# NyanCAD/CedarSim.jl

Measured on AMD Instinct MI355X. Metric: newton_iters_per_sec, higher is better.
Workload: dtype f64

## Files before the change

cedarsim.jl_amd/csrc/ch_bsim4.hpp:

```cpp
#pragma once
#include <cmath>
#include <cstdint>

#include "../../include/cedarhip.h"

#if defined(__HIPCC__)
#define CH_HD __host__ __device__
#define CH_D __device__ __forceinline__
#else
#define CH_HD
#define CH_D inline
#endif

namespace chip {

#define CH_B4_PACKED(X)                                                                              \
  X(type) X(mobmod) X(capmod) X(nf) X(leff) X(weff) X(weffCV) X(weffCJ) X(vtm) X(tratio1) X(toxe)    \
  X(coxe) X(coxp) X(factor1) X(phi) X(sqrtPhi) X(Xdep0) X(vbi_phi) X(cdep0) X(litl) X(ldeb) X(k1)    \
  X(k1ox) X(k2ox) X(vbsc) X(vfb_phi) X(vth0t) X(k3) X(k3b) X(vthNarrowW) X(lpe0term) X(LpeVb)        \
  X(dvt0) X(dvt1L) X(dvt2) X(dvt0w) X(dvt1wWL) X(dvt2w) X(eta0) X(etab) X(kt1eff) X(kt2t)            \
  X(theta0vb0) X(thetaRout) X(vfbzb) X(vtfbphi1) X(vtfbphi2) X(nfactor) X(cdsc) X(cdscb) X(cdscd)    \
  X(cit) X(voffcbn) X(mstar) X(ngate) X(polyT1) X(dvtp0) X(dvtp1) X(ua) X(ub) X(uc) X(u0temp) X(eu)  \
  X(vsattemp) X(a0) X(agsa0) X(a1) X(a2) X(b0term) X(keta) X(xj) X(dwg) X(dwb) X(rds0h) X(rdswmin)   \
  X(prwg) X(prwb) X(delta) X(pclmlitl) X(pdiblb) X(fproutL) X(pdits) X(pditsd) X(pditslL) X(pscbe1l) \
// ... 105 lines not shown
  const double k1ox = k1 * toxe / toxm, k2ox = k2 * toxe / toxm;
  O(k1) = k1; O(k1ox) = k1ox; O(k2ox) = k2ox; O(vbsc) = vbsc;
  const bool vth0Given = has(CH_B4_vth0);
  double vth0 = bin(CH_B4_vth0, type > 0 ? 0.7 : -0.7), vfb;
  if (has(CH_B4_vfb)) vfb = bin(CH_B4_vfb, -1.0);
  else if (vth0Given) vfb = type * vth0 - phi - k1 * sqrtPhi;
  else vfb = -1.0;
  if (!vth0Given) vth0 = type * (vfb + phi + k1ox * sqrtPhi);
  O(vfb_phi) = vfb + phi;
  O(vth0t) = type * vth0;
  O(k3) = k3; O(k3b) = k3b;
  const double vthNW = toxe * phi / (weff + w0);
  O(vthNarrowW) = vthNW;
  const double lpe0s = std::sqrt(1.0 + lpe0 / leff);
  O(lpe0term) = k1ox * (lpe0s - 1.0) * sqrtPhi;
  O(LpeVb) = std::sqrt(1.0 + lpeb / leff);
  O(dvt0) = dvt0; O(dvt1L) = dvt1 * leff; O(dvt2) = dvt2;
  O(dvt0w) = dvt0w; O(dvt1wWL) = dvt1w * weff * leff; O(dvt2w) = dvt2w;
  O(eta0) = bin(CH_B4_eta0, 0.08); O(etab) = bin(CH_B4_etab, -0.07);
  O(kt1eff) = (kt1 + kt1l / leff) * tr1; O(kt2t) = kt2 * tr1;
  auto sce = [&](double x) {
    if (x < EXP_TH) { const double e = std::exp(x), m1 = e - 1.0; return e / (m1 * m1 + 2.0 * e * MIN_EXP); }
    return 1.0 / (MAX_EXP - 2.0);
  };
  const double lt0 = std::sqrt(EPSSI / (epsrox * EPS0) * toxe * Xdep0);
  O(theta0vb0) = sce(dsub * leff / lt0);
  O(thetaRout) = bin(CH_B4_pdiblc1, 0.39) * sce(drout * leff / lt0) + bin(CH_B4_pdiblc2, 0.0086);
  {
    const double v0 = vbi - phi, f1x = factor1 * std::sqrt(Xdep0);
    const double t8 = dvt0w * sce(dvt1w * weff * leff / f1x) * v0, t9 = dvt0 * sce(dvt1 * leff / f1x) * v0;
    const double t5 = k1ox * (lpe0s - 1.0) * sqrtPhi + (kt1 + kt1l / leff) * tr1;
    O(vfbzb) = type * vth0 - t8 - t9 + k3 * vthNW + t5 - phi - k1 * sqrtPhi;
  }
  {
    const double t3 = type * vth0 - vfb - phi;
    double a = type > 0 ? 2.0 * t3 : 2.5 * t3, b = 4.0 * t3;
    O(vtfbphi1) = a < 0 ? 0 : a; O(vtfbphi2) = b < 0 ? 0 : b;
  }
  O(nfactor) = bin(CH_B4_nfactor, 1.0); O(cdsc) = bin(CH_B4_cdsc, 2.4e-4); O(cdscb) = bin(CH_B4_cdscb, 0);
  O(cdscd) = bin(CH_B4_cdscd, 0); O(cit) = bin(CH_B4_cit, 0);
  O(voffcbn) = (bin(CH_B4_voff, -0.08) + par(CH_B4_voffl, 0) / leff) * (1.0 + bin(CH_B4_tvoff, 0) * dT);
  O(mstar) = 0.5 + std::atan(bin(CH_B4_minv, 0)) / PI;
  O(ngate) = ngate;
  O(polyT1) = 1e6 * Q * EPSSI * ngate / (coxe * coxe);
  O(dvtp0) = bin(CH_B4_dvtp0, 0); O(dvtp1) = bin(CH_B4_dvtp1, 0);
  O(ua) = bin(CH_B4_ua, mobmod == 2 ? 1e-15 : 1e-9) + bin(CH_B4_ua1, 1e-9) * tr1;
  O(ub) = bin(CH_B4_ub, 1e-19) + bin(CH_B4_ub1, -1e-18) * tr1;
  O(uc) = bin(CH_B4_uc, mobmod == 1 ? -0.0465 : -0.0465e-9) + bin(CH_B4_uc1, mobmod == 1 ? -0.056 : -0.056e-9) * tr1;
  O(u0temp) = u0 * std::pow(tr, bin(CH_B4_ute, -1.5));
  O(eu) = bin(CH_B4_eu, type > 0 ? 1.67 : 1.0);
  O(vsattemp) = bin(CH_B4_vsat, 8e4) - bin(CH_B4_at, 3.3e4) * tr1;
  const double a0 = bin(CH_B4_a0, 1.0);
  O(a0) = a0; O(agsa0) = bin(CH_B4_ags, 0) * a0; O(a1) = bin(CH_B4_a1, 0); O(a2) = bin(CH_B4_a2, 1.0);
  O(b0term) = bin(CH_B4_b0, 0) / (weff + bin(CH_B4_b1, 0));
  O(keta) = bin(CH_B4_keta, -0.047); O(xj) = xj; O(dwg) = bin(CH_B4_dwg, 0); O(dwb) = bin(CH_B4_dwb, 0);
  {
    const double prt = bin(CH_B4_prt, 0), pww = std::pow(weffCJ * 1e6, bin(CH_B4_wr, 1.0)) * nf;
    double r0 = (bin(CH_B4_rdsw, 200.0) + prt * tr1) * nf / pww, rmin = (par(CH_B4_rdswmin, 0) + prt * tr1) * nf / pww;
    O(rds0h) = 0.5 * (r0 < 0 ? 0 : r0); O(rdswmin) = rmin < 0 ? 0 : rmin;
  }
  O(prwg) = bin(CH_B4_prwg, 1.0); O(prwb) = bin(CH_B4_prwb, 0); O(delta) = bin(CH_B4_delta, 0.01);
  O(pclmlitl) = bin(CH_B4_pclm, 1.3) * litl;
  if (bin(CH_B4_pclm, 1.3) <= MIN_EXP) O(pclmlitl) = 0.0;
  O(pdiblb) = bin(CH_B4_pdiblcb, 0);
  { const double fp = bin(CH_B4_fprout, 0); O(fproutL) = fp <= 0 ? 0.0 : fp * std::sqrt(leff); }
  O(pdits) = bin(CH_B4_pdits, 0); O(pditsd) = bin(CH_B4_pditsd, 0); O(pditslL) = 1.0 + par(CH_B4_pditsl, 0) * leff;
  O(pscbe1l) = bin(CH_B4_pscbe1, 4.24e8) * litl; O(pscbe2) = bin(CH_B4_pscbe2, 1e-5); O(pvag) = bin(CH_B4_pvag, 0);
  { const double al = bin(CH_B4_alpha0, 0) + bin(CH_B4_alpha1, 0) * leff; O(alphaL) = al <= 0 ? 0.0 : al / leff; }
  O(beta0) = bin(CH_B4_beta0, 0);
  {
    const double ag = bin(CH_B4_agidl, 0), bg = bin(CH_B4_bgidl, 2.3e9), cg = bin(CH_B4_cgidl, 0.5);
    O(agidlW) = (ag > 0 && bg > 0 && cg > 0) ? ag * weffCJ * nf : 0.0;
    O(bgidl) = bg; O(cgidl) = cg; O(egidl) = bin(CH_B4_egidl, 0.8); O(toxe3) = 3.0 * toxe;
  }
  O(xpart) = par(CH_B4_xpart, 0);
  const double cgsl = bin(CH_B4_cgsl, 0), cgdl = bin(CH_B4_cgdl, 0);
  const double cf = has(CH_B4_cf) ? bin(CH_B4_cf, 0) : 2.0 * epsrox * EPS0 / PI * std::log(1.0 + 0.4e-6 / toxe);
  const bool dlcOK = has(CH_B4_dlc) && dlc0 > 0;
  const double cgdo = has(CH_B4_cgdo) ? mp[CH_B4_cgdo] : (dlcOK ? dlc0 * coxe - cgdl : 0.6 * xj * coxe);
  const double cgso = has(CH_B4_cgso) ? mp[CH_B4_cgso] : (dlcOK ? dlc0 * coxe - cgsl : 0.6 * xj * coxe);
  const double cgbo = has(CH_B4_cgbo) ? mp[CH_B4_cgbo] : 2.0 * dwc0 * coxe;
  O(cgdo) = (cgdo + cf) * weffCV * nf; O(cgso) = (cgso + cf) * weffCV * nf; O(cgbo) = cgbo * leffCV * nf;
  O(cgslW) = cgsl * weffCV * nf; O(cgdlW) = cgdl * weffCV * nf;
  O(ckappas) = bin(CH_B4_ckappas, 0.6);
  O(ckappad) = has(CH_B4_ckappad) ? bin(CH_B4_ckappad, 0.6) : out[B4I_ckappas];
  O(abulkCVfactor) = 1.0 + std::pow(bin(CH_B4_clc, 1e-7) / leffCV, bin(CH_B4_cle, 0.6));
  O(acde) = bin(CH_B4_acde, 1.0) * std::pow(ndep / 2e16, -0.25);
  O(moinVtm) = bin(CH_B4_moin, 15.0) * vtm;
  O(noff) = bin(CH_B4_noff, 1.0); O(voffcv) = bin(CH_B4_voffcv, 0);
  O(CoxWL) = coxe * weffCV * leffCV * nf; O(toxp8) = 1e8 * toxp;
  {
    double jss = par(CH_B4_jss, 1e-4), jsws = par(CH_B4_jsws, 0), jswgs = par(CH_B4_jswgs, 0);
    double jsd = par(CH_B4_jsd, jss), jswd = par(CH_B4_jswd, jsws), jswgd = par(CH_B4_jswgd, jswgs);
    const double njs = par(CH_B4_njs, 1.0), njd = par(CH_B4_njd, njs);
    const double xtis = par(CH_B4_xtis, 3.0), xtid = par(CH_B4_xtid, xtis);
    if (dT != 0.0) {
      const double e0 = Eg0 / vtm0 - Eg / vtm, lt = std::log(tr);
      const double fs = std::exp((e0 + xtis * lt) / njs), fd = std::exp((e0 + xtid * lt) / njd);
      jss *= fs; jsws *= fs; jswgs *= fs; jsd *= fd; jswd *= fd; jswgd *= fd;
    }
    auto ct = [&](double c, double tc) { const double f = 1.0 + tc * dT; return f > 0 ? c * f : 0.0; };
    auto pt = [&](double p, double tp) { const double r = p - tp * dT; return r < 0.01 ? 0.01 : r; };
    const double tcj = par(CH_B4_tcj, 0), tcjsw = par(CH_B4_tcjsw, 0), tcjswg = par(CH_B4_tcjswg, 0);
    const double tpb = par(CH_B4_tpb, 0), tpbsw = par(CH_B4_tpbsw, 0), tpbswg = par(CH_B4_tpbswg, 0);
    const double cjs = par(CH_B4_cjs, 5e-4), cjd = par(CH_B4_cjd, cjs);
    const double cjsws = par(CH_B4_cjsws, 5e-10), cjswd = par(CH_B4_cjswd, cjsws);
    const double cjswgs = par(CH_B4_cjswgs, cjsws), cjswgd = par(CH_B4_cjswgd, cjswgs);
    const double pbs = par(CH_B4_pbs, 1.0), pbd = par(CH_B4_pbd, pbs), pbsws = par(CH_B4_pbsws, 1.0);
    const double pbswd = par(CH_B4_pbswd, pbsws), pbswgs = par(CH_B4_pbswgs, pbsws), pbswgd = par(CH_B4_pbswgd, pbswgs);
    O(mjs) = par(CH_B4_mjs, 0.5); O(mjd) = par(CH_B4_mjd, out[B4I_mjs]);
    O(mjsws) = par(CH_B4_mjsws, 0.33); O(mjswd) = par(CH_B4_mjswd, out[B4I_mjsws]);
    O(mjswgs) = par(CH_B4_mjswgs, out[B4I_mjsws]); O(mjswgd) = par(CH_B4_mjswgd, out[B4I_mjswgs]);
    O(PhiBS) = pt(pbs, tpb); O(PhiBD) = pt(pbd, tpb); O(PhiBSWS) = pt(pbsws, tpbsw); O(PhiBSWD) = pt(pbswd, tpbsw);
    O(PhiBSWGS) = pt(pbswgs, tpbswg); O(PhiBSWGD) = pt(pbswgd, tpbswg);
    const double dmcg = par(CH_B4_dmcg, 0), dmci = par(CH_B4_dmci, dmcg);
    const double Piso = 2.0 * (dmcg + dmci) + weffCJ, Aiso = (dmcg + dmci) * weffCJ, Psha = 2.0 * dmcg, Asha = dmcg * weffCJ;
    double eS, iS, eD, iD;
    if (((long)nf) % 2) { eS = eD = 1.0; iS = iD = (nf - 1.0) / 2.0; } else { eD = 0.0; iD = nf / 2.0; eS = 2.0; iS = nf / 2.0 - 1.0; }
    auto g = [&](int kpar) { return !std::isnan(ip[kpar]); };
    const double As = g(CH_MOS_AS) ? ip[CH_MOS_AS] : eS * Aiso + iS * Asha, Ad = g(CH_MOS_AD) ? ip[CH_MOS_AD] : eD * Aiso + iD * Asha;
    double Ps = g(CH_MOS_PS) ? (permod == 0 ? ip[CH_MOS_PS] : ip[CH_MOS_PS] - weffCJ * nf) : eS * Piso + iS * Psha;
    double Pd = g(CH_MOS_PD) ? (permod == 0 ? ip[CH_MOS_PD] : ip[CH_MOS_PD] - weffCJ * nf) : eD * Piso + iD * Psha;
    if (Ps < 0) Ps = 0;
    if (Pd < 0) Pd = 0;
    const double Isbs = As * jss + Ps * jsws + weffCJ * nf * jswgs, Isbd = Ad * jsd + Pd * jswd + weffCJ * nf * jswgd;
    O(Isbs) = Isbs; O(Isbd) = Isbd; O(Nvtms) = vtm * njs; O(Nvtmd) = vtm * njd;
    const double ijs = par(CH_B4_ijthsfwd, 0.1), ijd = par(CH_B4_ijthdfwd, ijs);
    if (Isbs > 0) { O(vjsmFwd) = vtm * njs * std::log(ijs / Isbs + 1.0); O(IVjsmFwd) = Isbs * std::exp(out[B4I_vjsmFwd] / (vtm * njs)); }
    if (Isbd > 0) { O(vjdmFwd) = vtm * njd * std::log(ijd / Isbd + 1.0); O(IVjdmFwd) = Isbd * std::exp(out[B4I_vjdmFwd] / (vtm * njd)); }
    O(czbs) = ct(cjs, tcj) * As; O(czbssw) = ct(cjsws, tcjsw) * Ps; O(czbsswg) = ct(cjswgs, tcjswg) * weffCJ * nf;
    O(czbd) = ct(cjd, tcj) * Ad; O(czbdsw) = ct(cjswd, tcjsw) * Pd; O(czbdswg) = ct(cjswgd, tcjswg) * weffCJ * nf;
  }
#undef O
  return CH_OK;
}

#if defined(__HIPCC__)
CH_D double frcp(double x) {
  const double r = __builtin_amdgcn_rcp(x);
  const double e = fma(-x, r, 1.0);
  return fma(r, fma(e, e, e), r);
}
CH_D double fsqrt(double x) {
  double y = __builtin_amdgcn_rsq(x);
  double g = x * y, h = 0.5 * y;
  double r = fma(-h, g, 0.5);
  g = fma(g, r, g); h = fma(h, r, h);
  r = fma(-h, g, 0.5);
  g = fma(g, r, g); h = fma(h, r, h);
  g = fma(fma(-g, g, x), h, g);
  return g;
}

template <int N>
struct DN {
  double v, p[N];
};
template <int N> CH_D DN<N> mkd(double v) { DN<N> r; r.v = v; for (int i = 0; i < N; ++i) r.p[i] = 0.0; return r; }
template <int N> CH_D DN<N> operator+(DN<N> a, DN<N> b) { DN<N> r; r.v = a.v + b.v; for (int i = 0; i < N; ++i) r.p[i] = a.p[i] + b.p[i]; return r; }
template <int N> CH_D DN<N> operator-(DN<N> a, DN<N> b) { DN<N> r; r.v = a.v - b.v; for (int i = 0; i < N; ++i) r.p[i] = a.p[i] - b.p[i]; return r; }
template <int N> CH_D DN<N> operator-(DN<N> a) { DN<N> r; r.v = -a.v; for (int i = 0; i < N; ++i) r.p[i] = -a.p[i]; return r; }
template <int N> CH_D DN<N> operator+(DN<N> a, double b) { a.v += b; return a; }
template <int N> CH_D DN<N> operator+(double b, DN<N> a) { a.v += b; return a; }
template <int N> CH_D DN<N> operator-(DN<N> a, double b) { a.v -= b; return a; }
template <int N> CH_D DN<N> operator-(double b, DN<N> a) { DN<N> r; r.v = b - a.v; for (int i = 0; i < N; ++i) r.p[i] = -a.p[i]; return r; }
template <int N> CH_D DN<N> operator*(DN<N> a, double b) { DN<N> r; r.v = a.v * b; for (int i = 0; i < N; ++i) r.p[i] = a.p[i] * b; return r; }
template <int N> CH_D DN<N> operator*(double b, DN<N> a) { return a * b; }
template <int N> CH_D DN<N> operator*(DN<N> a, DN<N> b) { DN<N> r; r.v = a.v * b.v; for (int i = 0; i < N; ++i) r.p[i] = fma(a.p[i], b.v, a.v * b.p[i]); return r; }
template <int N> CH_D DN<N> recip(DN<N> a) { const double r = frcp(a.v), m = -r * r; DN<N> o; o.v = r; for (int i = 0; i < N; ++i) o.p[i] = a.p[i] * m; return o; }
template <int N> CH_D DN<N> operator/(DN<N> a, DN<N> b) {
  const double r = frcp(b.v), q = a.v * r;
  DN<N> o; o.v = q; for (int i = 0; i < N; ++i) o.p[i] = fma(-q, b.p[i], a.p[i]) * r; return o;
}
template <int N> CH_D DN<N> operator/(DN<N> a, double b) { return a * frcp(b); }
template <int N> CH_D DN<N> operator/(double a, DN<N> b) { return recip(b) * a; }
template <int N> CH_D DN<N> chain(DN<N> a, double f, double fp) { DN<N> r; r.v = f; for (int i = 0; i < N; ++i) r.p[i] = a.p[i] * fp; return r; }
template <int N> CH_D DN<N> dsqrt(DN<N> a) { const double s = fsqrt(a.v); return chain(a, s, 0.5 * frcp(s)); }
enum { KP_EXP = 0, KP_LOG = 10, KP_PRE = 22, KP_COUNT = 26 };
#define CH_KPOOL_VALUES                                                                                                        \
                                                                                \
  0x1.ade156a5dcb37p-26, 0x1.28af3fca7ab0cp-22, 0x1.71dee623fde64p-19, 0x1.a01997c89e6b0p-16, 0x1.a01a014761f6ep-13,           \
  0x1.6c16c1852b7b0p-10, 0x1.1111111122322p-7, 0x1.55555555502a1p-5, 0x1.5555555555511p-3, 0x1.000000000000bp-1,               \
                        \
  1.0 / 19.0, 1.0 / 17.0, 1.0 / 15.0, 1.0 / 13.0, 1.0 / 11.0, 1.0 / 9.0, 1.0 / 7.0, 1.0 / 5.0, 1.0 / 3.0,                      \
  6.93147180369123816490e-01, 1.90821492927058770002e-10, 0.70710678118654752440,                                             \
  0x1.71547652b82fep+0, 0x1.62e42fefa39efp-1, 0x1.abc9e3b39803fp-56, 0.0
struct KLit {
  template <int I> CH_D void pair(double& a, double& b) const { constexpr double t[KP_COUNT] = {CH_KPOOL_VALUES}; a = t[I]; b = t[I + 1]; }
};
typedef double kp_d2 __attribute__((ext_vector_type(2)));
typedef const __attribute__((address_space(3))) kp_d2* kp_lds_ptr;
struct KLds {
  kp_lds_ptr p;
  template <int I> CH_D void pair(double& a, double& b) const { static_assert(I % 2 == 0, "pairs are 16-byte aligned"); const kp_d2 v = p[I / 2]; a = v.x; b = v.y; }
};
CH_D KLds kpool_fill(double* lds_table, int tid) {
  constexpr double t[KP_COUNT] = {CH_KPOOL_VALUES};
  double v = 0.0;
#pragma unroll
  for (int i = 0; i < KP_COUNT; ++i) v = (tid == i) ? t[i] : v;
  if (tid < KP_COUNT) lds_table[tid] = v;
  return KLds{(kp_lds_ptr)(__attribute__((address_space(3))) double*)lds_table};
}

template <class K>
CH_D double fexp(double x, const K k) {
#if defined(__HIP_DEVICE_COMPILE__)
  double c11, c10, c9, c8, c7, c6, c5, c4, c3, c2;
  k.template pair<KP_EXP + 0>(c11, c10); k.template pair<KP_EXP + 2>(c9, c8); k.template pair<KP_EXP + 4>(c7, c6);
  k.template pair<KP_EXP + 6>(c5, c4); k.template pair<KP_EXP + 8>(c3, c2);
  double il2, l2h, l2l, pd;
  k.template pair<KP_PRE + 0>(il2, l2h); k.template pair<KP_PRE + 2>(l2l, pd);
  const double dn = __builtin_rint(x * il2);
  double t = fma(-dn, l2h, x);
  t = fma(-dn, l2l, t);
  double p = fma(t, c11, c10);
  p = fma(t, p, c9); p = fma(t, p, c8); p = fma(t, p, c7); p = fma(t, p, c6); p = fma(t, p, c5); p = fma(t, p, c4);
  p = fma(t, p, c3); p = fma(t, p, c2); p = fma(t, p, 1.0); p = fma(t, p, 1.0);
  double z = __builtin_ldexp(p, (int)dn);
  z = x > 1024.0 ? __builtin_inf() : z;
  z = x < -1075.0 ? 0.0 : z;
  return z;
#else
  return exp(x);
#endif
}
CH_D double fexp(double x) { return fexp(x, KLit{}); }
template <int N, class K> CH_D DN<N> dexp(DN<N> a, const K k) { const double e = fexp(a.v, k); return chain(a, e, e); }
template <int N> CH_D DN<N> dexp(DN<N> a) { return dexp(a, KLit{}); }
template <class K>
CH_D double flog(double x, const K k) {
#if defined(__HIP_DEVICE_COMPILE__)
  double l19, l17, l15, l13, l11, l9, l7, l5, l3, ln2h, ln2l, pad;
  k.template pair<KP_LOG + 0>(l19, l17); k.template pair<KP_LOG + 2>(l15, l13); k.template pair<KP_LOG + 4>(l11, l9);
  k.template pair<KP_LOG + 6>(l7, l5); k.template pair<KP_LOG + 8>(l3, ln2h); k.template pair<KP_LOG + 10>(ln2l, pad);
  double m = __builtin_amdgcn_frexp_mant(x);
  int e = __builtin_amdgcn_frexp_exp(x);
  const bool lo = m < pad;
  m = lo ? 2.0 * m : m;
  e = lo ? e - 1 : e;
  const double s = (m - 1.0) * frcp(m + 1.0);
  const double z = s * s;
  double p = l19;
  p = fma(p, z, l17); p = fma(p, z, l15); p = fma(p, z, l13); p = fma(p, z, l11);
  p = fma(p, z, l9); p = fma(p, z, l7); p = fma(p, z, l5); p = fma(p, z, l3);
  const double lm = fma(2.0 * s, p * z, 2.0 * s);
  const double de = (double)e;
  const double r = fma(de, ln2h, fma(de, ln2l, lm));
  return (x > 0.0 && x < __builtin_inf()) ? r : (x == 0.0 ? -__builtin_inf() : (x > 0.0 ? x : __builtin_nan("")));
#else
  return log(x);
#endif
}
CH_D double flog(double x) { return flog(x, KLit{}); }
template <int N, class K> CH_D DN<N> dlog(DN<N> a, const K k) { return chain(a, flog(a.v, k), frcp(a.v)); }
template <int N> CH_D DN<N> dlog(DN<N> a) { return chain(a, flog(a.v), frcp(a.v)); }

template <int N, class K> CH_D DN<N> d_sce(DN<N> x, const K kc) {
  if (x.v < k::EXP_TH) {
    const DN<N> e = dexp(x, kc), m1 = e - 1.0;
    return e / (m1 * m1 + e * (2.0 * k::MIN_EXP));
  }
  return mkd<N>(1.0 / (k::MAX_EXP - 2.0));
}

struct B4Col {
  const double* p;
  CH_D double operator[](int i) const { return p[i]; }
};
CH_D B4Col b4_col(const double* table, long col) { return B4Col{table + col * (long)B4I_COUNT}; }

template <class K>
CH_D void diode(const K kc, double vb, double Is, double Nvtm, double vjm, double IVjm, double gmin, double& i, double& g) {
  if (Is <= 0.0) { i = gmin * vb; g = gmin; return; }
  const double iN = frcp(Nvtm);
  if (vb <= vjm) {
    const double t = vb * iN;
    if (t < -k::EXP_TH) { i = Is * (k::MIN_EXP - 1.0) + gmin * vb; g = gmin; }
    else { const double e = fexp(t, kc); i = Is * (e - 1.0) + gmin * vb; g = Is * e * iN + gmin; }
  } else {
    const double s = IVjm * iN;
    i = IVjm - Is + s * (vb - vjm) + gmin * vb; g = s + gmin;
  }
}
template <class K>
CH_D void junction(const K kc, double vb, double cz, double czsw, double czswg, double pb, double pbsw, double pbswg, double mj,
                   double mjsw, double mjswg, double& q, double& c) {
  if (vb < 0.0) {
    q = 0.0; c = 0.0;
    if (cz > 0.0) { const double a = 1.0 - vb * frcp(pb), s = fexp(-mj * flog(a, kc), kc); q += pb * cz * (1.0 - a * s) * frcp(1.0 - mj); c += cz * s; }
    if (czsw > 0.0) { const double a = 1.0 - vb * frcp(pbsw), s = fexp(-mjsw * flog(a, kc), kc); q += pbsw * czsw * (1.0 - a * s) * frcp(1.0 - mjsw); c += czsw * s; }
    if (czswg > 0.0) { const double a = 1.0 - vb * frcp(pbswg), s = fexp(-mjswg * flog(a, kc), kc); q += pbswg * czswg * (1.0 - a * s) * frcp(1.0 - mjswg); c += czswg * s; }
  } else {
    const double t0 = cz + czsw + czswg, t1 = cz * mj * frcp(pb) + czsw * mjsw * frcp(pbsw) + czswg * mjswg * frcp(pbswg);
    q = vb * (t0 + 0.5 * t1 * vb); c = t0 + t1 * vb;
  }
}
CH_D void overlap(double vg, double cov, double clW, double ckappa, double& q, double& c) {
  const double t0 = vg + 0.02, t1 = fsqrt(t0 * t0 + 0.08), t2 = 0.5 * (t0 - t1), dt2 = 0.5 * (1.0 - t0 * frcp(t1));
  const double t4 = fsqrt(1.0 - 4.0 * t2 * frcp(ckappa));
  q = (cov + clW) * vg - clW * (t2 + 0.5 * ckappa * (t4 - 1.0));
  c = (cov + clW) - clW * (dt2 - dt2 * frcp(t4));
}

template <int N>
struct B4Core {
  DN<N> iD, iS, iB, qd, qg, qs, qb;
};

template <int N, class K>
CH_D void b4_core(const K kc, const B4Col P, const DN<N> Vgs, const DN<N> Vds, const DN<N> Vbs, B4Core<N>& o) {
  using namespace k;
  typedef DN<N> D;
  auto dexp = [&](const D a) { return chip::dexp(a, kc); };
  auto dlog = [&](const D a) { return chip::dlog(a, kc); };
  auto d_sce = [&](const D a) { return chip::d_sce(a, kc); };
  const double phi = P[B4I_phi], sqrtPhi = P[B4I_sqrtPhi], Vtm = P[B4I_vtm], Leff = P[B4I_leff];
  const double coxe = P[B4I_coxe], itoxe = frcp(P[B4I_toxe]), icoxe = frcp(coxe), iLeff = frcp(Leff);

  D Vbseff;
  {
    const double vbsc = P[B4I_vbsc];
    const D t0 = Vbs - (vbsc + 0.001);
    const D t1 = dsqrt(t0 * t0 - 0.004 * vbsc);
    if (t0.v >= 0.0) Vbseff = 0.5 * (t0 + t1) + vbsc;
    else Vbseff = vbsc * (1.0 + (-0.002) / (t1 - t0));
    const double t9 = 0.95 * phi;
    const D u0 = t9 - Vbseff - 0.001;
    Vbseff = t9 - 0.5 * (u0 + dsqrt(u0 * u0 + 0.004 * t9));
  }
  const D Phis = phi - Vbseff;
  const D sqrtPhis = dsqrt(Phis);
  const D Xdep = sqrtPhis * (P[B4I_Xdep0] * frcp(sqrtPhi));

  const D sqXdep = dsqrt(Xdep);
  const double f1 = P[B4I_factor1], V0 = P[B4I_vbi_phi];
  auto ltf = [&](double dv2) -> D {
    const D a = Vbseff * dv2;
    const D b = (a.v >= -0.5) ? a + 1.0 : (1.0 + 3.0 * a) / (3.0 + 8.0 * a);
    return sqXdep * b * f1;
  };
  const D Theta0 = d_sce(P[B4I_dvt1L] / ltf(P[B4I_dvt2]));
  const D Delt_vth = Theta0 * (P[B4I_dvt0] * V0);
  const double dvt0w = P[B4I_dvt0w];
  D T2w = mkd<N>(0.0);
  if (dvt0w != 0.0) T2w = d_sce(P[B4I_dvt1wWL] / ltf(P[B4I_dvt2w])) * (dvt0w * V0);
  const D T1t = P[B4I_lpe0term] + P[B4I_kt1eff] + Vbseff * P[B4I_kt2t];
  D T3d = P[B4I_eta0] + P[B4I_etab] * Vbseff;
  if (T3d.v < 1.0e-4) T3d = (2.0e-4 - T3d) / (3.0 - 2.0e4 * T3d);
  const D DIBL_Sft = T3d * Vds * P[B4I_theta0vb0];
  const double vthNW = P[B4I_vthNarrowW], LpeVb = P[B4I_LpeVb], k1ox = P[B4I_k1ox], k2ox = P[B4I_k2ox];
  D Vth = P[B4I_vth0t] + (k1ox * sqrtPhis - P[B4I_k1] * sqrtPhi) * LpeVb - k2ox * Vbseff - Delt_vth - T2w +
          (P[B4I_k3] + P[B4I_k3b] * Vbseff) * vthNW + T1t - DIBL_Sft;

  D n;
  {
    const D c1 = EPSSI / Xdep;
    const D t4 = (P[B4I_nfactor] * c1 + (P[B4I_cdsc] + P[B4I_cdscb] * Vbseff + P[B4I_cdscd] * Vds) * Theta0 + P[B4I_cit]) * icoxe;
    n = (t4.v >= -0.5) ? t4 + 1.0 : (1.0 + 3.0 * t4) / (3.0 + 8.0 * t4);
  }
  {
    const double dvtp0 = P[B4I_dvtp0];
    if (dvtp0 > 0.0) {
      const D t0 = -P[B4I_dvtp1] * Vds;
      const D t2 = (t0.v < -EXP_TH) ? mkd<N>(MIN_EXP) : dexp(t0);
      const D t3 = Leff + dvtp0 * (1.0 + t2);
      Vth = Vth - n * (Vtm * dlog(Leff / t3));
    }
  }
  D Vgs_eff = Vgs;
  {
    const double ngate = P[B4I_ngate], vfbphi = P[B4I_vfb_phi];
    if (ngate > 1.0e18 && ngate < 1.0e25 && Vgs.v > vfbphi) {
      const double iT1p = frcp(P[B4I_polyT1]);
      const D t8 = Vgs - vfbphi;
      const D t4 = dsqrt(1.0 + t8 * (2.0 * iT1p));
      const D t2 = 2.0 * t8 / (t4 + 1.0);
      const D t3 = t2 * t2 * (0.5 * iT1p);
      const D t7 = 1.07 - t3;
      const D t6 = dsqrt(t7 * t7 + 0.224);
      Vgs_eff = Vgs - (1.12 - 0.5 * (t7 + t6));
    }
  }
  const D Vgst = Vgs_eff - Vth;

  D Vgsteff;
  const D inVt = recip(n * Vtm);
  {
    const double mstar = P[B4I_mstar], cc = coxe * frcp(P[B4I_cdep0]);
    const D t1 = mstar * Vgst;
    const D t2 = t1 * inVt;
    D t10;
    if (t2.v > EXP_TH) t10 = t1;
    else if (t2.v < -EXP_TH) t10 = n * (Vtm * log(1.0 + MIN_EXP));
    else t10 = (n * Vtm) * dlog(1.0 + dexp(t2));
    const D h2 = (P[B4I_voffcbn] - (1.0 - mstar) * Vgst) * inVt;
    D t9;
    if (h2.v < -EXP_TH) t9 = mstar + n * (cc * MIN_EXP);
    else if (h2.v > EXP_TH) t9 = mstar + n * (cc * MAX_EXP);
    else t9 = mstar + n * (cc * dexp(h2));
    Vgsteff = t10 / t9;
  }

  const D dsp = sqrtPhis - sqrtPhi;
  D Weff = P[B4I_weff] - 2.0 * (P[B4I_dwg] * Vgsteff + P[B4I_dwb] * dsp);
  if (Weff.v < 2.0e-8) Weff = 2.0e-8 * (4.0e-8 - Weff) / (6.0e-8 - 2.0 * Weff);
  D Rds;
  {
    const D t2 = recip(1.0 + P[B4I_prwg] * Vgsteff) + P[B4I_prwb] * dsp;
    Rds = P[B4I_rdswmin] + (t2 + dsqrt(t2 * t2 + 0.01)) * P[B4I_rds0h];
  }
  D Abulk0, Abulk;
  {
    const D t1 = (0.5 * k1ox * LpeVb) / sqrtPhis + (k2ox - P[B4I_k3b] * vthNW);
    const D t5 = Leff / (Leff + 2.0 * dsqrt(P[B4I_xj] * Xdep));
    const D t2 = P[B4I_a0] * t5 + P[B4I_b0term];
    Abulk0 = 1.0 + t1 * t2;
    const D dAdVg = -t1 * (P[B4I_agsa0] * (t5 * t5 * t5));
    Abulk = Abulk0 + dAdVg * Vgsteff;
    if (Abulk0.v < 0.1) Abulk0 = (0.2 - Abulk0) / (3.0 - 20.0 * Abulk0);
    if (Abulk.v < 0.1) Abulk = (0.2 - Abulk) / (3.0 - 20.0 * Abulk);
    const D t2k = P[B4I_keta] * Vbseff;
    const D t0k = (t2k.v >= -0.9) ? recip(1.0 + t2k) : (17.0 + 20.0 * t2k) / (0.8 + t2k);
    Abulk = Abulk * t0k;
    Abulk0 = Abulk0 * t0k;
  }
  D iueff;
  {
    const int mobmod = (int)P[B4I_mobmod];
    D t5;
    if (mobmod == 0) {
      const D t3 = (Vgsteff + Vth + Vth) * itoxe;
      t5 = t3 * (P[B4I_ua] + P[B4I_uc] * Vbseff + P[B4I_ub] * t3);
    } else if (mobmod == 1) {
      const D t3 = (Vgsteff + Vth + Vth) * itoxe;
      t5 = t3 * (P[B4I_ua] + P[B4I_ub] * t3) * (1.0 + P[B4I_uc] * Vbseff);
    } else {
      const D t0 = (Vgsteff + P[B4I_vtfbphi1]) * itoxe;
      t5 = dexp(P[B4I_eu] * dlog(t0)) * (P[B4I_ua] + P[B4I_uc] * Vbseff);
    }
    const D den = (t5.v >= -0.8) ? t5 + 1.0 : (0.6 + t5) / (7.0 + 10.0 * t5);
    iueff = den * frcp(P[B4I_u0temp]);
  }
  const D ueff = recip(iueff);
  const double vsat = P[B4I_vsattemp];
  const D WVCoxRds = Weff * Rds * (vsat * coxe);
  const D Esat = (2.0 * vsat) * iueff;
  const D EsatL = Esat * Leff;
  const D iEsatL = recip(EsatL);
  D Lambda;
  {
    const double a1 = P[B4I_a1], a2 = P[B4I_a2];
    if (a1 == 0.0) Lambda = mkd<N>(a2);
    else if (a1 > 0.0) {
      const double t0 = 1.0 - a2;
      const D t1 = t0 - a1 * Vgsteff - 0.0001;
      Lambda = a2 + t0 - 0.5 * (t1 + dsqrt(t1 * t1 + 0.0004 * t0));
    } else {
      const D t1 = a2 + a1 * Vgsteff - 0.0001;
      Lambda = 0.5 * (t1 + dsqrt(t1 * t1 + 0.0004 * a2));
    }
  }
  const D iLam = recip(Lambda);
  const D Vgst2Vtm = Vgsteff + 2.0 * Vtm;
  const D iVgst2Vtm = recip(Vgst2Vtm);
  D Vdsat;
  if (Rds.v == 0.0 && Lambda.v == 1.0) Vdsat = EsatL * Vgst2Vtm / (Abulk * EsatL + Vgst2Vtm);
  else {
    const D t9 = Abulk * WVCoxRds;
    const D t0 = 2.0 * Abulk * (t9 - 1.0 + iLam);
    const D t1 = Vgst2Vtm * (2.0 * iLam - 1.0) + Abulk * EsatL + 3.0 * (Vgst2Vtm * t9);
    const D t2 = Vgst2Vtm * (EsatL + 2.0 * (Vgst2Vtm * WVCoxRds));
    Vdsat = (t1 - dsqrt(t1 * t1 - 2.0 * t0 * t2)) / t0;
  }
  D Vdseff;
  {
    const double delta = P[B4I_delta];
    const D t1 = Vdsat - Vds - delta;
    const D t2 = dsqrt(t1 * t1 + 4.0 * delta * Vdsat);
    if (t1.v >= 0.0) Vdseff = Vdsat - 0.5 * (t1 + t2);
    else Vdseff = Vdsat * (1.0 - (2.0 * delta) / (t2 - t1));
    if (Vds.v == 0.0) Vdseff = Vds;
    if (Vdseff.v > Vds.v) Vdseff = Vds;
  }
  const D diffVds = Vds - Vdseff;
  const D Vasat = (EsatL + Vdsat + 2.0 * (WVCoxRds * Vgsteff) * (1.0 - 0.5 * Abulk * Vdsat * iVgst2Vtm)) / ((2.0 * iLam - 1.0) + WVCoxRds * Abulk);
  D Idl;
  {
    const D t0 = (Vgsteff + P[B4I_vtfbphi2]) * (0.5 * frcp(P[B4I_toxp8]));
    const D Tcen = 1.9e-9 / (1.0 + dexp(0.7 * dlog(t0)));
    const double coxp = P[B4I_coxp];
    const D Coxeff = (EPSSI * coxp) / (EPSSI + coxp * Tcen);
    const D beta = ueff * Coxeff * Weff * iLeff;
    const D fg1 = Vgsteff * (1.0 - 0.5 * Vdseff * Abulk * iVgst2Vtm);
    const D gche = beta * fg1 / (1.0 + Vdseff * iEsatL);
    Idl = gche / (1.0 + gche * Rds);
  }
  const double fpL = P[B4I_fproutL];
  const D FP = (fpL <= 0.0) ? mkd<N>(1.0) : recip(1.0 + fpL * iVgst2Vtm);
  D Pvag;
  {
    const D t9 = (P[B4I_pvag] * iEsatL) * Vgsteff;
    Pvag = (t9.v > -0.9) ? t9 + 1.0 : (0.8 + t9) / (17.0 + 20.0 * t9);
  }
  D iCclm, VACLM;
  {
    const double pl = P[B4I_pclmlitl];
    if (pl > 0.0 && diffVds.v > 1.0e-10) {
      const D Cclm = FP * Pvag * (1.0 + Rds * Idl) * (Leff + Vdsat * ueff * (0.5 * frcp(vsat))) * frcp(pl);
      iCclm = recip(Cclm);
      VACLM = Cclm * diffVds;
    } else { iCclm = mkd<N>(1.0 / MAX_EXP); VACLM = mkd<N>(MAX_EXP); }
  }
  D iVADIBL;
  {
    const double th = P[B4I_thetaRout];
    if (th > MIN_EXP) {
      const D t8 = Abulk * Vdsat;
      D va = (Vgst2Vtm - Vgst2Vtm * t8 / (Vgst2Vtm + t8)) * frcp(th);
      const D t7 = P[B4I_pdiblb] * Vbseff;
      va = va * ((t7.v >= -0.9) ? recip(1.0 + t7) : (17.0 + 20.0 * t7) / (0.8 + t7));
      iVADIBL = recip(va * Pvag);
    } else iVADIBL = mkd<N>(1.0 / MAX_EXP);
  }
  D iVADITS;
  {
    const double pdits = P[B4I_pdits];
    if (pdits > MIN_EXP) {
      const D t0 = P[B4I_pditsd] * Vds;
      const D t1 = (t0.v > EXP_TH) ? mkd<N>(MAX_EXP) : dexp(t0);
      iVADITS = recip((1.0 + P[B4I_pditslL] * t1) * frcp(pdits) * FP);
    } else iVADITS = mkd<N>(1.0 / MAX_EXP);
  }
  D iVASCBE;
  {
    const double ps2 = P[B4I_pscbe2], ps1l = P[B4I_pscbe1l];
    if (ps2 > 0.0) {
      if (diffVds.v > ps1l / EXP_TH) iVASCBE = (ps2 * iLeff) * dexp(-ps1l / diffVds);
      else iVASCBE = mkd<N>(ps2 * iLeff / MAX_EXP);
    } else iVASCBE = mkd<N>(1.0 / MAX_EXP);
  }
  D Idsa = Idl * (1.0 + diffVds * iVADIBL);
  Idsa = Idsa * (1.0 + diffVds * iVADITS);
  Idsa = Idsa * (1.0 + dlog((Vasat + VACLM) / Vasat) * iCclm);
  D Isub = mkd<N>(0.0);
  {
    const double aL = P[B4I_alphaL], beta0 = P[B4I_beta0];
    if (aL > 0.0 && beta0 > 0.0) {
      D t1;
      if (diffVds.v > beta0 / EXP_TH) t1 = aL * diffVds * dexp(-beta0 / diffVds);
      else t1 = (aL * MIN_EXP) * diffVds;
      Isub = t1 * (Idsa * Vdseff);
    }
  }
  const double nf = P[B4I_nf];
  const D Ids = Idsa * (1.0 + diffVds * iVASCBE) * Vdseff * nf;
  Isub = Isub * nf;
  D Igidl = mkd<N>(0.0), Igisl = mkd<N>(0.0);
  {
    const double agW = P[B4I_agidlW];
    if (agW > 0.0) {
      const double bg = P[B4I_bgidl], cg = P[B4I_cgidl], eg = P[B4I_egidl], it3x = frcp(P[B4I_toxe3]);
      const D Vbd = Vbs - Vds;
      const D t1 = (Vds - Vgs_eff - eg) * it3x;
      if (t1.v > 0.0 && Vbd.v <= 0.0) {
        const D t2 = bg / t1;
        const D ig = (t2.v < 100.0) ? agW * t1 * dexp(-t2) : (agW * 3.720075976e-44) * t1;
        const D t5 = -Vbd * Vbd * Vbd;
        Igidl = ig * (t5 / (cg + t5));
      }
      const D s1 = (-Vgs_eff - eg) * it3x;
      if (s1.v > 0.0 && Vbs.v <= 0.0) {
        const D t2 = bg / s1;
        const D ig = (t2.v < 100.0) ? agW * s1 * dexp(-t2) : (agW * 3.720075976e-44) * s1;
        const D t5 = -Vbs * Vbs * Vbs;
        Igisl = ig * (t5 / (cg + t5));
      }
    }
  }
  D qg = mkd<N>(0.0), qb = mkd<N>(0.0), qsm = mkd<N>(0.0), qdm = mkd<N>(0.0);
  const double xpart = P[B4I_xpart];
  if (xpart >= 0.0 && (int)P[B4I_capmod] != 0) {
    const D VbseffCV = (Vbseff.v < 0.0) ? Vbseff : phi - Phis;
    const double CoxWL = P[B4I_CoxWL], vfbzb = P[B4I_vfbzb], Cox = P[B4I_coxp], Tox = P[B4I_toxp8], ldeb = P[B4I_ldeb];
    const double iTox = frcp(Tox), cwl = CoxWL * icoxe;
    const D T0q = n * (Vtm * P[B4I_noff]);
    const D T1q = (Vgst - P[B4I_voffcv]) / T0q;
    D Vgc;
    if (T1q.v > EXP_TH) Vgc = Vgst - P[B4I_voffcv];
    else if (T1q.v < -EXP_TH) Vgc = T0q * log(1.0 + MIN_EXP);
    else Vgc = T0q * dlog(1.0 + dexp(T1q));
    const D V3 = vfbzb - Vgs_eff + VbseffCV - 0.02;
    const D Vfbeff = vfbzb - 0.5 * (V3 + dsqrt(V3 * V3 + ((vfbzb <= 0.0) ? -0.08 * vfbzb : 0.08 * vfbzb)));
    const D tm = (Vgs_eff - VbseffCV - vfbzb) * (P[B4I_acde] * iTox);
    D Tcen;
    if (tm.v > -EXP_TH && tm.v < EXP_TH) Tcen = ldeb * dexp(tm);
    else Tcen = mkd<N>(tm.v <= -EXP_TH ? ldeb * MIN_EXP : ldeb * MAX_EXP);
    const double LINK = 1.0e-11 * Tox;
    const D V3c = ldeb - Tcen - LINK;
    Tcen = ldeb - 0.5 * (V3c + dsqrt(V3c * V3c + 4.0 * LINK * ldeb));
    D CoxWLcen = (Cox * EPSSI * cwl) / (Cox * Tcen + EPSSI);
    const D Qac0 = CoxWLcen * (Vfbeff - vfbzb);
    const double h0 = 0.5 * k1ox;
    const D T3s = Vgs_eff - Vfbeff - VbseffCV - Vgc;
    D T1s;
    if (k1ox == 0.0) T1s = mkd<N>(0.0);
    else if (T3s.v < 0.0) T1s = h0 + T3s * frcp(k1ox);
    else T1s = dsqrt(h0 * h0 + T3s);
    const D Qsub0 = CoxWLcen * (k1ox * (T1s - h0));
    double Den, T0d;
    if (k1ox <= 0.0) { Den = 0.25 * P[B4I_moinVtm]; T0d = 0.5 * sqrtPhi; }
    else { Den = P[B4I_moinVtm] * k1ox * k1ox; T0d = k1ox * sqrtPhi; }
    const D DeltaPhi = Vtm * dlog(1.0 + (2.0 * T0d + Vgc) * Vgc * frcp(Den));
    const D T3t = 4.0 * (Vth - vfbzb - phi);
    const D T0t = ((T3t.v >= 0.0) ? Vgc + T3t : Vgc + 1.0e-20) * (0.5 * iTox);
    Tcen = 1.9e-9 / (1.0 + dexp(0.7 * dlog(T0t)));
    CoxWLcen = (Cox * EPSSI * cwl) / (Cox * Tcen + EPSSI);
    const D AbulkCV = Abulk0 * P[B4I_abulkCVfactor];
    const D T1 = Vgc - DeltaPhi;
    const D VdsatCV = T1 / AbulkCV;
    const D T0v = VdsatCV - Vds - 0.02;
    const D T1v = dsqrt(T0v * T0v + 0.08 * VdsatCV);
    D VdseffCV;
    if (T0v.v >= 0.0) VdseffCV = VdsatCV - 0.5 * (T0v + T1v);
    else VdseffCV = VdsatCV * (1.0 - 0.04 / (T1v - T0v));
    if (Vds.v == 0.0) VdseffCV = Vds;
    const D T0 = AbulkCV * VdseffCV;
    const D T2 = 12.0 * (T1 - 0.5 * T0 + 1.0e-20);
    const D iT2 = recip(T2);
    const D T3 = T0 * iT2;
    qg = CoxWLcen * (T1 - T0 * (0.5 - T3));
    qb = CoxWLcen * (1.0 - AbulkCV) * (0.5 * VdseffCV - T3 * VdseffCV);
    if (xpart > 0.5) qsm = -CoxWLcen * (0.5 * T1 + 0.25 * T0 - 0.5 * T0 * T3);
    else if (xpart < 0.5) {
      const D T4b = T1 * ((2.0 / 3.0) * T0 * T0 + T1 * (T1 - (4.0 / 3.0) * T0)) - (2.0 / 15.0) * T0 * T0 * T0;
      qsm = -(72.0 * CoxWLcen * (iT2 * iT2)) * T4b;
    } else qsm = -0.5 * qg;
    qg = qg + Qac0 + Qsub0 - qb;
    qb = qb - (Qac0 + Qsub0);
    qdm = -(qg + qb + qsm);
  }
  o.iD = Ids + Isub + Igidl; o.iS = Igisl - Ids; o.iB = -(Isub + Igidl + Igisl);
  o.qd = qdm; o.qg = qg; o.qs = qsm; o.qb = qb;
}

struct B4Two {
  double ibs, gbs, ibd, gbd, qbs, cbs, qbd, cbd, qgd, cgd, qgs, cgs, qgb, cgb;
};
template <class K>
CH_D void b4_two_terminal(const K kc, const B4Col P, double vgs, double vds, double vbs, double gmin, B4Two& t) {
  const double vbd = vbs - vds;
  diode(kc, vbs, P[B4I_Isbs], P[B4I_Nvtms], P[B4I_vjsmFwd], P[B4I_IVjsmFwd], gmin, t.ibs, t.gbs);
  diode(kc, vbd, P[B4I_Isbd], P[B4I_Nvtmd], P[B4I_vjdmFwd], P[B4I_IVjdmFwd], gmin, t.ibd, t.gbd);
  junction(kc, vbs, P[B4I_czbs], P[B4I_czbssw], P[B4I_czbsswg], P[B4I_PhiBS], P[B4I_PhiBSWS], P[B4I_PhiBSWGS], P[B4I_mjs], P[B4I_mjsws], P[B4I_mjswgs], t.qbs, t.cbs);
  junction(kc, vbd, P[B4I_czbd], P[B4I_czbdsw], P[B4I_czbdswg], P[B4I_PhiBD], P[B4I_PhiBSWD], P[B4I_PhiBSWGD], P[B4I_mjd], P[B4I_mjswd], P[B4I_mjswgd], t.qbd, t.cbd);
  if ((int)P[B4I_capmod] != 0) {
    overlap(vgs - vds, P[B4I_cgdo], P[B4I_cgdlW], P[B4I_ckappad], t.qgd, t.cgd);
    overlap(vgs, P[B4I_cgso], P[B4I_cgslW], P[B4I_ckappas], t.qgs, t.cgs);
    t.cgb = P[B4I_cgbo]; t.qgb = t.cgb * (vgs - vbs);
  } else { t.qgd = t.cgd = t.qgs = t.cgs = t.qgb = t.cgb = 0.0; }
}

template <class K = KLit>
CH_D void b4_device(const B4Col P, double vd, double vg, double vs, double vb, double gmin, double* out, const K kc = K{}) {
  const double tp = P[B4I_type];
  const double vds = tp * (vd - vs), vgs = tp * (vg - vs), vbs = tp * (vb - vs);
  const bool fwd = vds >= 0.0;
  typedef DN<3> D3;
  D3 Vgs = mkd<3>(fwd ? vgs : vgs - vds), Vds = mkd<3>(fwd ? vds : -vds), Vbs = mkd<3>(fwd ? vbs : vbs - vds);
  Vgs.p[0] = 1.0; Vds.p[1] = 1.0; Vbs.p[2] = 1.0;
  B4Core<3> c;
  b4_core<3>(kc, P, Vgs, Vds, Vbs, c);
  double* I = out; double* Qo = out + 4; double* G = out + 8; double* C = out + 24;
  auto put = [&](int row, const D3& x, double* val, double* M) {
    val[row] = x.v; M[row * 4 + 0] = x.p[1]; M[row * 4 + 1] = x.p[0]; M[row * 4 + 3] = x.p[2]; M[row * 4 + 2] = -(x.p[0] + x.p[1] + x.p[2]);
  };
  put(0, c.iD, I, G); put(1, mkd<3>(0.0), I, G); put(2, c.iS, I, G); put(3, c.iB, I, G);
  put(0, c.qd, Qo, C); put(1, c.qg, Qo, C); put(2, c.qs, Qo, C); put(3, c.qb, Qo, C);
  if (!fwd) {
    auto sw = [](double& x, double& y) { const double t = x; x = y; y = t; };
    sw(I[0], I[2]); sw(Qo[0], Qo[2]);
#pragma unroll
    for (int cc = 0; cc < 4; ++cc) { sw(G[0 * 4 + cc], G[2 * 4 + cc]); sw(C[0 * 4 + cc], C[2 * 4 + cc]); }
#pragma unroll
    for (int r = 0; r < 4; ++r) { sw(G[r * 4 + 0], G[r * 4 + 2]); sw(C[r * 4 + 0], C[r * 4 + 2]); }
  }
  B4Two t;
  b4_two_terminal(kc, P, vgs, vds, vbs, gmin, t);
  auto two = [&](double* val, double* M, int a, int b, double x, double dx) {
    val[a] += x; val[b] -= x;
    M[a * 4 + a] += dx; M[a * 4 + b] -= dx; M[b * 4 + a] -= dx; M[b * 4 + b] += dx;
  };
  two(I, G, 3, 2, t.ibs, t.gbs); two(I, G, 3, 0, t.ibd, t.gbd);
  two(Qo, C, 3, 2, t.qbs, t.cbs); two(Qo, C, 3, 0, t.qbd, t.cbd);
  two(Qo, C, 1, 0, t.qgd, t.cgd); two(Qo, C, 1, 2, t.qgs, t.cgs); two(Qo, C, 1, 3, t.qgb, t.cgb);
#pragma unroll
  for (int r = 0; r < 4; ++r) { I[r] *= tp; Qo[r] *= tp; }
}

CH_D void b4_device_quad(const B4Col P, double vd, double vg, double vs, double vb, double gmin, int sub, double m, double* st) {
  const double tp = P[B4I_type];
  const double vds = tp * (vd - vs), vgs = tp * (vg - vs), vbs = tp * (vb - vs);
  const bool fwd = vds >= 0.0;
  typedef DN<1> D1;
  D1 Vgs = mkd<1>(fwd ? vgs : vgs - vds), Vds = mkd<1>(fwd ? vds : -vds), Vbs = mkd<1>(fwd ? vbs : vbs - vds);
  Vgs.p[0] = sub == 0 ? 1.0 : 0.0; Vds.p[0] = sub == 1 ? 1.0 : 0.0; Vbs.p[0] = sub == 2 ? 1.0 : 0.0;
  B4Core<1> c;
  b4_core<1>(KLit{}, P, Vgs, Vds, Vbs, c);
  auto quad_sum = [](double x) { x += __shfl_xor(x, 1); x += __shfl_xor(x, 2); return x; };
  auto colval = [&](const D1& x) { const double sum = quad_sum(x.p[0]); return sub == 3 ? -sum : x.p[0]; };
  double gI[4] = {colval(c.iD), 0.0, colval(c.iS), colval(c.iB)};
  double gQ[4] = {colval(c.qd), colval(c.qg), colval(c.qs), colval(c.qb)};
  double I4[4] = {c.iD.v, 0.0, c.iS.v, c.iB.v}, Q4[4] = {c.qd.v, c.qg.v, c.qs.v, c.qb.v};
  int col = sub == 0 ? 1 : (sub == 1 ? 0 : (sub == 2 ? 3 : 2));
  if (!fwd) {
    auto sw = [](double& x, double& y) { const double t = x; x = y; y = t; };
    sw(gI[0], gI[2]); sw(gQ[0], gQ[2]); sw(I4[0], I4[2]); sw(Q4[0], Q4[2]);
    col = col == 0 ? 2 : (col == 2 ? 0 : col);
  }
  B4Two t;
  b4_two_terminal(KLit{}, P, vgs, vds, vbs, gmin, t);
  auto two = [&](double* val, double* gcol, int a, int b, double x, double dx) {
    val[a] += x; val[b] -= x;
    const double s = col == a ? dx : (col == b ? -dx : 0.0);
    gcol[a] += s; gcol[b] -= s;
  };
  two(I4, gI, 3, 2, t.ibs, t.gbs); two(I4, gI, 3, 0, t.ibd, t.gbd);
  two(Q4, gQ, 3, 2, t.qbs, t.cbs); two(Q4, gQ, 3, 0, t.qbd, t.cbd);
  two(Q4, gQ, 1, 0, t.qgd, t.cgd); two(Q4, gQ, 1, 2, t.qgs, t.cgs); two(Q4, gQ, 1, 3, t.qgb, t.cgb);
#pragma unroll
  for (int r = 0; r < 4; ++r) { st[8 + r * 4 + col] = m * gI[r]; st[24 + r * 4 + col] = m * gQ[r]; }
  if (sub == 3) {
    const double mt = m * tp;
#pragma unroll
    for (int r = 0; r < 4; ++r) { st[r] = mt * I4[r]; st[4 + r] = mt * Q4[r]; }
  }
}
#endif

}
```

cedarsim.jl_amd/csrc/ch_engine_persist.hpp:

```cpp
#pragma once

constexpr size_t P_MAX_ENTRIES = 64, P_MAX_PWL = 2048;
inline bool ch_circuit::persist_eligible(std::string& why, bool own_steps) {
  auto no = [&](const char* m) { why = m; return false; };
  if (nwt.path != 1) return no("the circuit takes the sparse path");
  if (desc.A.n_comp < 1) return no("the circuit has no unknowns");
  if (!(stru.lu_variant == 8 || stru.lu_variant == 12 || stru.lu_variant == 16)) return no("a Jacobian block has more than 16 unknowns");
  if (desc.A.wide) {
    if (desc.A.classes.size() != 1) return no("compiled Verilog-A devices in blocks of several classes");
    if (desc.A.nb > 0) return no("compiled Verilog-A devices in a bordered form");
    if (stru.wide_split ? (stru.wide_l + stru.wide_other > 32) : (stru.h_cms[0].nslots > 64)) return no("a block's compiled devices need more evaluation lanes than a wave pair offers");
    if (own_steps && tab.S == 1 && desc.A.n_comp > 1) return no("per-block steps of one circuit with compiled Verilog-A devices");
  } else if (stru.block_threads != 64) return no("a block needs more than one wavefront of device slots");
  if (tab.max_mc > 8) return no("more than 8 MOSFET classes in a block");
  if (tab.Ssrc != 1) return no("per-sample source parameters");
  const bool wg_consts = own_steps && tab.S == 1 && desc.A.n_comp > 1;
  if (!wg_consts && (stru.needed_src.size() > (size_t)P_MAXSRC || desc.A.known.size() + (size_t)stru.n_dev_src() > P_MAX_ENTRIES)) return no("more than 64 sources / known-node and source values per attempt");
  if (!(tab.S == 1 || desc.A.n_comp == 1)) return no("several blocks per sample in a multi-sample batch");
  if (desc.A.nb > 0 && (tab.S != 1 || desc.A.border_dev.size() > 8)) return no("bordered form: one sample and at most 8 devices on the border alone");
  for (const ClassMeta& m : stru.h_cms) if ((!desc.A.wide && m.nslots > 64) || m.nc > stru.lu_variant || m.n_work <= 0 || m.spare1 <= 0) return no("a block class does not fit the one-wave register path");
  if (ps.n_cu == 0) { hipDeviceProp_t prop; if (hipGetDeviceProperties(&prop, ctx->device) != hipSuccess) return no("hipGetDeviceProperties failed"); ps.n_cu = prop.multiProcessorCount; }
  const long nblk = (long)desc.A.n_comp * tab.S;
  const int bpw = persist_bpw(nblk);
  if (nblk > (long)bpw * ps.n_cu && !own_steps) return no("more blocks than resident wavefronts (4 per CU)");
  if (!own_steps && (nblk + bpw - 1) / bpw > 256) return no("more than 256 workgroups in a grid-wide reduction");
  size_t npwl = 0; for (int i : stru.needed_src) npwl += desc.src[i].ts.size();
  if (!wg_consts && npwl > P_MAX_PWL) return no("piecewise-linear tables above 2048 points");
  return true;
}
inline int ch_circuit::persist_bpw(long nblk) const {
  if (ps.n_cu > 0 && desc.A.wide && stru.wide_split && nblk <= 2L * ps.n_cu) return 2;
  return PW;
}
inline bool ch_circuit::persist_own_steps(const ch_tran_opts& o) const {
  return ((desc.A.n_comp == 1 && tab.S > 1) || (tab.S == 1 && desc.A.n_comp > 1 && desc.A.nb == 0 && !desc.A.wide)) && o.n_saveat > 0 && o.step_control != CH_STEPS_SHARED && !env_on(Env::LOCKSTEP);
}
inline size_t ch_circuit::persist_wave_doubles(bool wg_consts) const {
  const size_t n_ent = wg_consts ? (size_t)P_MAXSRC : desc.A.known.size() + stru.n_dev_src();
  return stru.lds_doubles_fixed + 16 * (size_t)desc.A.max_nc + 10 + 48 + P_MAXSRC + n_ent + (size_t)tab.max_mc * B4L_STRIDE + (stru.lds_extra_bytes + stru.lds_plan_bytes + 7) / 8 + 2;
}
inline bool ch_circuit::persist_blob(const std::vector<int>& kn, const std::vector<int>& ds, std::vector<int>& bi, std::vector<double>& bd, std::vector<int>& need) const {
  const int nsrc = (int)desc.src.size();
  std::vector<char> nd(std::max(1, nsrc), 0);
  for (int k : kn) for (auto& tm : desc.A.known[k].terms) nd[tm.first] = 1;
  for (int j : ds) if (j < (int)stru.dev_src.size()) nd[stru.dev_src[j]] = 1;
  need.clear();
  for (int i = 0; i < nsrc; ++i) if (nd[i]) need.push_back(i);
  std::vector<int> pos(std::max(1, nsrc), -1);
  for (size_t i = 0; i < need.size(); ++i) pos[need[i]] = (int)i;
  std::vector<double> pt, py;
  bi = {(int)need.size(), (int)(kn.size() + ds.size()), 0, (int)kn.size()};
  for (int i : need) { bi.push_back(desc.src[i].kind); bi.push_back((int)pt.size()); bi.push_back((int)desc.src[i].ts.size()); pt.insert(pt.end(), desc.src[i].ts.begin(), desc.src[i].ts.end()); py.insert(py.end(), desc.src[i].ys.begin(), desc.src[i].ys.end()); }
  bi[2] = (int)pt.size();
  std::vector<int> eptr(1, 0), eidx; std::vector<double> ecoef;
  for (int k : kn) { for (auto& tm : desc.A.known[k].terms) { eidx.push_back(pos[tm.first]); ecoef.push_back(tm.second); } eptr.push_back((int)eidx.size()); }
  for (int j : ds) { if (j < (int)stru.dev_src.size()) { eidx.push_back(pos[stru.dev_src[j]]); ecoef.push_back(1.0); } eptr.push_back((int)eidx.size()); }
  bi.insert(bi.end(), eptr.begin(), eptr.end()); bi.insert(bi.end(), eidx.begin(), eidx.end());
  bd.clear();
  for (int i : need) for (int k = 0; k < CH_SRC_NPAR; ++k) bd.push_back(tab.h_src_par[(size_t)i * CH_SRC_NPAR + k]);
  bd.insert(bd.end(), ecoef.begin(), ecoef.end()); bd.insert(bd.end(), pt.begin(), pt.end()); bd.insert(bd.end(), py.begin(), py.end());
  for (size_t q = 4; q < bi.size(); ++q) if (bi[q] < 0) return false;
  return need.size() <= (size_t)P_MAXSRC && kn.size() + ds.size() <= P_MAX_ENTRIES && pt.size() <= P_MAX_PWL;
}

inline const void* persist_kernel(bool wide, int mode, int nc, bool pair) {
  struct Row { bool wide; int mode, nc; bool pair; const void* fn; };
  static const Row rows[] = {
    {true, PM_OWN, 16, true, (const void*)tran_persistent_kernel<16, true, PM_OWN, true>}, {true, PM_OWN, 16, false, (const void*)tran_persistent_kernel<16, false, PM_OWN, true>},
    {true, PM_LOCKSTEP, 16, true, (const void*)tran_persistent_kernel<16, true, PM_LOCKSTEP, true>}, {true, PM_LOCKSTEP, 16, false, (const void*)tran_persistent_kernel<16, false, PM_LOCKSTEP, true>},
    {false, PM_BORDER, 16, true, (const void*)tran_persistent_kernel<16, true, PM_BORDER>}, {false, PM_BORDER, 16, false, (const void*)tran_persistent_kernel<16, false, PM_BORDER>},
    {false, PM_OWN, 12, true, (const void*)tran_persistent_kernel<12, true, PM_OWN>}, {false, PM_OWN, 12, false, (const void*)tran_persistent_kernel<12, false, PM_OWN>},
    {false, PM_OWN, 16, true, (const void*)tran_persistent_kernel<16, true, PM_OWN>}, {false, PM_OWN, 16, false, (const void*)tran_persistent_kernel<16, false, PM_OWN>},
    {false, PM_LOCKSTEP, 12, true, (const void*)tran_persistent_kernel<12, true>}, {false, PM_LOCKSTEP, 12, false, (const void*)tran_persistent_kernel<12, false>},
    {false, PM_LOCKSTEP, 16, true, (const void*)tran_persistent_kernel<16, true>}, {false, PM_LOCKSTEP, 16, false, (const void*)tran_persistent_kernel<16, false>},
  };
  for (const Row& r : rows) if (r.wide == wide && r.mode == mode && r.nc == nc && r.pair == pair) return r.fn;
  return nullptr;
}

struct PersistConsts {
  std::vector<int> ci; std::vector<double> cd; size_t max_ci = 0, max_cd = 0;
  std::vector<int> wgc, wgk;
  std::vector<double> bps_all;
};
inline bool ch_circuit::persist_consts(bool wg_consts, int n_wg, int bpw, double t0, double t1, PersistConsts& pc) {
  const int nblk = desc.A.n_comp * tab.S, nk = (int)desc.A.known.size(), nds = stru.n_dev_src();
  if (!wg_consts) {
    std::vector<int> kn(nk), ds(nds), need;
    std::iota(kn.begin(), kn.end(), 0); std::iota(ds.begin(), ds.end(), 0);
    if (!persist_blob(kn, ds, pc.ci, pc.cd, need)) { set_err("device-resident stepper: the source tables exceed the kernel's limits"); return false; }
    pc.max_ci = pc.ci.size(); pc.max_cd = pc.cd.size();
  } else {
    pc.wgk.assign((size_t)n_wg * P_MAXSRC, -1);
    for (int w = 0; w < n_wg; ++w) {
      std::vector<char> uk(nk, 0), ud(nds, 0);
      for (int b = w * bpw; b < std::min(nblk, (w + 1) * bpw); ++b)
        for (int i = 0; i < desc.A.comp_ndev[b]; ++i) {
          const EDev& e = desc.A.edev[desc.A.comp_dofs[b] + i];
          for (int k = 0; k < NTERM; ++k) if (e.term[k] < 0) uk[-e.term[k] - 1] = 1;
          if (e.src >= 0) ud[torn.dsrc_host[desc.A.comp_dofs[b] + i]] = 1;
        }
      std::vector<int> kn, ds, need, bi; std::vector<double> bd;
      for (int k = 0; k < nk; ++k) if (uk[k]) kn.push_back(k);
      for (int j = 0; j < nds; ++j) if (ud[j]) ds.push_back(j);
      if (ds.empty()) ds.push_back(0);
      if (!persist_blob(kn, ds, bi, bd, need)) { set_err("device-resident stepper: a workgroup's blocks reference more than 64 sources / known nodes"); return false; }
      for (size_t q = 0; q < kn.size(); ++q) pc.wgk[(size_t)w * P_MAXSRC + q] = kn[q];
      for (size_t q = 0; q < ds.size(); ++q) pc.wgk[(size_t)w * P_MAXSRC + kn.size() + q] = ds[q];
      std::vector<double> wb, wc;
      { std::vector<std::pair<double, double>> pts;
        for (int i : need) source_breakpoint_codes(desc.src[i], &tab.h_src_par[(size_t)i * CH_SRC_NPAR], t0, t1, pts);
        merge_breakpoints(pts, t1, wb, wc); }
      pc.wgc.insert(pc.wgc.end(), {(int)pc.ci.size(), (int)pc.cd.size(), (int)bi.size(), (int)bd.size(), (int)pc.bps_all.size(), (int)wb.size()});
      pc.ci.insert(pc.ci.end(), bi.begin(), bi.end()); pc.cd.insert(pc.cd.end(), bd.begin(), bd.end());
      pc.bps_all.insert(pc.bps_all.end(), wb.begin(), wb.end());
      pc.bps_all.insert(pc.bps_all.end(), wc.begin(), wc.end());
      pc.max_ci = std::max(pc.max_ci, bi.size()); pc.max_cd = std::max(pc.max_cd, bd.size());
    }
  }
  return true;
}

inline size_t ch_circuit::persist_va_arena(int bpw, size_t& lds) const {
  size_t va_arena = 0;
  if (desc.A.wide && !env_on(Env::VA_NO_LDS)) {
    size_t worst = 0;
    for (int cpt = 0; cpt < desc.A.n_comp; ++cpt) {
      size_t need = 0;
      for (int i = 0; i < desc.A.comp_ndev[cpt]; ++i) {
        const EDev& e = desc.A.edev[desc.A.comp_dofs[cpt] + i];
        if (e.kind != K_VA) continue;
        const int mod = desc.dev[e.hdev].ipar[0];
        need += (size_t)((va_gen::param_doubles(mod) + 1) & ~1) + (size_t)((va_gen::cache_doubles(mod) + 1) & ~1);
      }
      worst = std::max(worst, need);
    }
    const size_t room = lds < 148 * 1024 ? (148 * 1024 - lds) / sizeof(double) : 0;
    va_arena = std::min(worst * (size_t)bpw, room);
    lds += va_arena * sizeof(double);
    if (env_on(Env::DEBUG_STEPPER)) std::fprintf(stderr, "[stepper] compiled devices: %zu doubles per block, LDS arena %zu doubles, workgroup LDS %zu bytes\n", worst, va_arena, lds);
  }
  return va_arena;
}

inline int ch_circuit::persist_collect(ch_result& R, const TranCtl& cs, bool own_steps, bool single_batch, const std::vector<double>& htimes,
                                       const std::vector<double>& hpts, const std::vector<double>& hrows, int status, hclock::time_point tstart) {
  hipStream_t st = ctx->stream;
  const int n_obs = R.n_obs;
  stats.persist_attempts = cs.n_attempts;
  stats.persist_barrier_s = (double)cs.t_cycles_barrier * 1e-8;
#ifdef CH_STAMPS
  { static const char* nm[12] = {"set-up", "coefficients", "sources", "predictor", "eval", "gather", "rows+norm", "LU+solves", "update", "candidate", "grid-reduce", "controller"};
    std::fprintf(stderr, "[pstamps] attempts %lld; cycles per attempt (wave 0 of workgroup 0):", cs.n_attempts);
    for (int q = 0; q < 12; ++q) std::fprintf(stderr, " %s %.0f", nm[q], (double)cs.stamps[q] / (double)std::max<long long>(1, cs.n_attempts));
    std::fprintf(stderr, "\n"); }
#endif
  R.stats.naccept += cs.naccept; R.stats.nreject += cs.nreject; R.stats.nnonlinconvfail += cs.nconvfail;
  const long long arr_iters = (own_steps && tab.S == 1) ? cs.max_iters : cs.sum_iters;
  R.stats.n_block_iters += cs.sum_block_iters; R.stats.nnonliniter += arr_iters; R.stats.nf += arr_iters; R.stats.njacs += arr_iters;
  R.stats.nfactors += arr_iters; R.stats.nsolve += arr_iters;
  const size_t nt = htimes.size();
  R.times = htimes;
  R.pts.assign(nt, 0);
  if (own_steps == false) for (size_t r = 0; r < nt; ++r) R.pts[r] = (int32_t)hpts[r];
  R.values.assign((size_t)n_obs * nt * tab.S, 0.0);
  if (single_batch) {
    const size_t n = (size_t)n_obs * nt * tab.S;
    if (n > 0) {
      HIPCHK(ps.d_ptrans.alloc(n));
      hipLaunchKernelGGL(transpose_rows_kernel, dim3((unsigned)std::min<size_t>(65535, (n + 255) / 256)), dim3(256), 0, st, (const double*)ps.d_prows.p, ps.d_ptrans.p, (long)nt, (long)n_obs, tab.S);
      HIPCHK(hipGetLastError());
      HIPCHK(hipMemcpyAsync(R.values.data(), ps.d_ptrans.p, n * sizeof(double), hipMemcpyDeviceToHost, st));
      HIPCHK(hipStreamSynchronize(st));
      bool plain = true;
      for (int ob = 0; ob < n_obs && plain; ++ob) {
        if (stru.obs_primary[ob] != ob) plain = false;
        else if (desc.obs_kind[ob] == 0 && desc.A.node_unknown[desc.obs_index[ob]] < 0) plain = false;
        else if (desc.obs_kind[ob] == 1) { const int br = desc.dev[desc.obs_index[ob]].branch; if (br < 0 || desc.A.branch_unknown[br] < 0) plain = false; }
      }
      if (plain) { R.dev_values = ps.d_ptrans.p; R.dev_n = (int64_t)n; }
    }
  } else
  rows_to_obs_major(hrows.data(), nt, 0, nt, n_obs, tab.S, R.values.data());
  return finish_tran(R, 0, cs.t, status, tstart);
}

inline int ch_circuit::tran_persistent(double t0, double t1, const ch_tran_opts& o, ch_result& R, const std::vector<double>& bps, int kmax, double dtmin, double dtmax,
                                       int max_steps, int nmaxit, hclock::time_point tstart, bool& used, const ch_dc_opts* dcm, long long* dc_iters,
                                       const std::vector<double>* bpc) {
  used = false;
  hipStream_t st = ctx->stream;
  g_arena = &arena;
// ... 196 lines not shown
```

cedarsim.jl_amd/csrc/ch_kernels.hpp:

```cpp
#pragma once
#include <hip/hip_runtime.h>

#include "ch_analysis.hpp"
#include "ch_bsim4.hpp"
#include "_generated/va_models.hpp"

namespace chip {

struct ClassMeta {
  int nc, ndev, nonlinear, nslots;
  int wl_ofs, n_work, spare0, spare1;
  int n_mat_src, n_vec_src, blob_ofs, blob_ints;
};

struct BlockMeta {
  int uofs, dofs, mc_n, mc_ofs;
  ClassMeta cm;
  int mc[8];
};

struct BlockOut {
  int status;
  int iters;
  int ndiff;
// ... 87 lines not shown
};
__device__ __forceinline__ void widen_stamp(const double* t, double* st) {
#pragma unroll
  for (int k = 0; k < 4; ++k) {
    st[k] = t[k]; st[8 + k] = t[4 + k];
#pragma unroll
    for (int j = 0; j < 4; ++j) { st[16 + k * 8 + j] = t[8 + k * 4 + j]; st[80 + k * 8 + j] = t[24 + k * 4 + j]; }
  }
}

__device__ __forceinline__ void eval_linear(const EvalCtx& a, int kind, int d, long pi, double m, const double (&v)[4], const double* svl, double* st) {
  switch (kind) {
    case K_R: {
      const double g = m / a.dpar[pi], i = g * (v[0] - v[1]);
      st[0] = i; st[1] = -i; st[4] = 0.0; st[5] = 0.0;
      st[8] = g; st[9] = -g; st[12] = -g; st[13] = g;
      st[24] = 0.0; st[25] = 0.0; st[28] = 0.0; st[29] = 0.0;
    } break;
    case K_C: {
      const double c = m * a.dpar[pi], q = c * (v[0] - v[1]);
      st[0] = 0.0; st[1] = 0.0; st[4] = q; st[5] = -q;
      st[8] = 0.0; st[9] = 0.0; st[12] = 0.0; st[13] = 0.0;
      st[24] = c; st[25] = -c; st[28] = -c; st[29] = c;
    } break;
    case K_I: {
      const double i = m * svl[a.dsrc[d]];
      st[0] = i; st[1] = -i; st[4] = 0.0; st[5] = 0.0;
    } break;
    case K_V: case K_L: case K_VCVS_A: {
      const double ib = v[2];
      const double src = kind == K_V ? svl[a.dsrc[d]] : 0.0;
      const double l = kind == K_L ? a.dpar[pi] : 0.0;
      st[0] = m * ib; st[1] = -m * ib; st[2] = v[0] - v[1] - src;
      st[4] = 0.0; st[5] = 0.0; st[6] = -l * ib;
      st[8 + 2] = m; st[8 + 6] = -m; st[8 + 8] = 1.0; st[8 + 9] = -1.0; st[8 + 10] = 0.0;
      st[24 + 2] = 0.0; st[24 + 6] = 0.0; st[24 + 8] = 0.0; st[24 + 9] = 0.0; st[24 + 10] = -l;
    } break;
    case K_VCVS_B: {
      const double g = a.dpar[pi];
      st[0] = -g * (v[1] - v[2]); st[4] = 0.0;
      st[8 + 1] = -g; st[8 + 2] = g; st[24 + 1] = 0.0; st[24 + 2] = 0.0;
    } break;
    case K_VCCS: {
      const double g = m * a.dpar[pi], i = g * (v[2] - v[3]);
      st[0] = i; st[1] = -i; st[4] = 0.0; st[5] = 0.0;
      st[8 + 2] = g; st[8 + 3] = -g; st[8 + 6] = -g; st[8 + 7] = g;
      st[24 + 2] = 0.0; st[24 + 3] = 0.0; st[24 + 6] = 0.0; st[24 + 7] = 0.0;
    } break;
  }
}

__device__ __noinline__ void b4_device_call(const B4Col P, double vd, double vg, double vs, double vb, double gmin, double* out) {
  VA_KEEP_RETURN_ADDRESS;
  b4_device(P, vd, vg, vs, vb, gmin, out);
}
template <bool WIDE>
__device__ __forceinline__ void eval_slot(const EvalCtx a, int s, int dofs, int slot, const double* xl, int uofs,
                                          const double* kvl, const double* svl, const double* pl, double* stage) {
  const int dl = (slot >> 4) & 0x01ffffff;
  const int d = dofs + dl;
  double* st_final = stage + (size_t)dl * StampLayout<WIDE>::STRIDE;
  const int kind = a.dkind[d];
  const int* tm = a.dterm + NTERM * d;
  if (WIDE && kind == K_VA) {
    double vv[NTERM];
#pragma unroll
    for (int k = 0; k < NTERM; ++k) { const int t = tm[k]; vv[k] = t >= 0 ? xl[t - uofs] : kvl[-t - 1]; }
    const long pi = (long)a.dhdev[d] * a.Spar + (a.Spar > 1 ? s : 0);
    const va::Env env{a.temp_k, a.gmin};
    va_gen::stamp_dir_c(a.dcls_local[d], a.vapar + a.dsrc[d], a.vacache + a.dvac[d], vv, env, a.dmult[pi], slot & 7, (slot & 8) != 0,
                        (slot & (1 << 29)) ? ((slot >> 30) & 1) : -1, st_final);
    return;
  }
  double tmp40[WIDE ? 40 : 1];
  double* st = WIDE ? tmp40 : st_final;
  if (WIDE) {
#pragma unroll
    for (int j = 0; j < 40; ++j) tmp40[j] = 0.0;
  }
  double v[4];
#pragma unroll
  for (int k = 0; k < 4; ++k) { const int t = tm[k]; v[k] = t >= 0 ? xl[t - uofs] : kvl[-t - 1]; }
  const int hd = a.dhdev[d];
  const long pi = (long)hd * a.Spar + (a.Spar > 1 ? s : 0);
  const double m = a.dmult[pi];
  if (kind == K_MOS) {
    const B4Col P{pl + (size_t)a.dcls_local[d] * B4L_STRIDE};
    double o[40];
    if (WIDE) b4_device_call(P, v[0], v[1], v[2], v[3], a.gmin, o);
    else b4_device(P, v[0], v[1], v[2], v[3], a.gmin, o);
#pragma unroll
    for (int j = 0; j < 40; ++j) st[j] = m * o[j];
    if (WIDE) widen_stamp(st, st_final);
    return;
  }
  eval_linear(a, kind, d, pi, m, v, svl, st);
  if (WIDE) widen_stamp(st, st_final);
}

struct WideMeta {
  int mod, dl;
  const double* P; const double* C;
  double m;
  int t[NTERM];
};
__device__ __forceinline__ WideMeta load_wide_meta(const EvalCtx& a, int s, int dofs, int slot) {
  WideMeta q;
  q.mod = -1; q.dl = 0; q.P = nullptr; q.C = nullptr; q.m = 0.0;
#pragma unroll
  for (int k = 0; k < NTERM; ++k) q.t[k] = -1;
  if (slot < 0) return q;
  const int dl = (slot >> 4) & 0x01ffffff, d = dofs + dl;
  if (a.dkind[d] != K_VA) return q;
  q.dl = dl; q.mod = a.dcls_local[d];
  q.P = a.vapar + a.dsrc[d]; q.C = a.vacache + a.dvac[d];
  q.m = a.dmult[(long)a.dhdev[d] * a.Spar + (a.Spar > 1 ? s : 0)];
#pragma unroll
  for (int k = 0; k < NTERM; ++k) q.t[k] = a.dterm[NTERM * d + k];
  return q;
}
template <bool LDS>
__device__ __forceinline__ void eval_wide_cached(const WideMeta& q, const EvalCtx& a, int slot, const double* xl, int uofs, const double* kvl, double* stage) {
  double vv[NTERM];
#pragma unroll
  for (int k = 0; k < NTERM; ++k) { const int t = q.t[k]; vv[k] = t >= 0 ? xl[t - uofs] : kvl[-t - 1]; }
  const va::Env env{a.temp_k, a.gmin};
  const int part = (slot & (1 << 29)) ? ((slot >> 30) & 1) : -1;
  double* st = stage + (size_t)q.dl * StampLayout<true>::STRIDE;
  if (LDS) va_gen::stamp_dir_lds(q.mod, (va::lds_cptr)q.P, (va::lds_cptr)q.C, vv, env, q.m, slot & 7, (slot & 8) != 0, part, st);
  else va_gen::stamp_dir_c(q.mod, q.P, q.C, vv, env, q.m, slot & 7, (slot & 8) != 0, part, st);
}

struct SlotMeta {
  int kind;
  int dl;
  int t[4];
  int cls, src;
  double m, par;
};
__device__ __forceinline__ SlotMeta load_slot_meta(const EvalCtx& a, int s, int dofs, int uofs, int slot) {
  SlotMeta q;
  q.kind = 0; q.dl = 0; q.cls = 0; q.src = 0; q.m = 0.0; q.par = 0.0;
#pragma unroll
  for (int k = 0; k < 4; ++k) q.t[k] = -1;
  if (slot < 0) return q;
  const int dl = slot >> 4, d = dofs + dl;
  q.dl = dl; q.kind = a.dkind[d];
#pragma unroll
  for (int k = 0; k < 4; ++k) { const int t = a.dterm[NTERM * d + k]; q.t[k] = t >= 0 ? t - uofs : t; }
  const long pi = (long)a.dhdev[d] * a.Spar + (a.Spar > 1 ? s : 0);
  q.m = a.dmult[pi]; q.par = a.dpar[pi]; q.cls = a.dcls_local[d]; q.src = a.dsrc[d];
  return q;
}
template <int PART, class K = KLit>
__device__ __forceinline__ void eval_cached(const SlotMeta& q, double gmin, const double* xl, const double* kvl, const double* svl, const double* pl, double* stage, const K kc = K{}) {
  if (q.kind == 0 || (PART == 0 && q.kind != K_MOS)) return;
  double* st = stage + (size_t)q.dl * StampLayout<false>::STRIDE;
  double v[4];
#pragma unroll
  for (int k = 0; k < 4; ++k) v[k] = q.t[k] >= 0 ? xl[q.t[k]] : kvl[-q.t[k] - 1];
  if (q.kind == K_MOS) {
    const B4Col P{pl + (size_t)q.cls * B4L_STRIDE};
    double o[40];
    b4_device(P, v[0], v[1], v[2], v[3], gmin, o, kc);
    if (PART != 1) {
#pragma unroll
      for (int j = 0; j < 4; ++j) st[j] = q.m * o[j];
#pragma unroll
      for (int j = 8; j < 24; ++j) st[j] = q.m * o[j];
    }
    if (PART != 0) {
#pragma unroll
      for (int j = 4; j < 8; ++j) st[j] = q.m * o[j];
#pragma unroll
      for (int j = 24; j < 40; ++j) st[j] = q.m * o[j];
    }
    return;
  }
  const double m = q.m;
  switch (q.kind) {
    case K_R: {
      const double g = m / q.par, i = g * (v[0] - v[1]);
      st[0] = i; st[1] = -i; st[4] = 0.0; st[5] = 0.0;
      st[8] = g; st[9] = -g; st[12] = -g; st[13] = g;
      st[24] = 0.0; st[25] = 0.0; st[28] = 0.0; st[29] = 0.0;
    } break;
    case K_C: {
      const double c = m * q.par, qq = c * (v[0] - v[1]);
      st[0] = 0.0; st[1] = 0.0; st[4] = qq; st[5] = -qq;
      st[8] = 0.0; st[9] = 0.0; st[12] = 0.0; st[13] = 0.0;
      st[24] = c; st[25] = -c; st[28] = -c; st[29] = c;
    } break;
    case K_I: {
      const double i = m * svl[q.src];
      st[0] = i; st[1] = -i; st[4] = 0.0; st[5] = 0.0;
    } break;
    case K_V: case K_L: case K_VCVS_A: {
      const double ib = v[2];
      const double src = q.kind == K_V ? svl[q.src] : 0.0;
      const double l = q.kind == K_L ? q.par : 0.0;
      st[0] = m * ib; st[1] = -m * ib; st[2] = v[0] - v[1] - src;
      st[4] = 0.0; st[5] = 0.0; st[6] = -l * ib;
      st[8 + 2] = m; st[8 + 6] = -m; st[8 + 8] = 1.0; st[8 + 9] = -1.0; st[8 + 10] = 0.0;
      st[24 + 2] = 0.0; st[24 + 6] = 0.0; st[24 + 8] = 0.0; st[24 + 9] = 0.0; st[24 + 10] = -l;
    } break;
    case K_VCVS_B: {
      const double g = q.par;
      st[0] = -g * (v[1] - v[2]); st[4] = 0.0;
      st[8 + 1] = -g; st[8 + 2] = g; st[24 + 1] = 0.0; st[24 + 2] = 0.0;
    } break;
    case K_VCCS: {
      const double g = m * q.par, i = g * (v[2] - v[3]);
      st[0] = i; st[1] = -i; st[4] = 0.0; st[5] = 0.0;
      st[8 + 2] = g; st[8 + 3] = -g; st[8 + 6] = -g; st[8 + 7] = g;
      st[24 + 2] = 0.0; st[24 + 3] = 0.0; st[24 + 6] = 0.0; st[24 + 7] = 0.0;
    } break;
  }
}

template <int CTRL> __device__ __forceinline__ int dpp_i(int v) { return __builtin_amdgcn_update_dpp(v, v, CTRL, 0xF, 0xF, false); }
template <int CTRL> __device__ __forceinline__ double dpp_d(double v) {
  const int lo = dpp_i<CTRL>(__double2loint(v)), hi = dpp_i<CTRL>(__double2hiint(v));
  return __hiloint2double(hi, lo);
}
constexpr int DPP_QP_1032 = 0xB1, DPP_QP_2301 = 0x4E, DPP_HALF_MIRROR = 0x141, DPP_MIRROR = 0x140;
template <int NCV> __device__ __forceinline__ double row_max(double v) {
  v = fmax(v, dpp_d<DPP_QP_1032>(v)); v = fmax(v, dpp_d<DPP_QP_2301>(v));
  v = fmax(v, dpp_d<DPP_HALF_MIRROR>(v)); v = fmax(v, dpp_d<DPP_MIRROR>(v));
  if (NCV > 16) v = fmax(v, __shfl_xor(v, 16));
  return v;
}
template <int NCV> __device__ __forceinline__ double row_sum(double v) {
  v += dpp_d<DPP_QP_1032>(v); v += dpp_d<DPP_QP_2301>(v); v += dpp_d<DPP_HALF_MIRROR>(v); v += dpp_d<DPP_MIRROR>(v);
  if (NCV > 16) v += __shfl_xor(v, 16);
  return v;
}
template <int NCV> __device__ __forceinline__ int row_min_i(int v) {
  v = min(v, dpp_i<DPP_QP_1032>(v)); v = min(v, dpp_i<DPP_QP_2301>(v)); v = min(v, dpp_i<DPP_HALF_MIRROR>(v)); v = min(v, dpp_i<DPP_MIRROR>(v));
  if (NCV > 16) v = min(v, __shfl_xor(v, 16));
  return v;
}

template <int NCV> __device__ __forceinline__ int row_max_i(int v) {
  v = max(v, dpp_i<DPP_QP_1032>(v)); v = max(v, dpp_i<DPP_QP_2301>(v)); v = max(v, dpp_i<DPP_HALF_MIRROR>(v)); v = max(v, dpp_i<DPP_MIRROR>(v));
  if (NCV > 16) v = max(v, __shfl_xor(v, 16));
  return v;
}

template <int NC>
__device__ __forceinline__ bool lu_solve_regs(double (&r)[NC + 1], int nc, int lane, double& sol, int* myrow_out = nullptr) {
  bool done = lane >= nc;
  int mystep = -1;
  double ipiv = 0.0;
  int piv[NC];
#pragma unroll
  for (int k = 0; k < NC; ++k) {
    piv[k] = 0;
    if (k < nc) {
      const int hi = __double2hiint(r[k]) & 0x7fffffff;
      const int key = done ? -1 : ((hi & ~63) | (63 - lane));
      const int best = __builtin_amdgcn_readfirstlane(row_max_i<NC>(key));
      if (best < 64 || best >= 0x7e300000) return false;
      const int bi = 63 - (best & 63);
      piv[k] = bi;
      const double ipk = frcp(bcast(r[k], bi));
      const double l = (!done && lane != bi) ? r[k] * ipk : 0.0;
#pragma unroll
      for (int j = k + 1; j <= NC; ++j) r[j] = fma(-l, bcast(r[j], bi), r[j]);
      if (lane == bi) { done = true; mystep = k; ipiv = ipk; }
    }
  }
  double rhs = 0.0;
#pragma unroll
  for (int j = 0; j <= NC; ++j) if (j == nc) rhs = r[j];
  double out = 0.0;
#pragma unroll
  for (int k = NC - 1; k >= 0; --k) {
    if (k < nc) {
      const double xk = bcast(rhs * ipiv, piv[k]);
      if (lane == k) out = xk;
      if (mystep >= 0 && mystep < k) rhs = fma(-r[k], xk, rhs);
    }
  }
  sol = out;
  if (myrow_out) {
    int mr = lane;
#pragma unroll
    for (int k = 0; k < NC; ++k) if (k < nc && lane == k) mr = piv[k];
    *myrow_out = mr;
  }
  return true;
}

template <int K> __device__ __forceinline__ double row_bcast(double v) {
  static_assert(K >= 0 && K < 16, "row_newbcast lane");
  const double b = __builtin_amdgcn_update_dpp(v, v, 0x150 + K, 0xF, 0xF, true);
  return b;
}
template <int NC, int J> struct RowDot {
  static __device__ __forceinline__ double run(const double (&c)[NC], double x, int nc, double q) {
    if constexpr (J < NC) {
      if (J < nc) { const double xj = row_bcast<J>(x); q = fma(c[J], xj, q); }
      return RowDot<NC, J + 1>::run(c, x, nc, q);
    } else return q;
  }
};

template <int NC, int K>
struct LuStaticStep {
  static __device__ __forceinline__ void fwd(double (&r)[NC + 1], int nc, int lane, int& lkey, double& ipiv) {
    if constexpr (K < NC) {
      if (K < nc) {
        const double ipk = frcp(row_bcast<K>(r[K]));
        double pj[NC + 1];
#pragma unroll
        for (int j = K + 1; j <= NC; ++j) pj[j] = row_bcast<K>(r[j]);
        if (lane == K) ipiv = ipk;
// ... 885 lines not shown
```

cedarsim.jl_amd/csrc/ch_persist.hpp:

```cpp
#pragma once
#include <hip/hip_runtime.h>

#include "ch_gather_plan.hpp"
#include "ch_kernels.hpp"

#ifdef CH_STAMPS
#define P_STAMP(slot) do { const unsigned long long now_ = __builtin_readcyclecounter(); pacc_[slot] += now_ - plast_; plast_ = now_; } while (0)
#else
#define P_STAMP(slot) do { } while (0)
#endif

namespace chip {

constexpr int PW = 4;
constexpr int P_MAXSRC = 64;
constexpr int P_NREC = 8;
constexpr int P_SCR = 64;
enum { PX_RUNNING = 0, PX_DONE = 1, PX_ROWS_FULL = 2, PX_ABORT = 3 };

struct TranCtl {
  double t, h;
  double tslot[8];
  int k, nhist, steps_at_order, reset_rate;
  int ibp, isave, status, exit_reason;
// ... 176 lines not shown
    double v = part[f];
#pragma unroll
    for (int w = 1; w < PW; ++w) { const double u = part[w * P_NREC + f]; v = fmaxop ? fmax(v, u) : v + u; }
    if (p.n_wg > 1) {
      if (lane < 16) st_gran(wrec + (size_t)wg * 16 + g16, p_split(v, lane, gen));
      const long long t0 = wall_clock64();
      if (wg < n_grp) {
        const int members = (p.n_wg - grp + 7) >> 3;
        p_u64 x[8];
        for (;;) {
          bool all = true;
          const unsigned ab = ld_agent_u(abort_flag);
#pragma unroll
          for (int q = 0; q < 8; ++q) {
            const int mm = q * 4 + m4;
            x[q] = mm < members ? ld_gran(wrec + (size_t)(grp + 8 * mm) * 16 + g16) : ((p_u64)gen << 32);
            all = all && (unsigned)(x[q] >> 32) == gen;
          }
          if (__all(all)) break;
          if (ab != 0u) { ok = false; break; }
          if (wall_clock64() - t0 > p.spin_ticks) { __hip_atomic_store(abort_flag, 1u | (gen << 8), __ATOMIC_RELAXED, __HIP_MEMORY_SCOPE_AGENT); ok = false; break; }
          __builtin_amdgcn_s_sleep(1);
        }
        double acc = (m4 < members) ? p_join(x[0], lane) : 0.0;
#pragma unroll
        for (int q = 1; q < 8; ++q) {
          const double u = (q * 4 + m4 < members) ? p_join(x[q], lane) : 0.0;
          acc = fmaxop ? fmax(acc, u) : acc + u;
        }
        acc = p_rows4(acc, fmaxop, scr, lane);
        if (lane < 16) st_gran(grec + (size_t)grp * 16 + g16, p_split(acc, lane, gen));
      }
      p_u64 y[2];
      for (;;) {
        bool all = true;
        const unsigned ab = ok ? ld_agent_u(abort_flag) : 1u;
#pragma unroll
        for (int q = 0; q < 2; ++q) {
          const int gg = q * 4 + m4;
          y[q] = (ok && gg < n_grp) ? ld_gran(grec + (size_t)gg * 16 + g16) : ((p_u64)gen << 32);
          all = all && (unsigned)(y[q] >> 32) == gen;
        }
        if (__all(all) || !ok) break;
        if (ab != 0u) { ok = false; break; }
        if (wall_clock64() - t0 > p.spin_ticks) { __hip_atomic_store(abort_flag, 2u | (gen << 8), __ATOMIC_RELAXED, __HIP_MEMORY_SCOPE_AGENT); ok = false; break; }
        __builtin_amdgcn_s_sleep(1);
      }
      double acc = (m4 < n_grp) ? p_join(y[0], lane) : 0.0;
      { const double u = (4 + m4 < n_grp) ? p_join(y[1], lane) : 0.0; acc = fmaxop ? fmax(acc, u) : acc + u; }
      v = p_rows4(acc, fmaxop, scr, lane);
    }
    if (lane < 16 && !(lane & 1)) summ[f] = v;
    if (lane == 0) *s_abort = ok ? 0 : 1;
  }
  __syncthreads();
  return *s_abort == 0;
}

__device__ __forceinline__ double p_coef(double tau0, const double* tsl, int head, int kk, int np, int nkm1, int nkp1, bool lte, double hh, int lane, double& a0) {
  double tau[8];
  tau[0] = tau0;
#pragma unroll
  for (int i = 1; i < 8; ++i) tau[i] = tsl[(head - (i - 1)) & 7];
  const int set = lane >> 3, j = lane & 7;
  const int npk = kk | (np << 4) | (nkm1 << 8) | (nkp1 << 12);
  const int n = set <= 3 ? (npk >> (4 * set)) & 15 : 0;
  const bool act = set <= 3 && j >= 1 && j <= n;
  const unsigned mn = act ? ((2u << n) - 2u) & ~(1u << j) : 0u;
  const unsigned md = mn | ((act && set == 0) ? 1u : 0u);
  const bool rcp = lane >= 33 && lane <= 37, cks = lane >= 38 && lane <= 40;
  const int pick = lane == 38 ? kk + 1 : lane == 39 ? kk : kk + 2;
  const int m = cks ? ((pick >= 1 && pick <= 8) ? pick : 1) : j;
  const double tj = tsl[(head - (m - 1)) & 7];
  double num = 1.0, den = 1.0;
#pragma unroll
  for (int i = 0; i < 8; ++i) {
    num *= ((mn >> i) & 1u) ? tau[0] - tau[i] : 1.0;
    den *= ((md >> i) & 1u) ? tj - tau[i] : 1.0;
  }
  if (!act) { num = 0.0; den = 1.0; }
  const bool on = rcp ? j <= kk : lane == 38 ? lte : lane == 39 ? nkm1 > 0 : nkp1 > 0;
  if (rcp || cks) { num = on ? (rcp ? 1.0 : hh) : 0.0; den = tau[0] - tj; }
  if (num == 0.0) den = 1.0;
  const double q = num / den;
  a0 = bcast(row_sum<16>(rcp ? q : 0.0), 32);
  return q;
}
__device__ __attribute__((noinline, cold)) double p_coef_dense(double tsv, const double* tsl, int head, int msv, int lane) {
  double a0;
  return p_coef(tsv, tsl, head, 0, msv, 0, 0, false, 0.0, lane, a0);
}

enum { PM_LOCKSTEP = 0, PM_OWN = 1, PM_BORDER = 2 };
template <int NC, bool PAIR, int MODE = PM_LOCKSTEP, bool WIDE = false>
__global__ __launch_bounds__(PW * 64, 1) void tran_persistent_kernel(const PersistArgs p) {
  typedef StampLayout<WIDE> SL;
  extern __shared__ double lds[];
  __shared__ int s_abort;
  __shared__ double s_bdec[4];
  __shared__ __attribute__((aligned(16))) double s_kpool[KP_COUNT];
  const NewtonArgs& a = p.a;
  const int tid = threadIdx.x, lane = tid & 63, wave = tid >> 6, wg = blockIdx.x;
  const long long cyc0 = wall_clock64();
  long long cyc_bar = 0;
#ifdef CH_STAMPS
  unsigned long long pacc_[12] = {0, 0, 0, 0, 0, 0, 0, 0, 0, 0, 0, 0}, plast_ = __builtin_readcyclecounter();
#endif
  double* cdl = lds;
  int* cil = (int*)(cdl + p.n_cd);
  double* part = cdl + p.n_cd + ((p.n_ci + 1) >> 1);
  double* summ = part + PW * P_NREC;
  int* pfl = (int*)(summ + P_NREC);
  double* W = summ + P_NREC + 4 + P_SCR + (size_t)wave * p.wave_doubles;
  constexpr bool own = MODE == PM_OWN;
  const int* const wgc = own ? p.wgc : nullptr;
  const double* bps_own = nullptr; int nbp_own = 0;
  if (own && wgc) {
    const int* e = wgc + 6 * wg;
    const int* gci = p.ci + e[0]; const double* gcd = p.cd + e[1]; const int n_ci = e[2], n_cd = e[3];
    bps_own = p.bps + e[4]; nbp_own = e[5];
    for (int i = tid; i < n_cd; i += PW * 64) cdl[i] = gcd[i];
    for (int i = tid; i < n_ci; i += PW * 64) cil[i] = gci[i];
  } else {
    for (int i = tid; i < p.n_cd; i += PW * 64) cdl[i] = p.cd[i];
    for (int i = tid; i < p.n_ci; i += PW * 64) cil[i] = p.ci[i];
  }
#define P_BPS ((own && wgc) ? bps_own : p.bps)
#define P_NBP ((own && wgc) ? nbp_own : p.nbp)
  if (tid == 0) s_abort = 0;
  if (tid < 8) pfl[tid] = 0;
  const KLds kpool = kpool_fill(s_kpool, tid);
  __syncthreads();
  const PConst C{cil, cdl};

  const int blk = wg * p.bpw + wave;
  const bool live = wave < p.bpw && blk < p.nblk;
  const int bq = live ? blk : 0;
  const int c = bq / a.S, s = bq - c * a.S;
  const BlockMeta bm = a.bmeta[c];
  const ClassMeta cm = bm.cm;
  const int nc = cm.nc, ndev = cm.ndev, uofs = bm.uofs, dofs = bm.dofs, lda = nc + 1;
  double* st = W;
  double* A = st + (size_t)ndev * SL::STRIDE;
  double* Cm = A + (size_t)nc * lda;
  double* xl = Cm + (size_t)nc * nc;
  double* xp = xl + nc; double* Fv = xp + nc; double* Qv = Fv + nc; double* hq = Qv + nc;
  double* wv = hq + nc; double* qn = wv + nc; double* pm = qn + nc; double* pp = pm + nc; double* x0l = pp + nc;
  int* dml = (int*)(x0l + nc);
  double* Xh = x0l + 2 * nc; double* Qh = Xh + 8 * nc;
  double* tsl = Qh + 8 * nc; double* coef = tsl + 8;
  long long* stl = (long long*)(coef + 40);
  double* kvl = coef + 48; double* svl = kvl + (wgc ? C.ci[3] : a.nk);
  double* pl = wgc ? kvl + P_MAXSRC : svl + a.nsrc;
  int* mptr = (int*)(pl + (size_t)a.max_mc * B4L_STRIDE);
  int* slots = mptr + (nc * nc + 1) + (nc + 1);
  const int* gplan = mptr + cm.blob_ints;
  const int g_recs = (cm.spare0 - GP_HEAD_INTS) / 3;
  const uint2* gsrc = (const uint2*)(gplan + GP_HEAD_INTS);
  const unsigned* gctl = (const unsigned*)(gplan + GP_HEAD_INTS + 2 * g_recs);
  const int g_trips = __builtin_amdgcn_readfirstlane(cm.spare1);
  const long sofs = (long)s * a.n_unk + uofs;
  const bool mine = live && lane < nc;
  const int nc_s = __builtin_amdgcn_readfirstlane(nc);
  const int role = wave & 1, pairq = wave >> 1, half = lane >> 5;
  int* pf = pfl + pairq * 4;
  const int blk_h = wg * p.bpw + (wave & ~1) + half;
  const bool live_h = PAIR && (wave & ~1) + half < p.bpw && blk_h < p.nblk;
  const int bqh = live_h ? blk_h : 0, c_h = bqh / a.S, s_h = bqh - c_h * a.S;
  const int uofs_h = PAIR ? a.bmeta[c_h].uofs : uofs, dofs_h = PAIR ? a.bmeta[c_h].dofs : dofs;
  double* Wh = summ + P_NREC + 4 + P_SCR + (size_t)((wave & ~1) + half) * p.wave_doubles;
  double* st_h = Wh; double* xl_h = Wh + (xl - W); double* pl_h = Wh + (pl - W);
  const int* slots_h = (const int*)((const char*)slots + ((const char*)Wh - (const char*)W));
  int pseq = 0; bool pair_broken = false;
  auto pair_sync = [&]() {
    ++pseq;
    lds_fence();
    if (lane == 0) __hip_atomic_store(pf + role, pseq, __ATOMIC_RELAXED, __HIP_MEMORY_SCOPE_WORKGROUP);
    long long t0w = 0;
    for (unsigned trip = 1; __hip_atomic_load(pf + (1 - role), __ATOMIC_RELAXED, __HIP_MEMORY_SCOPE_WORKGROUP) < pseq; ++trip) {
      if (trip % P_SPIN_CLOCK == 0u) {
        const long long now = wall_clock64();
        if (trip == P_SPIN_CLOCK) t0w = now;
        else if (now - t0w > p.spin_ticks) { pair_broken = true; __hip_atomic_store(p.counters + 9 * 32, 3u | ((unsigned)pseq << 8), __ATOMIC_RELAXED, __HIP_MEMORY_SCOPE_AGENT); break; }
      }
      __builtin_amdgcn_s_sleep(0);
    }
    lds_fence();
  };

  if (live) {
    const int* bsrc = a.blob + cm.blob_ofs;
    for (int i = lane; i < cm.blob_ints + cm.spare0; i += 64) mptr[i] = bsrc[i];
    const long scol = a.Smos > 1 ? s : 0;
    const int total = bm.mc_n * B4I_COUNT;
    for (int e = lane; e < total; e += 64) {
      const int j = e / B4I_COUNT, i = e - j * B4I_COUNT;
      int cl = bm.mc[0];
#pragma unroll
      for (int q = 1; q < 8; ++q) cl = (j == q) ? bm.mc[q] : cl;
      pl[j * B4L_STRIDE + i] = a.mosp[((long)cl * a.Smos + scol) * (long)B4I_COUNT + i];
    }
    for (int i = lane; i < nc * lda + nc * nc; i += 64) A[i] = 0.0;
    if (mine) {
      dml[lane] = a.dmask[uofs + lane] | ((a.unk_obs[uofs + lane] + 1) << 8);
#pragma unroll
      for (int j = 0; j < 7; ++j) {
        const bool have = j < p.ctl->nhist;
        Xh[((8 - j) & 7) * nc + lane] = have ? a.X[(long)j * a.slot_stride + sofs + lane] : 0.0;
        Qh[((8 - j) & 7) * nc + lane] = have ? a.Qh[(long)j * a.slot_stride + sofs + lane] : 0.0;
      }
      Xh[1 * nc + lane] = 0.0; Qh[1 * nc + lane] = 0.0;
    }
  }
  if (lane < 8) tsl[(8 - lane) & 7] = p.ctl->tslot[lane];
  {
    const double nd = row_sum<16>((mine && (dml[lane] & 1)) ? 1.0 : 0.0);
    if (lane == 0) coef[35] = nd;
  }
  double t, h; int k, nhist, steps_at_order, ibp, isave, status = CH_OK, exit_reason = PX_RUNNING;
  bool reset_rate;
  int nsaved, step;
  enum { ST_ACC = 0, ST_REJ, ST_FAIL, ST_ITERS, ST_BITERS, ST_ATT };
  int head = 0;
  {
    const TranCtl* cs = p.ctl;
    t = cs->t; h = cs->h; k = cs->k; nhist = cs->nhist; steps_at_order = cs->steps_at_order; reset_rate = cs->reset_rate != 0;
    ibp = cs->ibp; isave = cs->isave; nsaved = (int)cs->nsaved; step = (int)cs->step;
    if (lane == 0) { stl[ST_ACC] = cs->naccept; stl[ST_REJ] = cs->nreject; stl[ST_FAIL] = cs->nconvfail; stl[ST_ITERS] = cs->sum_iters; stl[ST_BITERS] = cs->sum_block_iters; stl[ST_ATT] = cs->n_attempts; }
  }
  double rate_prev = 1.0;
  int myrow = lane;
  const unsigned g_head = live ? (unsigned)gplan[lane] : 0u;
  if (MODE != PM_BORDER && a.perm && mine && p.resume) myrow = lane ^ (int)a.perm[(long)blk * 16 + lane];
  lds_fence();
  __syncthreads();

  const int s_e = PAIR ? s_h : s;
  const EvalCtx ectx{a.dkind, a.dterm, a.dsrc, a.dcls_local, a.dhdev, a.dpar, a.dmult, a.Spar, a.gmin_s[a.Sgmin > 1 ? s_e : 0],
                     WIDE ? a.vapar + (long)s_e * a.va_stride : a.vapar, WIDE ? a.temp_s[a.Stemp > 1 ? s_e : 0] + 273.15 : 300.15,
                     WIDE ? a.vacache + (long)s_e * a.vac_stride : nullptr, WIDE ? a.dvac : nullptr};
  const double gmin_h = a.gmin_s[a.Sgmin > 1 ? (PAIR ? s_h : s) : 0];
  SlotMeta smeta;
  int wslot = -1;
  if (WIDE) {
    smeta = load_slot_meta(ectx, 0, 0, 0, -1);
    if (PAIR) {
      const int sq = lane & 31;
      if (live_h) {
        if (sq < p.wide_l) wslot = slots_h[role == 0 ? sq : 64 + sq];
        else if (role == 0 && sq - p.wide_l < p.wide_other) wslot = slots_h[64 + p.wide_l + (sq - p.wide_l)];
      }
    } else if (live && lane < cm.nslots) wslot = slots[lane];
  }
  WideMeta wmeta = load_wide_meta(ectx, PAIR ? s_h : s, PAIR ? dofs_h : dofs, WIDE ? wslot : -1);
  bool va_lds = false;
  if (WIDE && p.va_arena > 0) {
    __shared__ unsigned long long s_va_ptr[32];
    __shared__ int s_va_ofs[32];
    __shared__ int s_va_n, s_va_top, s_va_fail;
    double* arena = summ + P_NREC + 4 + P_SCR + (size_t)PW * p.wave_doubles;
    if (tid == 0) { s_va_n = 0; s_va_top = 0; s_va_fail = 0; }
    __syncthreads();
    const double* staged[2] = {nullptr, nullptr};
    for (int w = 0; w < PW; ++w) {
      if (wave == w) {
#pragma unroll
        for (int which = 0; which < 2; ++which) {
          const double* g = which ? wmeta.C : wmeta.P;
          const int n = wmeta.mod < 0 ? 0 : (which ? va_gen::cache_doubles(wmeta.mod) : va_gen::param_doubles(wmeta.mod));
          bool pend = n > 0;
          for (;;) {
            const unsigned long long bal = __ballot(pend);
            if (!bal) break;
            const int srcl = __ffsll((long long)bal) - 1;
            const unsigned long long gp = ((unsigned long long)(unsigned)__shfl((int)((unsigned long long)g >> 32), srcl) << 32) | (unsigned)__shfl((int)(unsigned long long)g, srcl);
            const int nn = __shfl(n, srcl);
            const int ndir = s_va_n, top = s_va_top;
            int ofs = -1;
            for (int e = 0; e < ndir; ++e) if (s_va_ptr[e] == gp) ofs = s_va_ofs[e];
            if (ofs < 0 && ndir < 32 && top + nn <= p.va_arena) {
              ofs = top;
              const double* gsrc = (const double*)gp;
              for (int i = lane; i < nn; i += 64) arena[top + i] = gsrc[i];
              lds_fence();
              if (lane == 0) { s_va_ptr[ndir] = gp; s_va_ofs[ndir] = top; s_va_n = ndir + 1; s_va_top = top + ((nn + 1) & ~1); }
              lds_fence();
            }
            if (ofs < 0 && lane == 0) s_va_fail = 1;
            if (pend && (unsigned long long)g == gp) { staged[which] = ofs >= 0 ? arena + ofs : nullptr; pend = false; }
          }
        }
      }
      __syncthreads();
    }
    va_lds = s_va_fail == 0;
    if (va_lds && wmeta.mod >= 0) { wmeta.P = staged[0] ? staged[0] : arena; wmeta.C = staged[1] ? staged[1] : arena; }
  }
  if (!WIDE)
  {
    int slot = -1;
    if (PAIR) { const int sq = lane & 31; if (live_h && sq < cm.nslots) slot = slots_h[sq]; }
    else if (live && lane < cm.nslots) slot = slots[lane];
    smeta = load_slot_meta(ectx, PAIR ? s_h : s, PAIR ? dofs_h : dofs, PAIR ? uofs_h : uofs, slot);
    if (wgc && smeta.kind != 0) {
      const int* wk = p.wgk + (size_t)wg * P_MAXSRC;
      const int nkl = C.ci[3], nel = C.n_ent();
#pragma unroll
      for (int k = 0; k < 4; ++k) if (smeta.t[k] < 0) {
        const int g = -smeta.t[k] - 1; int j = 0;
        while (j < nkl - 1 && wk[j] != g) ++j;
        smeta.t[k] = -(j + 1);
      }
      if (smeta.kind == K_I || smeta.kind == K_V) { int j = nkl; while (j < nel - 1 && wk[j] != smeta.src) ++j; smeta.src = j - nkl; }
    }
  }
  const int n_ent = C.n_ent();
  const int e_p0 = lane < n_ent ? C.ent_ptr()[lane] : 0, e_nt = lane < n_ent ? C.ent_ptr()[lane + 1] - e_p0 : 0;
  const int e_i0 = e_nt > 0 ? C.ent_idx()[e_p0] : 0, e_i1 = e_nt > 1 ? C.ent_idx()[e_p0 + 1] : 0;
  const double e_c0 = e_nt > 0 ? C.ent_coef()[e_p0] : 0.0, e_c1 = e_nt > 1 ? C.ent_coef()[e_p0 + 1] : 0.0;
  double s0_lo = __builtin_inf(), s0_hi = -__builtin_inf(), s0_y = 0.0, s0_m = 0.0, s1_lo = __builtin_inf(), s1_hi = -__builtin_inf(), s1_y = 0.0, s1_m = 0.0;
  double bp_next = 0.0; int bp_at = -1;
  double bp_code = -1.0;
  double sv_next = 0.0; int sv_at = -1;
  const long long row_stride = (long long)p.n_obs * a.S;
  const int my_ob = mine ? (dml[lane] >> 8) - 1 : -1;
  unsigned gen = 0;

  if (!p.resume) {
    if (p.n_saveat == 0) {
      if (my_ob >= 0) p.out_rows[(long long)nsaved * row_stride + (long long)my_ob * a.S + s] = Xh[lane];
      if (blk == 0 && lane == 0) p.out_times[nsaved] = t;
      ++nsaved;
    } else {
      while (isave < p.n_saveat && p.saveat[isave] <= t) {
        if (my_ob >= 0) p.out_rows[(long long)nsaved * row_stride + (long long)my_ob * a.S + s] = Xh[lane];
        if (blk == 0 && lane == 0) p.out_times[nsaved] = p.saveat[isave];
        ++nsaved; ++isave;
      }
    }
  }

  P_STAMP(0);
  while (step < p.max_steps && t < p.t1) {
    if (p.n_saveat == 0 && nsaved >= p.max_rows) { exit_reason = PX_ROWS_FULL; break; }
    int ln = lane;
    asm volatile("" : "+v"(ln));
    for (;;) {
      if (bp_at != ibp) { bp_next = ibp < P_NBP ? P_BPS[ibp] : p.t1; bp_code = ibp < P_NBP ? P_BPS[P_NBP + ibp] : -1.0; bp_at = ibp; }
      if (ibp < P_NBP && bp_next <= t * (1 + 1e-15) + 1e-300) ++ibp; else break;
    }
    const double tb = bp_next;
    bool hit_bp = false;
    double tn = t + h;
    if (tn >= tb - 1e-3 * h) { tn = tb; hit_bp = true; }
    const double hh = tn - t;
    const bool dcm = MODE == PM_BORDER && p.dc_mode != 0;
    if (!dcm && hh < p.dtmin) { status = CH_ERR_DTMIN; break; }
    const int nh = nhist, kk = k < nh ? k : nh, np = (kk + 1) < nh ? (kk + 1) : nh;
    const bool lte = np >= kk + 1;
    const bool try_up = lte && kk < p.kmax && nh >= kk + 2 && steps_at_order + 1 >= kk + 1;
    const int nkm1 = (lte && kk > 1) ? kk : 0, nkp1 = try_up ? kk + 2 : 0;
    double alpha0;
    const double cq = p_coef(tn, tsl, head, kk, np, nkm1, nkp1, lte, hh, ln, alpha0);
    if (dcm) alpha0 = 0.0;
    if (ln < 32 || (ln >= 38 && ln <= 40)) coef[ln < 32 ? ln : ln - 6] = cq;
    lds_fence();
    P_STAMP(1);
    {
      const double ts = (hit_bp && tn > 0.0) ? __longlong_as_double(__double_as_longlong(tn) - 1) : (hit_bp ? nextafter(tn, -__builtin_inf()) : tn);
      if (dcm) { if (lane < n_ent) kvl[lane] = p.dc_entries[lane]; }
      else if (lane < n_ent) {
        double v = 0.0;
        if (e_nt <= 2) {
          if (e_nt > 0) {
            double u;
            if (s0_lo <= ts && ts < s0_hi) u = (s0_m == 0.0) ? s0_y : s0_y + (ts - s0_lo) * s0_m;
            else { const PPiece q = p_source_miss(C.ci, C.cd, e_i0, ts); s0_lo = q.lo; s0_hi = q.hi; s0_y = q.y; s0_m = q.m; u = q.u; }
            v += e_c0 * u;
          }
          if (e_nt > 1) {
            double u;
            if (s1_lo <= ts && ts < s1_hi) u = (s1_m == 0.0) ? s1_y : s1_y + (ts - s1_lo) * s1_m;
            else { const PPiece q = p_source_miss(C.ci, C.cd, e_i1, ts); s1_lo = q.lo; s1_hi = q.hi; s1_y = q.y; s1_m = q.m; u = q.u; }
            v += e_c1 * u;
          }
        } else for (int q = e_p0; q < e_p0 + e_nt; ++q) v += C.ent_coef()[q] * p_source_cold(C.ci, C.cd, C.ent_idx()[q], ts);
        kvl[lane] = v;
      }
    }
    P_STAMP(2);
    const int cand = (head + 1) & 7;
    double x0 = 0.0;
    {
      double pr = 0.0, hs = 0.0, m1 = 0.0, p1 = 0.0;
      const double* xr = Xh + (mine ? lane : 0);
      const double* qr = Qh + (mine ? lane : 0);
#pragma unroll
      for (int j = 0; j < 7; ++j) {
        const int so = ((head - j) & 7) * nc_s;
        const double xj = xr[so], qj = j < 5 ? qr[so] : 0.0;
        const double xv = (mine && j < nh) ? xj : 0.0;
        if (j == 0) x0 = xv;
        pr = fma(coef[8 + j + 1], xv, pr);
        m1 = fma(coef[16 + j + 1], xv, m1);
        p1 = fma(coef[24 + j + 1], xv, p1);
        if (j < 5) hs = fma(coef[j + 1], (mine && j < kk) ? qj : 0.0, hs);
      }
      if (mine) {
        xp[lane] = pr; xl[lane] = pr; hq[lane] = hs; qn[lane] = 0.0; pm[lane] = m1; pp[lane] = p1;
        wv[lane] = 1.0 / (a.reltol * fabs(x0) + a.abstol);
      }
    }
    if (dcm && mine) { xp[lane] = x0; xl[lane] = x0; hq[lane] = 0.0; pm[lane] = x0; pp[lane] = x0; }
    lds_fence();
    P_STAMP(3);

    int nstat = 1, iters = 0;
    double rate_new = -1.0, dn_prev = 0.0;
    const double rp = reset_rate ? 1.0 : rate_prev;
    bool done_own = !live;
    constexpr bool bbd = MODE == PM_BORDER;
    const int no = nc - p.nb;
    bool stop_all = false, abort_all = false;
    bool dc_bad = false;
    double bA = 0.0, bB = 0.0, bC = 0.0, bN = 0.0;
    if (live || PAIR || bbd) {
      for (int it = 0; PAIR || bbd || it <= a.maxit; ++it) {
        if (bbd && stop_all) break;
        if (PAIR) {
          if (lane == 0) pf[2 + role] = done_own ? 1 : 0;
          pair_sync();
          const int d0 = pf[2], d1 = pf[3];
          if (!bbd && ((d0 && d1) || pair_broken)) break;
          if (!(half ? d1 : d0)) {
            if (WIDE) {
              if (wmeta.mod >= 0) { if (va_lds) eval_wide_cached<true>(wmeta, ectx, wslot, xl_h, uofs_h, kvl, st_h); else eval_wide_cached<false>(wmeta, ectx, wslot, xl_h, uofs_h, kvl, st_h); }
              else if (wslot >= 0) eval_slot<true>(ectx, s_h, dofs_h, wslot, xl_h, uofs_h, kvl, svl, pl_h, st_h);
            }
            else {
            if (role == 0) eval_cached<0>(smeta, gmin_h, xl_h, kvl, svl, pl_h, st_h, kpool);
            if (role == 1 ? (p.pair_dbg & 1) == 0 : (p.pair_dbg & 1) == 1) eval_cached<1>(smeta, gmin_h, xl_h, kvl, svl, pl_h, st_h, kpool);
            }
          }
          pair_sync();
          P_STAMP(4);
          if (!bbd) {
            if (pair_broken) break;
            if (done_own) continue;
          }
        } else {
        if (WIDE) {
          if (wmeta.mod >= 0) { if (va_lds) eval_wide_cached<true>(wmeta, ectx, wslot, xl, uofs, kvl, st); else eval_wide_cached<false>(wmeta, ectx, wslot, xl, uofs, kvl, st); }
          else if (wslot >= 0) eval_slot<true>(ectx, s, dofs, wslot, xl, uofs, kvl, svl, pl, st);
        }
        else if (!bbd || live) eval_cached<-1>(smeta, gmin_h, xl, kvl, svl, pl, st, kpool);
        lds_fence();
        P_STAMP(4);
        }
        {
          const int T = (bbd && !live) ? 0 : g_trips;
          double s1 = 0.0, s2 = 0.0;
          const int gb = (int)(g_head & 0xffffu), gn = (int)(g_head >> 16);
          int rec = gn > 0 ? gb : 0;
          uint2 ow = gsrc[rec]; unsigned cw = gctl[rec];
          for (int tr = 0; tr < T; ++tr) {
            const uint2 o = ow; const unsigned c = cw;
            rec = tr + 1 < gn ? gb + tr + 1 : 0;
            ow = gsrc[rec]; cw = gctl[rec];
            const int n = (int)(c & GP_N_MASK);
            const bool vec = c & GP_VEC;
            const int off2 = vec ? SL::QO : SL::CO;
            const int o0 = (int)(o.x & 0xffffu), o1 = (int)(o.x >> 16), o2 = (int)(o.y & 0xffffu), o3 = (int)(o.y >> 16);
            const int oa = (int)((c >> GP_A_SHIFT) & GP_OFS_MASK), oc = (int)(c >> GP_C_SHIFT);
            const double a0 = st[o0], b0 = st[o0 + off2], a1 = st[o1], b1 = st[o1 + off2], a2 = st[o2], b2 = st[o2 + off2], a3 = st[o3], b3 = st[o3 + off2];
            const double hqe = Cm[oc + nc_s];
            { const double u1 = s1 + a0, u2 = s2 + b0; s1 = n > 0 ? u1 : s1; s2 = n > 0 ? u2 : s2; }
            { const double u1 = s1 + a1, u2 = s2 + b1; s1 = n > 1 ? u1 : s1; s2 = n > 1 ? u2 : s2; }
            { const double u1 = s1 + a2, u2 = s2 + b2; s1 = n > 2 ? u1 : s1; s2 = n > 2 ? u2 : s2; }
            { const double u1 = s1 + a3, u2 = s2 + b3; s1 = n > 3 ? u1 : s1; s2 = n > 3 ? u2 : s2; }
            if (c & GP_END) {
              const double G = s1 + alpha0 * s2;
              if (vec) {
                const double F = G + hqe;
                Cm[oc - nc_s] = F;
                A[oa] = -F;
              } else A[oa] = G;
              Cm[oc] = s2;
              s1 = 0.0; s2 = 0.0;
            }
          }
        }
        lds_fence();
        P_STAMP(5);
        constexpr int NCR = NC;
        double r[NCR + 1], cr[NCR];
        if constexpr (MODE == PM_BORDER) {
#pragma unroll
          for (int j = 0; j <= NCR; ++j) r[j] = (mine && j <= nc) ? A[lane * lda + j] : 0.0;
        }
        int lr = lane;
        asm volatile("" : "+v"(lr));
        const int rlim = ((bbd ? live : true) && lr < nc) ? nc : 0;
        const int rrow = rlim > 0 ? lr : 0;
        {
          const double* crow = Cm + rrow * nc_s;
#pragma unroll
          for (int j = 0; j < NCR; ++j) { const double v = crow[j]; cr[j] = j < rlim ? v : 0.0; }
        }
        const double Fr = Fv[rrow], Qr = Qv[rrow], xr_ = xl[rrow], wr = wv[rrow];
        const double Fi = rlim > 0 ? Fr : 0.0, Qi = rlim > 0 ? Qr : 0.0, xi = rlim > 0 ? xr_ : 0.0, wi = rlim > 0 ? wr : 0.0;
        const double fnorm = bcast(row_max<NCR>(fabs(Fi)), 0);
        if (bbd) {
          bool lfail = live && (!(fnorm == fnorm) || fnorm > 1e300 || dc_bad);
          const double fown = bcast(row_max<NCR>((mine && lane < no) ? fabs(Fi) : 0.0), 0);
          int piv[NCR]; int mystep; double ipiv;
          if (!lu_bbd_factor<NCR>(r, no, nc, lane, piv, mystep, ipiv)) lfail = live;
          double srec[P_NREC];
          {
            double c0 = 0.0, c1 = 0.0, cr_ = 0.0;
#pragma unroll
            for (int j = 0; j <= NCR; ++j) { if (j == no) c0 = r[j]; if (j == no + 1 && j < nc) c1 = r[j]; if (j == nc) cr_ = r[j]; }
            const bool use = live && !lfail;
            srec[0] = use ? bcast(c0, no) : 0.0; srec[1] = use ? bcast(c1, no) : 0.0; srec[2] = use ? bcast(cr_, no) : 0.0;
            const int l1 = p.nb > 1 ? no + 1 : no;
            srec[3] = (use && p.nb > 1) ? bcast(c0, l1) : 0.0; srec[4] = (use && p.nb > 1) ? bcast(c1, l1) : 0.0; srec[5] = (use && p.nb > 1) ? bcast(cr_, l1) : 0.0;
            srec[6] = (lfail ? 1.0 : 0.0) + (pair_broken ? 1048576.0 : 0.0);
            srec[7] = (dcm && live && !(fown < p.dc_abstol)) ? 1.0 : 0.0;
          }
          ++gen;
          const long long cbA = wall_clock64();
          bool okr = p_grid_reduce<true>(p, gen, srec, part, summ, &s_abort, wave, lane, wg);
          double S00 = summ[0], S01 = summ[1], g0 = summ[2], S10 = summ[3], S11 = summ[4], g1 = summ[5];
          const bool gfail = summ[6] != 0.0;
          const double n_viol = summ[7];
          if (!okr || summ[6] >= 1048576.0) abort_all = true;
          __syncthreads();
          cyc_bar += wall_clock64() - cbA;
          if (abort_all) break;
          if (gfail) { nstat = 2; break; }
          {
            const double xb0 = xl[no], xb1 = p.nb > 1 ? xl[no + 1] : 0.0;
            double hb0 = 0.0, hb1 = 0.0;
#pragma unroll
            for (int j = 0; j < 5; ++j) {
              const int sl = (head - j) & 7;
              const double w = (j < kk) ? coef[j + 1] : 0.0;
              hb0 = fma(w, (j < kk) ? Xh[sl * nc + no] : 0.0, hb0);
              if (p.nb > 1) hb1 = fma(w, (j < kk) ? Xh[sl * nc + no + 1] : 0.0, hb1);
            }
            if (dcm) { hb0 = 0.0; hb1 = 0.0; }
            for (int q = 0; q < p.n_bdev; ++q) {
              const int ta = p.bd_ta[q], tb = p.bd_tb[q];
              const double va = ta >= 0 ? (ta == 0 ? xb0 : xb1) : kvl[-ta - 1], vb = tb >= 0 ? (tb == 0 ? xb0 : xb1) : kvl[-tb - 1];
              double gj, f;
              if (p.bd_kind[q] == K_R) { gj = p.bd_val[q]; f = gj * (va - vb); }
              else {
                const double ha = ta >= 0 ? (ta == 0 ? hb0 : hb1) : 0.0, hb = tb >= 0 ? (tb == 0 ? hb0 : hb1) : 0.0;
                gj = alpha0 * p.bd_val[q]; f = gj * (va - vb) + p.bd_val[q] * (ha - hb);
              }
              if (ta == 0) { S00 += gj; g0 -= f; if (tb == 1) S01 -= gj; }
              if (ta == 1) { S11 += gj; g1 -= f; if (tb == 0) S10 -= gj; }
              if (tb == 0) { S00 += gj; g0 += f; if (ta == 1) S01 -= gj; }
              if (tb == 1) { S11 += gj; g1 += f; if (ta == 0) S10 -= gj; }
            }
          }
          double dxb0, dxb1 = 0.0;
          if (p.nb > 1) {
            const double det = S00 * S11 - S01 * S10;
            dxb0 = (g0 * S11 - S01 * g1) / det; dxb1 = (S00 * g1 - S10 * g0) / det;
          } else dxb0 = g0 / S00;
          if (wave == 0 && lane == 0) { s_bdec[0] = dxb0; s_bdec[1] = dxb1; s_bdec[2] = g0; s_bdec[3] = g1; }
          __syncthreads();
          dxb0 = s_bdec[0]; dxb1 = s_bdec[1]; g0 = s_bdec[2]; g1 = s_bdec[3];
          if (!(fabs(dxb0) < 1e300) || !(fabs(dxb1) < 1e300)) { nstat = 2; break; }
          if (dcm) {
            if (n_viol == 0.0 && fmax(fabs(g0), fabs(g1)) < p.dc_abstol) { nstat = 0; stop_all = true; continue; }
            double dx = 0.0, mo = 0.0;
            if (live) {
              dx = lu_bbd_back<NCR>(r, no, nc, lane, piv, mystep, ipiv, dxb0, dxb1);
              mo = bcast(row_max<NCR>((mine && lane < no && !(dml[lane] & 2)) ? fabs(dx) : 0.0), 0);
              if (__ballot(mine && !(dx == dx))) dc_bad = true;
            }
            double brec[P_NREC] = {0.0, 0.0, 0.0, 0.0, mo, 0.0, 0.0, 0.0};
            ++gen;
            const long long cbD = wall_clock64();
            const bool okd = p_grid_reduce(p, gen, brec, part, summ, &s_abort, wave, lane, wg);
            const double gmax = fmax(summ[4], fmax(fabs(dxb0), fabs(dxb1)));
            __syncthreads();
            cyc_bar += wall_clock64() - cbD;
            if (!okd) { abort_all = true; break; }
            const double sc = (p.dv_max > 0.0 && gmax > p.dv_max) ? p.dv_max / gmax : 1.0;
            if (live) {
              const double xn = xi + sc * dx;
              if (mine) xl[lane] = xn;
              if (__ballot(mine && (!(xn == xn) || fabs(xn) > 1e300))) dc_bad = true;
            }
            ++iters;
            if (it + 1 >= p.dc_maxit) stop_all = true;
            lds_fence();
            continue;
          }
          double e2own = 0.0, l2k = 0.0, l2m = 0.0, l2p = 0.0, lnd = 0.0, lbad = 0.0;
          if (live) {
            const double dx = lu_bbd_back<NCR>(r, no, nc, lane, piv, mystep, ipiv, dxb0, dxb1);
            const double xn = xi + dx;
            if (mine) xl[lane] = xn;
            const bool bad = mine && (!(xn == xn) || fabs(xn) > 1e300);
            double q = Qi;
// ... 254 lines not shown
```

Before: 58710.

## Track derivative sparsity in dual numbers and precompute per-class reciprocals in LDS

The dual-number type now carries a compile-time sparsity state for each partial, so operations skip partials known to be zero. Seeds have a single nonzero partial, and constants carry none. Separately, per-model-class reciprocals (1/toxe, 1/PhiBS, 1/(1-mj), and others) are computed once when parameters are loaded into LDS and read from a table. This replaces frcp calls inside every BSIM4 evaluation. The cost is extra LDS per wave and added template complexity, and signed-zero semantics must be preserved.

New measurement: 60020 (median of 6 runs). 1.02x the previous value.

```diff
diff --git a/cedarsim.jl_amd/csrc/ch_bsim4.hpp b/cedarsim.jl_amd/csrc/ch_bsim4.hpp
--- a/cedarsim.jl_amd/csrc/ch_bsim4.hpp
+++ b/cedarsim.jl_amd/csrc/ch_bsim4.hpp
@@ -281,30 +281,124 @@
   return g;
 }
 
-template <int N>
+namespace dn {
+enum : unsigned { ZP = 0, ZN = 1, ZR = 2, PR = 3, PX = 4 };
+constexpr unsigned st(unsigned s, int i) { return (s >> (3 * i)) & 7u; }
+constexpr bool has(unsigned s, int i) { return st(s, i) >= PR; }
+constexpr int slot(unsigned s, int i) { int c = 0; for (int j = 0; j < i; ++j) c += has(s, j) ? 1 : 0; return c; }
+constexpr unsigned all(int n, unsigned k) { unsigned s = 0; for (int i = 0; i < n; ++i) s |= k << (3 * i); return s; }
+constexpr unsigned mask(unsigned s, int n) { unsigned m = 0; for (int i = 0; i < n; ++i) m |= has(s, i) ? 1u << i : 0u; return m; }
+constexpr unsigned from_mask(unsigned m, int n) { unsigned s = 0; for (int i = 0; i < n; ++i) s |= (((m >> i) & 1u) ? PR : ZR) << (3 * i); return s; }
+constexpr unsigned neg1(unsigned a) { return a == ZP ? ZN : (a == ZN ? ZP : a); }
+constexpr unsigned add1(unsigned a, unsigned b) {
+  if (a >= PR && b >= PR) return PR;
+  if (a >= PR) return b == ZN ? a : PR;
+  if (b >= PR) return a == ZN ? b : PR;
+  return (a == ZR || b == ZR) ? ZR : ((a == ZN && b == ZN) ? ZN : ZP);
+}
+constexpr unsigned sub1(unsigned a, unsigned b) {
+  if (a >= PR && b >= PR) return PR;
+  if (a >= PR) return b == ZP ? a : PR;
+  if (b >= PR) return a == ZN ? b : PR;
+  return (a == ZR || b == ZR) ? ZR : ((a == ZN && b == ZP) ? ZN : ZP);
+}
+constexpr unsigned scl1(unsigned a, unsigned) { return a >= PR ? PX : ZR; }
+constexpr unsigned mul1(unsigned a, unsigned b) { return (a >= PR || b >= PR) ? PR : ZR; }
+constexpr unsigned div1(unsigned a, unsigned b) { return (a >= PR || b >= PR) ? PX : ZR; }
+constexpr unsigned lift(unsigned (*f)(unsigned, unsigned), unsigned a, unsigned b, int n) {
+  unsigned s = 0; for (int i = 0; i < n; ++i) s |= f(st(a, i), st(b, i)) << (3 * i); return s;
+}
+constexpr unsigned neg(unsigned a, int n) { unsigned s = 0; for (int i = 0; i < n; ++i) s |= neg1(st(a, i)) << (3 * i); return s; }
+CH_D double mulr(double x, double y) {
+#pragma clang fp contract(off)
+  return x * y;
+}
+}
+template <int N, unsigned S = dn::all(N, dn::PR)>
 struct DN {
-  double v, p[N];
+  static constexpr int n = N, cnt = dn::slot(S, N);
+  static constexpr unsigned state = S, mask = dn::mask(S, N);
+  double v, p[cnt ? cnt : 1];
+  DN() = default;
+  template <unsigned S2>
+  CH_D DN(const DN<N, S2>& a) {
+    v = a.v;
+    static_assert(ok_from(S2), "a conversion only widens");
+    for (int i = 0; i < N; ++i) if (dn::has(S, i)) p[dn::slot(S, i)] = a.get(i);
+  }
+  static constexpr bool ok_from(unsigned s2) {
+    for (int i = 0; i < N; ++i) {
+      const unsigned t = dn::st(S, i), f = dn::st(s2, i);
+      if (!(t == dn::PR || (t == dn::ZR && f < dn::PR) || t == f)) return false;
+    }
+    return true;
+  }
+  CH_D double get(int i) const { return dn::has(S, i) ? p[dn::slot(S, i)] : (dn::st(S, i) == dn::ZN ? -0.0 : 0.0); }
 };
 template <int N> CH_D DN<N> mkd(double v) { DN<N> r; r.v = v; for (int i = 0; i < N; ++i) r.p[i] = 0.0; return r; }
-template <int N> CH_D DN<N> operator+(DN<N> a, DN<N> b) { DN<N> r; r.v = a.v + b.v; for (int i = 0; i < N; ++i) r.p[i] = a.p[i] + b.p[i]; return r; }
-template <int N> CH_D DN<N> operator-(DN<N> a, DN<N> b) { DN<N> r; r.v = a.v - b.v; for (int i = 0; i < N; ++i) r.p[i] = a.p[i] - b.p[i]; return r; }
-template <int N> CH_D DN<N> operator-(DN<N> a) { DN<N> r; r.v = -a.v; for (int i = 0; i < N; ++i) r.p[i] = -a.p[i]; return r; }
-template <int N> CH_D DN<N> operator+(DN<N> a, double b) { a.v += b; return a; }
-template <int N> CH_D DN<N> operator+(double b, DN<N> a) { a.v += b; return a; }
-template <int N> CH_D DN<N> operator-(DN<N> a, double b) { a.v -= b; return a; }
-template <int N> CH_D DN<N> operator-(double b, DN<N> a) { DN<N> r; r.v = b - a.v; for (int i = 0; i < N; ++i) r.p[i] = -a.p[i]; return r; }
-template <int N> CH_D DN<N> operator*(DN<N> a, double b) { DN<N> r; r.v = a.v * b; for (int i = 0; i < N; ++i) r.p[i] = a.p[i] * b; return r; }
-template <int N> CH_D DN<N> operator*(double b, DN<N> a) { return a * b; }
-template <int N> CH_D DN<N> operator*(DN<N> a, DN<N> b) { DN<N> r; r.v = a.v * b.v; for (int i = 0; i < N; ++i) r.p[i] = fma(a.p[i], b.v, a.v * b.p[i]); return r; }
-template <int N> CH_D DN<N> recip(DN<N> a) { const double r = frcp(a.v), m = -r * r; DN<N> o; o.v = r; for (int i = 0; i < N; ++i) o.p[i] = a.p[i] * m; return o; }
-template <int N> CH_D DN<N> operator/(DN<N> a, DN<N> b) {
+template <int N> CH_D DN<N, dn::all(N, dn::ZP)> cstd(double v) { DN<N, dn::all(N, dn::ZP)> r; r.v = v; return r; }
+template <int N, int I> CH_D DN<N, dn::PR << (3 * I)> seed(double v) { DN<N, dn::PR << (3 * I)> r; r.v = v; r.p[0] = 1.0; return r; }
+#define CH_DN_EACH(SR) for (int i = 0; i < N; ++i) if (dn::has(SR, i))
+template <int N, unsigned SA, unsigned SB> CH_D DN<N, dn::lift(dn::add1, SA, SB, N)> operator+(DN<N, SA> a, DN<N, SB> b) {
+  constexpr unsigned SR = dn::lift(dn::add1, SA, SB, N);
+  DN<N, SR> r; r.v = a.v + b.v;
+  CH_DN_EACH(SR) {
+    double& o = r.p[dn::slot(SR, i)];
+    const unsigned sa = dn::st(SA, i), sb = dn::st(SB, i);
+    if (sa >= dn::PR && sb >= dn::PR) o = a.get(i) + b.get(i);
+    else if (sa >= dn::PR) o = (sa == dn::PX && sb != dn::ZN) ? a.get(i) + 0.0 : a.get(i);
+    else o = (sb == dn::PX && sa != dn::ZN) ? b.get(i) + 0.0 : b.get(i);
+  }
+  return r;
+}
+template <int N, unsigned SA, unsigned SB> CH_D DN<N, dn::lift(dn::sub1, SA, SB, N)> operator-(DN<N, SA> a, DN<N, SB> b) {
+  constexpr unsigned SR = dn::lift(dn::sub1, SA, SB, N);
+  DN<N, SR> r; r.v = a.v - b.v;
+  CH_DN_EACH(SR) {
+    double& o = r.p[dn::slot(SR, i)];
+    const unsigned sa = dn::st(SA, i), sb = dn::st(SB, i);
+    if (sa >= dn::PR && sb >= dn::PR) o = a.get(i) - b.get(i);
+    else if (sa >= dn::PR) o = (sa == dn::PX && sb != dn::ZP) ? a.get(i) + 0.0 : a.get(i);
+    else o = (sb == dn::PX && sa != dn::ZN) ? 0.0 - b.get(i) : -b.get(i);
+  }
+  return r;
+}
+template <int N, unsigned S> CH_D DN<N, dn::neg(S, N)> operator-(DN<N, S> a) { DN<N, dn::neg(S, N)> r; r.v = -a.v; for (int i = 0; i < a.cnt; ++i) r.p[i] = -a.p[i]; return r; }
+template <int N, unsigned S> CH_D DN<N, S> operator+(DN<N, S> a, double b) { a.v += b; return a; }
+template <int N, unsigned S> CH_D DN<N, S> operator+(double b, DN<N, S> a) { a.v += b; return a; }
+template <int N, unsigned S> CH_D DN<N, S> operator-(DN<N, S> a, double b) { a.v -= b; return a; }
+template <int N, unsigned S> CH_D DN<N, dn::neg(S, N)> operator-(double b, DN<N, S> a) { DN<N, dn::neg(S, N)> r; r.v = b - a.v; for (int i = 0; i < a.cnt; ++i) r.p[i] = -a.p[i]; return r; }
+template <int N, unsigned S> CH_D DN<N, dn::lift(dn::scl1, S, S, N)> operator*(DN<N, S> a, double b) { DN<N, dn::lift(dn::scl1, S, S, N)> r; r.v = a.v * b; for (int i = 0; i < a.cnt; ++i) r.p[i] = a.p[i] * b; return r; }
+template <int N, unsigned S> CH_D DN<N, dn::lift(dn::scl1, S, S, N)> operator*(double b, DN<N, S> a) { return a * b; }
+template <int N, unsigned SA, unsigned SB> CH_D DN<N, dn::lift(dn::mul1, SA, SB, N)> operator*(DN<N, SA> a, DN<N, SB> b) {
+  constexpr unsigned SR = dn::lift(dn::mul1, SA, SB, N);
+  DN<N, SR> r; r.v = a.v * b.v;
+  CH_DN_EACH(SR) {
+    double& o = r.p[dn::slot(SR, i)];
+    if (dn::has(SA, i) && dn::has(SB, i)) o = fma(a.get(i), b.v, a.v * b.get(i));
+    else if (dn::has(SA, i)) o = dn::mulr(a.get(i), b.v);
+    else o = dn::mulr(a.v, b.get(i));
+  }
+  return r;
+}
+template <int N, unsigned S> CH_D DN<N, dn::lift(dn::scl1, S, S, N)> recip(DN<N, S> a) { const double r = frcp(a.v), m = -r * r; DN<N, dn::lift(dn::scl1, S, S, N)> o; o.v = r; for (int i = 0; i < a.cnt; ++i) o.p[i] = a.p[i] * m; return o; }
+template <int N, unsigned SA, unsigned SB> CH_D DN<N, dn::lift(dn::div1, SA, SB, N)> operator/(DN<N, SA> a, DN<N, SB> b) {
+  constexpr unsigned SR = dn::lift(dn::div1, SA, SB, N);
   const double r = frcp(b.v), q = a.v * r;
-  DN<N> o; o.v = q; for (int i = 0; i < N; ++i) o.p[i] = fma(-q, b.p[i], a.p[i]) * r; return o;
-}
-template <int N> CH_D DN<N> operator/(DN<N> a, double b) { return a * frcp(b); }
-template <int N> CH_D DN<N> operator/(double a, DN<N> b) { return recip(b) * a; }
-template <int N> CH_D DN<N> chain(DN<N> a, double f, double fp) { DN<N> r; r.v = f; for (int i = 0; i < N; ++i) r.p[i] = a.p[i] * fp; return r; }
-template <int N> CH_D DN<N> dsqrt(DN<N> a) { const double s = fsqrt(a.v); return chain(a, s, 0.5 * frcp(s)); }
+  DN<N, SR> o; o.v = q;
+  CH_DN_EACH(SR) {
+    double& x = o.p[dn::slot(SR, i)];
+    if (dn::has(SA, i) && dn::has(SB, i)) x = fma(-q, b.get(i), a.get(i)) * r;
+    else if (dn::has(SA, i)) x = a.get(i) * r;
+    else x = dn::mulr(-q, b.get(i)) * r;
+  }
+  return o;
+}
+#undef CH_DN_EACH
+template <int N, unsigned S> CH_D DN<N, dn::lift(dn::scl1, S, S, N)> operator/(DN<N, S> a, double b) { return a * frcp(b); }
+template <int N, unsigned S> CH_D DN<N, dn::lift(dn::scl1, S, S, N)> operator/(double a, DN<N, S> b) { return recip(b) * a; }
+template <int N, unsigned S> CH_D DN<N, dn::lift(dn::scl1, S, S, N)> chain(DN<N, S> a, double f, double fp) { DN<N, dn::lift(dn::scl1, S, S, N)> r; r.v = f; for (int i = 0; i < a.cnt; ++i) r.p[i] = a.p[i] * fp; return r; }
+template <int N, unsigned S> CH_D DN<N, dn::lift(dn::scl1, S, S, N)> dsqrt(DN<N, S> a) { const double s = fsqrt(a.v); return chain(a, s, 0.5 * frcp(s)); }
 enum { KP_EXP = 0, KP_LOG = 10, KP_PRE = 22, KP_COUNT = 26 };
 #define CH_KPOOL_VALUES                                                                                                        \
                                                                                 \
@@ -355,8 +449,8 @@
 #endif
 }
 CH_D double fexp(double x) { return fexp(x, KLit{}); }
-template <int N, class K> CH_D DN<N> dexp(DN<N> a, const K k) { const double e = fexp(a.v, k); return chain(a, e, e); }
-template <int N> CH_D DN<N> dexp(DN<N> a) { return dexp(a, KLit{}); }
+template <int N, unsigned S, class K> CH_D auto dexp(DN<N, S> a, const K k) { const double e = fexp(a.v, k); return chain(a, e, e); }
+template <int N, unsigned S> CH_D auto dexp(DN<N, S> a) { return dexp(a, KLit{}); }
 template <class K>
 CH_D double flog(double x, const K k) {
 #if defined(__HIP_DEVICE_COMPILE__)
@@ -382,15 +476,15 @@
 #endif
 }
 CH_D double flog(double x) { return flog(x, KLit{}); }
-template <int N, class K> CH_D DN<N> dlog(DN<N> a, const K k) { return chain(a, flog(a.v, k), frcp(a.v)); }
-template <int N> CH_D DN<N> dlog(DN<N> a) { return chain(a, flog(a.v), frcp(a.v)); }
-
-template <int N, class K> CH_D DN<N> d_sce(DN<N> x, const K kc) {
+template <int N, unsigned S, class K> CH_D auto dlog(DN<N, S> a, const K k) { return chain(a, flog(a.v, k), frcp(a.v)); }
+template <int N, unsigned S> CH_D auto dlog(DN<N, S> a) { return chain(a, flog(a.v), frcp(a.v)); }
+
+template <int N, unsigned S, class K> CH_D DN<N, dn::from_mask(dn::mask(S, N), N)> d_sce(DN<N, S> x, const K kc) {
   if (x.v < k::EXP_TH) {
-    const DN<N> e = dexp(x, kc), m1 = e - 1.0;
+    const auto e = dexp(x, kc), m1 = e - 1.0;
     return e / (m1 * m1 + e * (2.0 * k::MIN_EXP));
   }
-  return mkd<N>(1.0 / (k::MAX_EXP - 2.0));
+  return cstd<N>(1.0 / (k::MAX_EXP - 2.0));
 }
 
 struct B4Col {
@@ -399,10 +493,64 @@
 };
 CH_D B4Col b4_col(const double* table, long col) { return B4Col{table + col * (long)B4I_COUNT}; }
 
-template <class K>
-CH_D void diode(const K kc, double vb, double Is, double Nvtm, double vjm, double IVjm, double gmin, double& i, double& g) {
+enum B4DIdx {
+  B4D_itoxe, B4D_icoxe, B4D_iLeff, B4D_isqrtPhi, B4D_ipolyT1, B4D_icdep0, B4D_iu0temp, B4D_ivsat, B4D_itoxp8, B4D_ipclmlitl,
+  B4D_ithetaRout, B4D_ipdits, B4D_itoxe3, B4D_ik1ox, B4D_iDen,
+  B4D_iNvtms, B4D_iNvtmd,
+  B4D_iPhiBS, B4D_iPhiBSWS, B4D_iPhiBSWGS, B4D_i1mjs, B4D_i1mjsws, B4D_i1mjswgs,
+  B4D_iPhiBD, B4D_iPhiBSWD, B4D_iPhiBSWGD, B4D_i1mjd, B4D_i1mjswd, B4D_i1mjswgd,
+  B4D_ickappad, B4D_ickappas, B4D_COUNT
+};
+constexpr int B4D_STRIDE = 32;
+static_assert(B4D_COUNT <= B4D_STRIDE, "one table row per class");
+CH_D double b4_derive(const B4Col P, int i) {
+  switch (i) {
+    case B4D_itoxe: return frcp(P[B4I_toxe]);
+    case B4D_icoxe: return frcp(P[B4I_coxe]);
+    case B4D_iLeff: return frcp(P[B4I_leff]);
+    case B4D_isqrtPhi: return frcp(P[B4I_sqrtPhi]);
+    case B4D_ipolyT1: return frcp(P[B4I_polyT1]);
+    case B4D_icdep0: return frcp(P[B4I_cdep0]);
+    case B4D_iu0temp: return frcp(P[B4I_u0temp]);
+    case B4D_ivsat: return frcp(P[B4I_vsattemp]);
+    case B4D_itoxp8: return frcp(P[B4I_toxp8]);
+    case B4D_ipclmlitl: return frcp(P[B4I_pclmlitl]);
+    case B4D_ithetaRout: return frcp(P[B4I_thetaRout]);
+    case B4D_ipdits: return frcp(P[B4I_pdits]);
+    case B4D_itoxe3: return frcp(P[B4I_toxe3]);
+    case B4D_ik1ox: return frcp(P[B4I_k1ox]);
+    case B4D_iDen: { const double k1ox = P[B4I_k1ox]; return frcp(k1ox <= 0.0 ? 0.25 * P[B4I_moinVtm] : P[B4I_moinVtm] * k1ox * k1ox); }
+    case B4D_iNvtms: return frcp(P[B4I_Nvtms]);
+    case B4D_iNvtmd: return frcp(P[B4I_Nvtmd]);
+    case B4D_iPhiBS: return frcp(P[B4I_PhiBS]);
+    case B4D_iPhiBSWS: return frcp(P[B4I_PhiBSWS]);
+    case B4D_iPhiBSWGS: return frcp(P[B4I_PhiBSWGS]);
+    case B4D_i1mjs: return frcp(1.0 - P[B4I_mjs]);
+    case B4D_i1mjsws: return frcp(1.0 - P[B4I_mjsws]);
+    case B4D_i1mjswgs: return frcp(1.0 - P[B4I_mjswgs]);
+    case B4D_iPhiBD: return frcp(P[B4I_PhiBD]);
+    case B4D_iPhiBSWD: return frcp(P[B4I_PhiBSWD]);
+    case B4D_iPhiBSWGD: return frcp(P[B4I_PhiBSWGD]);
+    case B4D_i1mjd: return frcp(1.0 - P[B4I_mjd]);
+    case B4D_i1mjswd: return frcp(1.0 - P[B4I_mjswd]);
+    case B4D_i1mjswgd: return frcp(1.0 - P[B4I_mjswgd]);
+    case B4D_ickappad: return frcp(P[B4I_ckappad]);
+    case B4D_ickappas: return frcp(P[B4I_ckappas]);
+  }
+  return 0.0;
+}
+struct B4DHere {
+  CH_D double get(const B4Col P, int i) const { return b4_derive(P, i); }
+};
+struct B4DTab {
+  const double* d;
+  CH_D double get(const B4Col, int i) const { return d[i]; }
+};
+
+template <class K, class DS>
+CH_D void diode(const K kc, const DS ds, const B4Col P, int iNvtm, double vb, double Is, double vjm, double IVjm, double gmin, double& i, double& g) {
   if (Is <= 0.0) { i = gmin * vb; g = gmin; return; }
-  const double iN = frcp(Nvtm);
+  const double iN = ds.get(P, iNvtm);
   if (vb <= vjm) {
     const double t = vb * iN;
     if (t < -k::EXP_TH) { i = Is * (k::MIN_EXP - 1.0) + gmin * vb; g = gmin; }
@@ -412,22 +560,22 @@
     i = IVjm - Is + s * (vb - vjm) + gmin * vb; g = s + gmin;
   }
 }
-template <class K>
-CH_D void junction(const K kc, double vb, double cz, double czsw, double czswg, double pb, double pbsw, double pbswg, double mj,
+template <class K, class DS>
+CH_D void junction(const K kc, const DS ds, const B4Col P, int d0, double vb, double cz, double czsw, double czswg, double pb, double pbsw, double pbswg, double mj,
                    double mjsw, double mjswg, double& q, double& c) {
   if (vb < 0.0) {
     q = 0.0; c = 0.0;
-    if (cz > 0.0) { const double a = 1.0 - vb * frcp(pb), s = fexp(-mj * flog(a, kc), kc); q += pb * cz * (1.0 - a * s) * frcp(1.0 - mj); c += cz * s; }
-    if (czsw > 0.0) { const double a = 1.0 - vb * frcp(pbsw), s = fexp(-mjsw * flog(a, kc), kc); q += pbsw * czsw * (1.0 - a * s) * frcp(1.0 - mjsw); c += czsw * s; }
-    if (czswg > 0.0) { const double a = 1.0 - vb * frcp(pbswg), s = fexp(-mjswg * flog(a, kc), kc); q += pbswg * czswg * (1.0 - a * s) * frcp(1.0 - mjswg); c += czswg * s; }
+    if (cz > 0.0) { const double a = 1.0 - vb * ds.get(P, d0 + 0), s = fexp(-mj * flog(a, kc), kc); q += pb * cz * (1.0 - a * s) * ds.get(P, d0 + 3); c += cz * s; }
+    if (czsw > 0.0) { const double a = 1.0 - vb * ds.get(P, d0 + 1), s = fexp(-mjsw * flog(a, kc), kc); q += pbsw * czsw * (1.0 - a * s) * ds.get(P, d0 + 4); c += czsw * s; }
+    if (czswg > 0.0) { const double a = 1.0 - vb * ds.get(P, d0 + 2), s = fexp(-mjswg * flog(a, kc), kc); q += pbswg * czswg * (1.0 - a * s) * ds.get(P, d0 + 5); c += czswg * s; }
   } else {
-    const double t0 = cz + czsw + czswg, t1 = cz * mj * frcp(pb) + czsw * mjsw * frcp(pbsw) + czswg * mjswg * frcp(pbswg);
+    const double t0 = cz + czsw + czswg, t1 = cz * mj * ds.get(P, d0 + 0) + czsw * mjsw * ds.get(P, d0 + 1) + czswg * mjswg * ds.get(P, d0 + 2);
     q = vb * (t0 + 0.5 * t1 * vb); c = t0 + t1 * vb;
   }
 }
-CH_D void overlap(double vg, double cov, double clW, double ckappa, double& q, double& c) {
+CH_D void overlap(double vg, double cov, double clW, double ckappa, double ickappa, double& q, double& c) {
   const double t0 = vg + 0.02, t1 = fsqrt(t0 * t0 + 0.08), t2 = 0.5 * (t0 - t1), dt2 = 0.5 * (1.0 - t0 * frcp(t1));
-  const double t4 = fsqrt(1.0 - 4.0 * t2 * frcp(ckappa));
+  const double t4 = fsqrt(1.0 - 4.0 * t2 * ickappa);
   q = (cov + clW) * vg - clW * (t2 + 0.5 * ckappa * (t4 - 1.0));
   c = (cov + clW) - clW * (dt2 - dt2 * frcp(t4));
 }
@@ -437,120 +585,128 @@
   DN<N> iD, iS, iB, qd, qg, qs, qb;
 };
 
-template <int N, class K>
-CH_D void b4_core(const K kc, const B4Col P, const DN<N> Vgs, const DN<N> Vds, const DN<N> Vbs, B4Core<N>& o) {
+template <int N, class K, class DS, class VG, class VD, class VB>
+CH_D void b4_core(const K kc, const DS ds, const B4Col P, const VG Vgs, const VD Vds, const VB Vbs, B4Core<N>& o) {
   using namespace k;
-  typedef DN<N> D;
-  auto dexp = [&](const D a) { return chip::dexp(a, kc); };
-  auto dlog = [&](const D a) { return chip::dlog(a, kc); };
-  auto d_sce = [&](const D a) { return chip::d_sce(a, kc); };
+  constexpr unsigned MG = VG::mask, MD = VD::mask, MB = VB::mask;
+  constexpr bool DENSE = (MG & MD & MB) == (MG | MD | MB);
+  typedef DN<N, dn::from_mask(MG, N)> DG;
+  typedef DN<N, dn::from_mask(MD, N)> DD;
+  typedef DN<N, dn::from_mask(MB, N)> DB;
+  typedef DN<N, dn::from_mask(MG | MD, N)> DGD;
+  typedef DN<N, dn::from_mask(MG | MB, N)> DGB;
+  typedef DN<N, dn::from_mask(MB | MD, N)> DBD;
+  typedef DN<N, dn::from_mask(MG | MD | MB, N)> D;
+  auto cst = [](double x) { if constexpr (DENSE) return mkd<N>(x); else return cstd<N>(x); };
+  auto dexp = [&](const auto a) { return chip::dexp(a, kc); };
+  auto dlog = [&](const auto a) { return chip::dlog(a, kc); };
+  auto d_sce = [&](const auto a) { return chip::d_sce(a, kc); };
   const double phi = P[B4I_phi], sqrtPhi = P[B4I_sqrtPhi], Vtm = P[B4I_vtm], Leff = P[B4I_leff];
-  const double coxe = P[B4I_coxe], itoxe = frcp(P[B4I_toxe]), icoxe = frcp(coxe), iLeff = frcp(Leff);
-
-  D Vbseff;
+  const double coxe = P[B4I_coxe], itoxe = ds.get(P, B4D_itoxe), icoxe = ds.get(P, B4D_icoxe), iLeff = ds.get(P, B4D_iLeff);
+
+  DB Vbseff0;
   {
     const double vbsc = P[B4I_vbsc];
-    const D t0 = Vbs - (vbsc + 0.001);
-    const D t1 = dsqrt(t0 * t0 - 0.004 * vbsc);
-    if (t0.v >= 0.0) Vbseff = 0.5 * (t0 + t1) + vbsc;
-    else Vbseff = vbsc * (1.0 + (-0.002) / (t1 - t0));
-    const double t9 = 0.95 * phi;
-    const D u0 = t9 - Vbseff - 0.001;
-    Vbseff = t9 - 0.5 * (u0 + dsqrt(u0 * u0 + 0.004 * t9));
-  }
-  const D Phis = phi - Vbseff;
-  const D sqrtPhis = dsqrt(Phis);
-  const D Xdep = sqrtPhis * (P[B4I_Xdep0] * frcp(sqrtPhi));
-
-  const D sqXdep = dsqrt(Xdep);
+    const auto t0 = Vbs - (vbsc + 0.001);
+    const auto t1 = dsqrt(t0 * t0 - 0.004 * vbsc);
+    if (t0.v >= 0.0) Vbseff0 = 0.5 * (t0 + t1) + vbsc;
+    else Vbseff0 = vbsc * (1.0 + (-0.002) / (t1 - t0));
+  }
+  const double t9b = 0.95 * phi;
+  const auto u0b = t9b - Vbseff0 - 0.001;
+  const auto Vbseff = t9b - 0.5 * (u0b + dsqrt(u0b * u0b + 0.004 * t9b));
+  const auto Phis = phi - Vbseff;
+  const auto sqrtPhis = dsqrt(Phis);
+  const auto Xdep = sqrtPhis * (P[B4I_Xdep0] * ds.get(P, B4D_isqrtPhi));
+
+  const auto sqXdep = dsqrt(Xdep);
   const double f1 = P[B4I_factor1], V0 = P[B4I_vbi_phi];
-  auto ltf = [&](double dv2) -> D {
-    const D a = Vbseff * dv2;
-    const D b = (a.v >= -0.5) ? a + 1.0 : (1.0 + 3.0 * a) / (3.0 + 8.0 * a);
+  auto ltf = [&](double dv2) {
+    const auto a = Vbseff * dv2;
+    const DB b = (a.v >= -0.5) ? DB(a + 1.0) : DB((1.0 + 3.0 * a) / (3.0 + 8.0 * a));
     return sqXdep * b * f1;
   };
-  const D Theta0 = d_sce(P[B4I_dvt1L] / ltf(P[B4I_dvt2]));
-  const D Delt_vth = Theta0 * (P[B4I_dvt0] * V0);
+  const auto Theta0 = d_sce(P[B4I_dvt1L] / ltf(P[B4I_dvt2]));
+  const auto Delt_vth = Theta0 * (P[B4I_dvt0] * V0);
   const double dvt0w = P[B4I_dvt0w];
-  D T2w = mkd<N>(0.0);
+  DB T2w = cst(0.0);
   if (dvt0w != 0.0) T2w = d_sce(P[B4I_dvt1wWL] / ltf(P[B4I_dvt2w])) * (dvt0w * V0);
-  const D T1t = P[B4I_lpe0term] + P[B4I_kt1eff] + Vbseff * P[B4I_kt2t];
-  D T3d = P[B4I_eta0] + P[B4I_etab] * Vbseff;
+  const auto T1t = P[B4I_lpe0term] + P[B4I_kt1eff] + Vbseff * P[B4I_kt2t];
+  DB T3d = P[B4I_eta0] + P[B4I_etab] * Vbseff;
   if (T3d.v < 1.0e-4) T3d = (2.0e-4 - T3d) / (3.0 - 2.0e4 * T3d);
-  const D DIBL_Sft = T3d * Vds * P[B4I_theta0vb0];
+  const auto DIBL_Sft = T3d * Vds * P[B4I_theta0vb0];
   const double vthNW = P[B4I_vthNarrowW], LpeVb = P[B4I_LpeVb], k1ox = P[B4I_k1ox], k2ox = P[B4I_k2ox];
-  D Vth = P[B4I_vth0t] + (k1ox * sqrtPhis - P[B4I_k1] * sqrtPhi) * LpeVb - k2ox * Vbseff - Delt_vth - T2w +
+  DBD Vth = P[B4I_vth0t] + (k1ox * sqrtPhis - P[B4I_k1] * sqrtPhi) * LpeVb - k2ox * Vbseff - Delt_vth - T2w +
           (P[B4I_k3] + P[B4I_k3b] * Vbseff) * vthNW + T1t - DIBL_Sft;
 
-  D n;
-  {
-    const D c1 = EPSSI / Xdep;
-    const D t4 = (P[B4I_nfactor] * c1 + (P[B4I_cdsc] + P[B4I_cdscb] * Vbseff + P[B4I_cdscd] * Vds) * Theta0 + P[B4I_cit]) * icoxe;
-    n = (t4.v >= -0.5) ? t4 + 1.0 : (1.0 + 3.0 * t4) / (3.0 + 8.0 * t4);
+  DBD n;
+  {
+    const auto c1 = EPSSI / Xdep;
+    const auto t4 = (P[B4I_nfactor] * c1 + (P[B4I_cdsc] + P[B4I_cdscb] * Vbseff + P[B4I_cdscd] * Vds) * Theta0 + P[B4I_cit]) * icoxe;
+    n = (t4.v >= -0.5) ? DBD(t4 + 1.0) : DBD((1.0 + 3.0 * t4) / (3.0 + 8.0 * t4));
   }
   {
     const double dvtp0 = P[B4I_dvtp0];
     if (dvtp0 > 0.0) {
-      const D t0 = -P[B4I_dvtp1] * Vds;
-      const D t2 = (t0.v < -EXP_TH) ? mkd<N>(MIN_EXP) : dexp(t0);
-      const D t3 = Leff + dvtp0 * (1.0 + t2);
+      const auto t0 = -P[B4I_dvtp1] * Vds;
+      const DD t2 = (t0.v < -EXP_TH) ? DD(cst(MIN_EXP)) : DD(dexp(t0));
+      const auto t3 = Leff + dvtp0 * (1.0 + t2);
       Vth = Vth - n * (Vtm * dlog(Leff / t3));
     }
   }
-  D Vgs_eff = Vgs;
+  DG Vgs_eff = Vgs;
   {
     const double ngate = P[B4I_ngate], vfbphi = P[B4I_vfb_phi];
     if (ngate > 1.0e18 && ngate < 1.0e25 && Vgs.v > vfbphi) {
-      const double iT1p = frcp(P[B4I_polyT1]);
-      const D t8 = Vgs - vfbphi;
-      const D t4 = dsqrt(1.0 + t8 * (2.0 * iT1p));
-      const D t2 = 2.0 * t8 / (t4 + 1.0);
-      const D t3 = t2 * t2 * (0.5 * iT1p);
-      const D t7 = 1.07 - t3;
-      const D t6 = dsqrt(t7 * t7 + 0.224);
+      const double iT1p = ds.get(P, B4D_ipolyT1);
+      const auto t8 = Vgs - vfbphi;
+      const auto t4 = dsqrt(1.0 + t8 * (2.0 * iT1p));
+      const auto t2 = 2.0 * t8 / (t4 + 1.0);
+      const auto t3 = t2 * t2 * (0.5 * iT1p);
+      const auto t7 = 1.07 - t3;
+      const auto t6 = dsqrt(t7 * t7 + 0.224);
       Vgs_eff = Vgs - (1.12 - 0.5 * (t7 + t6));
     }
   }
-  const D Vgst = Vgs_eff - Vth;
-
-  D Vgsteff;
-  const D inVt = recip(n * Vtm);
-  {
-    const double mstar = P[B4I_mstar], cc = coxe * frcp(P[B4I_cdep0]);
-    const D t1 = mstar * Vgst;
-    const D t2 = t1 * inVt;
-    D t10;
+  const auto Vgst = Vgs_eff - Vth;
+
+  const auto inVt = recip(n * Vtm);
+  D t10, t9;
+  {
+    const double mstar = P[B4I_mstar], cc = coxe * ds.get(P, B4D_icdep0);
+    const auto t1 = mstar * Vgst;
+    const auto t2 = t1 * inVt;
     if (t2.v > EXP_TH) t10 = t1;
     else if (t2.v < -EXP_TH) t10 = n * (Vtm * log(1.0 + MIN_EXP));
     else t10 = (n * Vtm) * dlog(1.0 + dexp(t2));
-    const D h2 = (P[B4I_voffcbn] - (1.0 - mstar) * Vgst) * inVt;
-    D t9;
+    const auto h2 = (P[B4I_voffcbn] - (1.0 - mstar) * Vgst) * inVt;
     if (h2.v < -EXP_TH) t9 = mstar + n * (cc * MIN_EXP);
     else if (h2.v > EXP_TH) t9 = mstar + n * (cc * MAX_EXP);
     else t9 = mstar + n * (cc * dexp(h2));
-    Vgsteff = t10 / t9;
-  }
-
-  const D dsp = sqrtPhis - sqrtPhi;
+  }
+  const auto Vgsteff = t10 / t9;
+
+  const auto dsp = sqrtPhis - sqrtPhi;
   D Weff = P[B4I_weff] - 2.0 * (P[B4I_dwg] * Vgsteff + P[B4I_dwb] * dsp);
   if (Weff.v < 2.0e-8) Weff = 2.0e-8 * (4.0e-8 - Weff) / (6.0e-8 - 2.0 * Weff);
   D Rds;
   {
-    const D t2 = recip(1.0 + P[B4I_prwg] * Vgsteff) + P[B4I_prwb] * dsp;
+    const auto t2 = recip(1.0 + P[B4I_prwg] * Vgsteff) + P[B4I_prwb] * dsp;
     Rds = P[B4I_rdswmin] + (t2 + dsqrt(t2 * t2 + 0.01)) * P[B4I_rds0h];
   }
-  D Abulk0, Abulk;
-  {
-    const D t1 = (0.5 * k1ox * LpeVb) / sqrtPhis + (k2ox - P[B4I_k3b] * vthNW);
-    const D t5 = Leff / (Leff + 2.0 * dsqrt(P[B4I_xj] * Xdep));
-    const D t2 = P[B4I_a0] * t5 + P[B4I_b0term];
+  DB Abulk0;
+  D Abulk;
+  {
+    const auto t1 = (0.5 * k1ox * LpeVb) / sqrtPhis + (k2ox - P[B4I_k3b] * vthNW);
+    const auto t5 = Leff / (Leff + 2.0 * dsqrt(P[B4I_xj] * Xdep));
+    const auto t2 = P[B4I_a0] * t5 + P[B4I_b0term];
     Abulk0 = 1.0 + t1 * t2;
-    const D dAdVg = -t1 * (P[B4I_agsa0] * (t5 * t5 * t5));
+    const auto dAdVg = -t1 * (P[B4I_agsa0] * (t5 * t5 * t5));
     Abulk = Abulk0 + dAdVg * Vgsteff;
     if (Abulk0.v < 0.1) Abulk0 = (0.2 - Abulk0) / (3.0 - 20.0 * Abulk0);
     if (Abulk.v < 0.1) Abulk = (0.2 - Abulk) / (3.0 - 20.0 * Abulk);
-    const D t2k = P[B4I_keta] * Vbseff;
-    const D t0k = (t2k.v >= -0.9) ? recip(1.0 + t2k) : (17.0 + 20.0 * t2k) / (0.8 + t2k);
+    const auto t2k = P[B4I_keta] * Vbseff;
+    const DB t0k = (t2k.v >= -0.9) ? DB(recip(1.0 + t2k)) : DB((17.0 + 20.0 * t2k) / (0.8 + t2k));
     Abulk = Abulk * t0k;
     Abulk0 = Abulk0 * t0k;
   }
@@ -559,120 +715,121 @@
     const int mobmod = (int)P[B4I_mobmod];
     D t5;
     if (mobmod == 0) {
-      const D t3 = (Vgsteff + Vth + Vth) * itoxe;
+      const auto t3 = (Vgsteff + Vth + Vth) * itoxe;
       t5 = t3 * (P[B4I_ua] + P[B4I_uc] * Vbseff + P[B4I_ub] * t3);
     } else if (mobmod == 1) {
-      const D t3 = (Vgsteff + Vth + Vth) * itoxe;
+      const auto t3 = (Vgsteff + Vth + Vth) * itoxe;
       t5 = t3 * (P[B4I_ua] + P[B4I_ub] * t3) * (1.0 + P[B4I_uc] * Vbseff);
     } else {
-      const D t0 = (Vgsteff + P[B4I_vtfbphi1]) * itoxe;
+      const auto t0 = (Vgsteff + P[B4I_vtfbphi1]) * itoxe;
       t5 = dexp(P[B4I_eu] * dlog(t0)) * (P[B4I_ua] + P[B4I_uc] * Vbseff);
     }
-    const D den = (t5.v >= -0.8) ? t5 + 1.0 : (0.6 + t5) / (7.0 + 10.0 * t5);
-    iueff = den * frcp(P[B4I_u0temp]);
-  }
-  const D ueff = recip(iueff);
+    const D den = (t5.v >= -0.8) ? D(t5 + 1.0) : D((0.6 + t5) / (7.0 + 10.0 * t5));
+    iueff = den * ds.get(P, B4D_iu0temp);
+  }
+  const auto ueff = recip(iueff);
   const double vsat = P[B4I_vsattemp];
-  const D WVCoxRds = Weff * Rds * (vsat * coxe);
-  const D Esat = (2.0 * vsat) * iueff;
-  const D EsatL = Esat * Leff;
-  const D iEsatL = recip(EsatL);
+  const auto WVCoxRds = Weff * Rds * (vsat * coxe);
+  const auto Esat = (2.0 * vsat) * iueff;
+  const auto EsatL = Esat * Leff;
+  const auto iEsatL = recip(EsatL);
   D Lambda;
   {
     const double a1 = P[B4I_a1], a2 = P[B4I_a2];
-    if (a1 == 0.0) Lambda = mkd<N>(a2);
+    if (a1 == 0.0) Lambda = cst(a2);
     else if (a1 > 0.0) {
       const double t0 = 1.0 - a2;
-      const D t1 = t0 - a1 * Vgsteff - 0.0001;
+      const auto t1 = t0 - a1 * Vgsteff - 0.0001;
       Lambda = a2 + t0 - 0.5 * (t1 + dsqrt(t1 * t1 + 0.0004 * t0));
     } else {
-      const D t1 = a2 + a1 * Vgsteff - 0.0001;
+      const auto t1 = a2 + a1 * Vgsteff - 0.0001;
       Lambda = 0.5 * (t1 + dsqrt(t1 * t1 + 0.0004 * a2));
     }
   }
-  const D iLam = recip(Lambda);
-  const D Vgst2Vtm = Vgsteff + 2.0 * Vtm;
-  const D iVgst2Vtm = recip(Vgst2Vtm);
+  const auto iLam = recip(Lambda);
+  const auto Vgst2Vtm = Vgsteff + 2.0 * Vtm;
+  const auto iVgst2Vtm = recip(Vgst2Vtm);
   D Vdsat;
   if (Rds.v == 0.0 && Lambda.v == 1.0) Vdsat = EsatL * Vgst2Vtm / (Abulk * EsatL + Vgst2Vtm);
   else {
-    const D t9 = Abulk * WVCoxRds;
-    const D t0 = 2.0 * Abulk * (t9 - 1.0 + iLam);
-    const D t1 = Vgst2Vtm * (2.0 * iLam - 1.0) + Abulk * EsatL + 3.0 * (Vgst2Vtm * t9);
-    const D t2 = Vgst2Vtm * (EsatL + 2.0 * (Vgst2Vtm * WVCoxRds));
+    const auto t9 = Abulk * WVCoxRds;
+    const auto t0 = 2.0 * Abulk * (t9 - 1.0 + iLam);
+    const auto t1 = Vgst2Vtm * (2.0 * iLam - 1.0) + Abulk * EsatL + 3.0 * (Vgst2Vtm * t9);
+    const auto t2 = Vgst2Vtm * (EsatL + 2.0 * (Vgst2Vtm * WVCoxRds));
     Vdsat = (t1 - dsqrt(t1 * t1 - 2.0 * t0 * t2)) / t0;
   }
   D Vdseff;
   {
     const double delta = P[B4I_delta];
-    const D t1 = Vdsat - Vds - delta;
-    const D t2 = dsqrt(t1 * t1 + 4.0 * delta * Vdsat);
+    const auto t1 = Vdsat - Vds - delta;
+    const auto t2 = dsqrt(t1 * t1 + 4.0 * delta * Vdsat);
     if (t1.v >= 0.0) Vdseff = Vdsat - 0.5 * (t1 + t2);
     else Vdseff = Vdsat * (1.0 - (2.0 * delta) / (t2 - t1));
     if (Vds.v == 0.0) Vdseff = Vds;
     if (Vdseff.v > Vds.v) Vdseff = Vds;
   }
-  const D diffVds = Vds - Vdseff;
-  const D Vasat = (EsatL + Vdsat + 2.0 * (WVCoxRds * Vgsteff) * (1.0 - 0.5 * Abulk * Vdsat * iVgst2Vtm)) / ((2.0 * iLam - 1.0) + WVCoxRds * Abulk);
+  const auto diffVds = Vds - Vdseff;
+  const auto Vasat = (EsatL + Vdsat + 2.0 * (WVCoxRds * Vgsteff) * (1.0 - 0.5 * Abulk * Vdsat * iVgst2Vtm)) / ((2.0 * iLam - 1.0) + WVCoxRds * Abulk);
   D Idl;
   {
-    const D t0 = (Vgsteff + P[B4I_vtfbphi2]) * (0.5 * frcp(P[B4I_toxp8]));
-    const D Tcen = 1.9e-9 / (1.0 + dexp(0.7 * dlog(t0)));
+    const auto t0 = (Vgsteff + P[B4I_vtfbphi2]) * (0.5 * ds.get(P, B4D_itoxp8));
+    const auto Tcen = 1.9e-9 / (1.0 + dexp(0.7 * dlog(t0)));
     const double coxp = P[B4I_coxp];
-    const D Coxeff = (EPSSI * coxp) / (EPSSI + coxp * Tcen);
-    const D beta = ueff * Coxeff * Weff * iLeff;
-    const D fg1 = Vgsteff * (1.0 - 0.5 * Vdseff * Abulk * iVgst2Vtm);
-    const D gche = beta * fg1 / (1.0 + Vdseff * iEsatL);
+    const auto Coxeff = (EPSSI * coxp) / (EPSSI + coxp * Tcen);
+    const auto beta = ueff * Coxeff * Weff * iLeff;
+    const auto fg1 = Vgsteff * (1.0 - 0.5 * Vdseff * Abulk * iVgst2Vtm);
+    const auto gche = beta * fg1 / (1.0 + Vdseff * iEsatL);
     Idl = gche / (1.0 + gche * Rds);
   }
   const double fpL = P[B4I_fproutL];
-  const D FP = (fpL <= 0.0) ? mkd<N>(1.0) : recip(1.0 + fpL * iVgst2Vtm);
+  const D FP = (fpL <= 0.0) ? D(cst(1.0)) : D(recip(1.0 + fpL * iVgst2Vtm));
   D Pvag;
   {
-    const D t9 = (P[B4I_pvag] * iEsatL) * Vgsteff;
-    Pvag = (t9.v > -0.9) ? t9 + 1.0 : (0.8 + t9) / (17.0 + 20.0 * t9);
+    const auto t9 = (P[B4I_pvag] * iEsatL) * Vgsteff;
+    Pvag = (t9.v > -0.9) ? D(t9 + 1.0) : D((0.8 + t9) / (17.0 + 20.0 * t9));
   }
   D iCclm, VACLM;
   {
     const double pl = P[B4I_pclmlitl];
     if (pl > 0.0 && diffVds.v > 1.0e-10) {
-      const D Cclm = FP * Pvag * (1.0 + Rds * Idl) * (Leff + Vdsat * ueff * (0.5 * frcp(vsat))) * frcp(pl);
+      const auto Cclm = FP * Pvag * (1.0 + Rds * Idl) * (Leff + Vdsat * ueff * (0.5 * ds.get(P, B4D_ivsat))) * ds.get(P, B4D_ipclmlitl);
       iCclm = recip(Cclm);
       VACLM = Cclm * diffVds;
-    } else { iCclm = mkd<N>(1.0 / MAX_EXP); VACLM = mkd<N>(MAX_EXP); }
+    } else { iCclm = cst(1.0 / MAX_EXP); VACLM = cst(MAX_EXP); }
   }
   D iVADIBL;
   {
     const double th = P[B4I_thetaRout];
     if (th > MIN_EXP) {
-      const D t8 = Abulk * Vdsat;
-      D va = (Vgst2Vtm - Vgst2Vtm * t8 / (Vgst2Vtm + t8)) * frcp(th);
-      const D t7 = P[B4I_pdiblb] * Vbseff;
-      va = va * ((t7.v >= -0.9) ? recip(1.0 + t7) : (17.0 + 20.0 * t7) / (0.8 + t7));
+      const auto t8 = Abulk * Vdsat;
+      const auto va0 = (Vgst2Vtm - Vgst2Vtm * t8 / (Vgst2Vtm + t8)) * ds.get(P, B4D_ithetaRout);
+      const auto t7 = P[B4I_pdiblb] * Vbseff;
+      const DB f7 = (t7.v >= -0.9) ? DB(recip(1.0 + t7)) : DB((17.0 + 20.0 * t7) / (0.8 + t7));
+      const auto va = va0 * f7;
       iVADIBL = recip(va * Pvag);
-    } else iVADIBL = mkd<N>(1.0 / MAX_EXP);
+    } else iVADIBL = cst(1.0 / MAX_EXP);
   }
   D iVADITS;
   {
     const double pdits = P[B4I_pdits];
     if (pdits > MIN_EXP) {
-      const D t0 = P[B4I_pditsd] * Vds;
-      const D t1 = (t0.v > EXP_TH) ? mkd<N>(MAX_EXP) : dexp(t0);
-      iVADITS = recip((1.0 + P[B4I_pditslL] * t1) * frcp(pdits) * FP);
-    } else iVADITS = mkd<N>(1.0 / MAX_EXP);
+      const auto t0 = P[B4I_pditsd] * Vds;
+      const DD t1 = (t0.v > EXP_TH) ? DD(cst(MAX_EXP)) : DD(dexp(t0));
+      iVADITS = recip((1.0 + P[B4I_pditslL] * t1) * ds.get(P, B4D_ipdits) * FP);
+    } else iVADITS = cst(1.0 / MAX_EXP);
   }
   D iVASCBE;
   {
     const double ps2 = P[B4I_pscbe2], ps1l = P[B4I_pscbe1l];
     if (ps2 > 0.0) {
       if (diffVds.v > ps1l / EXP_TH) iVASCBE = (ps2 * iLeff) * dexp(-ps1l / diffVds);
-      else iVASCBE = mkd<N>(ps2 * iLeff / MAX_EXP);
-    } else iVASCBE = mkd<N>(1.0 / MAX_EXP);
+      else iVASCBE = cst(ps2 * iLeff / MAX_EXP);
+    } else iVASCBE = cst(1.0 / MAX_EXP);
   }
   D Idsa = Idl * (1.0 + diffVds * iVADIBL);
   Idsa = Idsa * (1.0 + diffVds * iVADITS);
   Idsa = Idsa * (1.0 + dlog((Vasat + VACLM) / Vasat) * iCclm);
-  D Isub = mkd<N>(0.0);
+  D Isub = cst(0.0);
   {
     const double aL = P[B4I_alphaL], beta0 = P[B4I_beta0];
     if (aL > 0.0 && beta0 > 0.0) {
@@ -683,86 +840,84 @@
     }
   }
   const double nf = P[B4I_nf];
-  const D Ids = Idsa * (1.0 + diffVds * iVASCBE) * Vdseff * nf;
+  const auto Ids = Idsa * (1.0 + diffVds * iVASCBE) * Vdseff * nf;
   Isub = Isub * nf;
-  D Igidl = mkd<N>(0.0), Igisl = mkd<N>(0.0);
+  D Igidl = cst(0.0), Igisl = cst(0.0);
   {
     const double agW = P[B4I_agidlW];
     if (agW > 0.0) {
-      const double bg = P[B4I_bgidl], cg = P[B4I_cgidl], eg = P[B4I_egidl], it3x = frcp(P[B4I_toxe3]);
-      const D Vbd = Vbs - Vds;
-      const D t1 = (Vds - Vgs_eff - eg) * it3x;
+      const double bg = P[B4I_bgidl], cg = P[B4I_cgidl], eg = P[B4I_egidl], it3x = ds.get(P, B4D_itoxe3);
+      const auto Vbd = Vbs - Vds;
+      const auto t1 = (Vds - Vgs_eff - eg) * it3x;
       if (t1.v > 0.0 && Vbd.v <= 0.0) {
-        const D t2 = bg / t1;
-        const D ig = (t2.v < 100.0) ? agW * t1 * dexp(-t2) : (agW * 3.720075976e-44) * t1;
-        const D t5 = -Vbd * Vbd * Vbd;
+        const auto t2 = bg / t1;
+        const DGD ig = (t2.v < 100.0) ? DGD(agW * t1 * dexp(-t2)) : DGD((agW * 3.720075976e-44) * t1);
+        const auto t5 = -Vbd * Vbd * Vbd;
         Igidl = ig * (t5 / (cg + t5));
       }
-      const D s1 = (-Vgs_eff - eg) * it3x;
+      const auto s1 = (-Vgs_eff - eg) * it3x;
       if (s1.v > 0.0 && Vbs.v <= 0.0) {
-        const D t2 = bg / s1;
-        const D ig = (t2.v < 100.0) ? agW * s1 * dexp(-t2) : (agW * 3.720075976e-44) * s1;
-        const D t5 = -Vbs * Vbs * Vbs;
+        const auto t2 = bg / s1;
+        const DG ig = (t2.v < 100.0) ? DG(agW * s1 * dexp(-t2)) : DG((agW * 3.720075976e-44) * s1);
+        const auto t5 = -Vbs * Vbs * Vbs;
         Igisl = ig * (t5 / (cg + t5));
       }
     }
   }
-  D qg = mkd<N>(0.0), qb = mkd<N>(0.0), qsm = mkd<N>(0.0), qdm = mkd<N>(0.0);
+  D qg = cst(0.0), qb = cst(0.0), qsm = cst(0.0), qdm = cst(0.0);
   const double xpart = P[B4I_xpart];
   if (xpart >= 0.0 && (int)P[B4I_capmod] != 0) {
-    const D VbseffCV = (Vbseff.v < 0.0) ? Vbseff : phi - Phis;
+    const DB VbseffCV = (Vbseff.v < 0.0) ? DB(Vbseff) : DB(phi - Phis);
     const double CoxWL = P[B4I_CoxWL], vfbzb = P[B4I_vfbzb], Cox = P[B4I_coxp], Tox = P[B4I_toxp8], ldeb = P[B4I_ldeb];
-    const double iTox = frcp(Tox), cwl = CoxWL * icoxe;
-    const D T0q = n * (Vtm * P[B4I_noff]);
-    const D T1q = (Vgst - P[B4I_voffcv]) / T0q;
+    const double iTox = ds.get(P, B4D_itoxp8), cwl = CoxWL * icoxe;
+    const auto T0q = n * (Vtm * P[B4I_noff]);
+    const auto T1q = (Vgst - P[B4I_voffcv]) / T0q;
     D Vgc;
     if (T1q.v > EXP_TH) Vgc = Vgst - P[B4I_voffcv];
     else if (T1q.v < -EXP_TH) Vgc = T0q * log(1.0 + MIN_EXP);
     else Vgc = T0q * dlog(1.0 + dexp(T1q));
-    const D V3 = vfbzb - Vgs_eff + VbseffCV - 0.02;
-    const D Vfbeff = vfbzb - 0.5 * (V3 + dsqrt(V3 * V3 + ((vfbzb <= 0.0) ? -0.08 * vfbzb : 0.08 * vfbzb)));
-    const D tm = (Vgs_eff - VbseffCV - vfbzb) * (P[B4I_acde] * iTox);
-    D Tcen;
-    if (tm.v > -EXP_TH && tm.v < EXP_TH) Tcen = ldeb * dexp(tm);
-    else Tcen = mkd<N>(tm.v <= -EXP_TH ? ldeb * MIN_EXP : ldeb * MAX_EXP);
+    const auto V3 = vfbzb - Vgs_eff + VbseffCV - 0.02;
+    const auto Vfbeff = vfbzb - 0.5 * (V3 + dsqrt(V3 * V3 + ((vfbzb <= 0.0) ? -0.08 * vfbzb : 0.08 * vfbzb)));
+    const auto tm = (Vgs_eff - VbseffCV - vfbzb) * (P[B4I_acde] * iTox);
+    DGB Tcen0;
+    if (tm.v > -EXP_TH && tm.v < EXP_TH) Tcen0 = ldeb * dexp(tm);
+    else Tcen0 = cst(tm.v <= -EXP_TH ? ldeb * MIN_EXP : ldeb * MAX_EXP);
     const double LINK = 1.0e-11 * Tox;
-    const D V3c = ldeb - Tcen - LINK;
-    Tcen = ldeb - 0.5 * (V3c + dsqrt(V3c * V3c + 4.0 * LINK * ldeb));
-    D CoxWLcen = (Cox * EPSSI * cwl) / (Cox * Tcen + EPSSI);
-    const D Qac0 = CoxWLcen * (Vfbeff - vfbzb);
+    const auto V3c = ldeb - Tcen0 - LINK;
+    const auto Tcen1 = ldeb - 0.5 * (V3c + dsqrt(V3c * V3c + 4.0 * LINK * ldeb));
+    const auto CoxWLcen1 = (Cox * EPSSI * cwl) / (Cox * Tcen1 + EPSSI);
+    const auto Qac0 = CoxWLcen1 * (Vfbeff - vfbzb);
     const double h0 = 0.5 * k1ox;
-    const D T3s = Vgs_eff - Vfbeff - VbseffCV - Vgc;
+    const auto T3s = Vgs_eff - Vfbeff - VbseffCV - Vgc;
     D T1s;
-    if (k1ox == 0.0) T1s = mkd<N>(0.0);
-    else if (T3s.v < 0.0) T1s = h0 + T3s * frcp(k1ox);
+    if (k1ox == 0.0) T1s = cst(0.0);
+    else if (T3s.v < 0.0) T1s = h0 + T3s * ds.get(P, B4D_ik1ox);
     else T1s = dsqrt(h0 * h0 + T3s);
-    const D Qsub0 = CoxWLcen * (k1ox * (T1s - h0));
-    double Den, T0d;
-    if (k1ox <= 0.0) { Den = 0.25 * P[B4I_moinVtm]; T0d = 0.5 * sqrtPhi; }
-    else { Den = P[B4I_moinVtm] * k1ox * k1ox; T0d = k1ox * sqrtPhi; }
-    const D DeltaPhi = Vtm * dlog(1.0 + (2.0 * T0d + Vgc) * Vgc * frcp(Den));
-    const D T3t = 4.0 * (Vth - vfbzb - phi);
-    const D T0t = ((T3t.v >= 0.0) ? Vgc + T3t : Vgc + 1.0e-20) * (0.5 * iTox);
-    Tcen = 1.9e-9 / (1.0 + dexp(0.7 * dlog(T0t)));
-    CoxWLcen = (Cox * EPSSI * cwl) / (Cox * Tcen + EPSSI);
-    const D AbulkCV = Abulk0 * P[B4I_abulkCVfactor];
-    const D T1 = Vgc - DeltaPhi;
-    const D VdsatCV = T1 / AbulkCV;
-    const D T0v = VdsatCV - Vds - 0.02;
-    const D T1v = dsqrt(T0v * T0v + 0.08 * VdsatCV);
+    const auto Qsub0 = CoxWLcen1 * (k1ox * (T1s - h0));
+    const double T0d = (k1ox <= 0.0) ? 0.5 * sqrtPhi : k1ox * sqrtPhi;
+    const auto DeltaPhi = Vtm * dlog(1.0 + (2.0 * T0d + Vgc) * Vgc * ds.get(P, B4D_iDen));
+    const auto T3t = 4.0 * (Vth - vfbzb - phi);
+    const auto T0t = ((T3t.v >= 0.0) ? D(Vgc + T3t) : D(Vgc + 1.0e-20)) * (0.5 * iTox);
+    const auto Tcen = 1.9e-9 / (1.0 + dexp(0.7 * dlog(T0t)));
+    const auto CoxWLcen = (Cox * EPSSI * cwl) / (Cox * Tcen + EPSSI);
+    const auto AbulkCV = Abulk0 * P[B4I_abulkCVfactor];
+    const auto T1 = Vgc - DeltaPhi;
+    const auto VdsatCV = T1 / AbulkCV;
+    const auto T0v = VdsatCV - Vds - 0.02;
+    const auto T1v = dsqrt(T0v * T0v + 0.08 * VdsatCV);
     D VdseffCV;
     if (T0v.v >= 0.0) VdseffCV = VdsatCV - 0.5 * (T0v + T1v);
     else VdseffCV = VdsatCV * (1.0 - 0.04 / (T1v - T0v));
     if (Vds.v == 0.0) VdseffCV = Vds;
-    const D T0 = AbulkCV * VdseffCV;
-    const D T2 = 12.0 * (T1 - 0.5 * T0 + 1.0e-20);
-    const D iT2 = recip(T2);
-    const D T3 = T0 * iT2;
+    const auto T0 = AbulkCV * VdseffCV;
+    const auto T2 = 12.0 * (T1 - 0.5 * T0 + 1.0e-20);
+    const auto iT2 = recip(T2);
+    const auto T3 = T0 * iT2;
     qg = CoxWLcen * (T1 - T0 * (0.5 - T3));
     qb = CoxWLcen * (1.0 - AbulkCV) * (0.5 * VdseffCV - T3 * VdseffCV);
     if (xpart > 0.5) qsm = -CoxWLcen * (0.5 * T1 + 0.25 * T0 - 0.5 * T0 * T3);
     else if (xpart < 0.5) {
-      const D T4b = T1 * ((2.0 / 3.0) * T0 * T0 + T1 * (T1 - (4.0 / 3.0) * T0)) - (2.0 / 15.0) * T0 * T0 * T0;
+      const auto T4b = T1 * ((2.0 / 3.0) * T0 * T0 + T1 * (T1 - (4.0 / 3.0) * T0)) - (2.0 / 15.0) * T0 * T0 * T0;
       qsm = -(72.0 * CoxWLcen * (iT2 * iT2)) * T4b;
     } else qsm = -0.5 * qg;
     qg = qg + Qac0 + Qsub0 - qb;
@@ -776,35 +931,35 @@
 struct B4Two {
   double ibs, gbs, ibd, gbd, qbs, cbs, qbd, cbd, qgd, cgd, qgs, cgs, qgb, cgb;
 };
-template <class K>
-CH_D void b4_two_terminal(const K kc, const B4Col P, double vgs, double vds, double vbs, double gmin, B4Two& t) {
+template <class K, class DS>
+CH_D void b4_two_terminal(const K kc, const DS ds, const B4Col P, double vgs, double vds, double vbs, double gmin, B4Two& t) {
   const double vbd = vbs - vds;
-  diode(kc, vbs, P[B4I_Isbs], P[B4I_Nvtms], P[B4I_vjsmFwd], P[B4I_IVjsmFwd], gmin, t.ibs, t.gbs);
-  diode(kc, vbd, P[B4I_Isbd], P[B4I_Nvtmd], P[B4I_vjdmFwd], P[B4I_IVjdmFwd], gmin, t.ibd, t.gbd);
-  junction(kc, vbs, P[B4I_czbs], P[B4I_czbssw], P[B4I_czbsswg], P[B4I_PhiBS], P[B4I_PhiBSWS], P[B4I_PhiBSWGS], P[B4I_mjs], P[B4I_mjsws], P[B4I_mjswgs], t.qbs, t.cbs);
-  junction(kc, vbd, P[B4I_czbd], P[B4I_czbdsw], P[B4I_czbdswg], P[B4I_PhiBD], P[B4I_PhiBSWD], P[B4I_PhiBSWGD], P[B4I_mjd], P[B4I_mjswd], P[B4I_mjswgd], t.qbd, t.cbd);
+  diode(kc, ds, P, B4D_iNvtms, vbs, P[B4I_Isbs], P[B4I_vjsmFwd], P[B4I_IVjsmFwd], gmin, t.ibs, t.gbs);
+  diode(kc, ds, P, B4D_iNvtmd, vbd, P[B4I_Isbd], P[B4I_vjdmFwd], P[B4I_IVjdmFwd], gmin, t.ibd, t.gbd);
+  junction(kc, ds, P, B4D_iPhiBS, vbs, P[B4I_czbs], P[B4I_czbssw], P[B4I_czbsswg], P[B4I_PhiBS], P[B4I_PhiBSWS], P[B4I_PhiBSWGS], P[B4I_mjs], P[B4I_mjsws], P[B4I_mjswgs], t.qbs, t.cbs);
+  junction(kc, ds, P, B4D_iPhiBD, vbd, P[B4I_czbd], P[B4I_czbdsw], P[B4I_czbdswg], P[B4I_PhiBD], P[B4I_PhiBSWD], P[B4I_PhiBSWGD], P[B4I_mjd], P[B4I_mjswd], P[B4I_mjswgd], t.qbd, t.cbd);
   if ((int)P[B4I_capmod] != 0) {
-    overlap(vgs - vds, P[B4I_cgdo], P[B4I_cgdlW], P[B4I_ckappad], t.qgd, t.cgd);
-    overlap(vgs, P[B4I_cgso], P[B4I_cgslW], P[B4I_ckappas], t.qgs, t.cgs);
+    overlap(vgs - vds, P[B4I_cgdo], P[B4I_cgdlW], P[B4I_ckappad], ds.get(P, B4D_ickappad), t.qgd, t.cgd);
+    overlap(vgs, P[B4I_cgso], P[B4I_cgslW], P[B4I_ckappas], ds.get(P, B4D_ickappas), t.qgs, t.cgs);
     t.cgb = P[B4I_cgbo]; t.qgb = t.cgb * (vgs - vbs);
   } else { t.qgd = t.cgd = t.qgs = t.cgs = t.qgb = t.cgb = 0.0; }
 }
 
-template <class K = KLit>
-CH_D void b4_device(const B4Col P, double vd, double vg, double vs, double vb, double gmin, double* out, const K kc = K{}) {
+template <class K = KLit, class DS = B4DHere>
+CH_D void b4_device(const B4Col P, double vd, double vg, double vs, double vb, double gmin, double* out, const K kc = K{}, const DS ds = DS{}) {
   const double tp = P[B4I_type];
   const double vds = tp * (vd - vs), vgs = tp * (vg - vs), vbs = tp * (vb - vs);
   const bool fwd = vds >= 0.0;
-  typedef DN<3> D3;
-  D3 Vgs = mkd<3>(fwd ? vgs : vgs - vds), Vds = mkd<3>(fwd ? vds : -vds), Vbs = mkd<3>(fwd ? vbs : vbs - vds);
-  Vgs.p[0] = 1.0; Vds.p[1] = 1.0; Vbs.p[2] = 1.0;
+  const auto Vgs = seed<3, 0>(fwd ? vgs : vgs - vds);
+  const auto Vds = seed<3, 1>(fwd ? vds : -vds);
+  const auto Vbs = seed<3, 2>(fwd ? vbs : vbs - vds);
   B4Core<3> c;
-  b4_core<3>(kc, P, Vgs, Vds, Vbs, c);
+  b4_core<3>(kc, ds, P, Vgs, Vds, Vbs, c);
   double* I = out; double* Qo = out + 4; double* G = out + 8; double* C = out + 24;
-  auto put = [&](int row, const D3& x, double* val, double* M) {
-    val[row] = x.v; M[row * 4 + 0] = x.p[1]; M[row * 4 + 1] = x.p[0]; M[row * 4 + 3] = x.p[2]; M[row * 4 + 2] = -(x.p[0] + x.p[1] + x.p[2]);
+  auto put = [&](int row, const auto& x, double* val, double* M) {
+    val[row] = x.v; M[row * 4 + 0] = x.get(1); M[row * 4 + 1] = x.get(0); M[row * 4 + 3] = x.get(2); M[row * 4 + 2] = -(x.get(0) + x.get(1) + x.get(2));
   };
-  put(0, c.iD, I, G); put(1, mkd<3>(0.0), I, G); put(2, c.iS, I, G); put(3, c.iB, I, G);
+  put(0, c.iD, I, G); put(1, cstd<3>(0.0), I, G); put(2, c.iS, I, G); put(3, c.iB, I, G);
   put(0, c.qd, Qo, C); put(1, c.qg, Qo, C); put(2, c.qs, Qo, C); put(3, c.qb, Qo, C);
   if (!fwd) {
     auto sw = [](double& x, double& y) { const double t = x; x = y; y = t; };
@@ -815,7 +970,7 @@
     for (int r = 0; r < 4; ++r) { sw(G[r * 4 + 0], G[r * 4 + 2]); sw(C[r * 4 + 0], C[r * 4 + 2]); }
   }
   B4Two t;
-  b4_two_terminal(kc, P, vgs, vds, vbs, gmin, t);
+  b4_two_terminal(kc, ds, P, vgs, vds, vbs, gmin, t);
   auto two = [&](double* val, double* M, int a, int b, double x, double dx) {
     val[a] += x; val[b] -= x;
     M[a * 4 + a] += dx; M[a * 4 + b] -= dx; M[b * 4 + a] -= dx; M[b * 4 + b] += dx;
@@ -835,7 +990,7 @@
   D1 Vgs = mkd<1>(fwd ? vgs : vgs - vds), Vds = mkd<1>(fwd ? vds : -vds), Vbs = mkd<1>(fwd ? vbs : vbs - vds);
   Vgs.p[0] = sub == 0 ? 1.0 : 0.0; Vds.p[0] = sub == 1 ? 1.0 : 0.0; Vbs.p[0] = sub == 2 ? 1.0 : 0.0;
   B4Core<1> c;
-  b4_core<1>(KLit{}, P, Vgs, Vds, Vbs, c);
+  b4_core<1>(KLit{}, B4DHere{}, P, Vgs, Vds, Vbs, c);
   auto quad_sum = [](double x) { x += __shfl_xor(x, 1); x += __shfl_xor(x, 2); return x; };
   auto colval = [&](const D1& x) { const double sum = quad_sum(x.p[0]); return sub == 3 ? -sum : x.p[0]; };
   double gI[4] = {colval(c.iD), 0.0, colval(c.iS), colval(c.iB)};
@@ -848,7 +1003,7 @@
     col = col == 0 ? 2 : (col == 2 ? 0 : col);
   }
   B4Two t;
-  b4_two_terminal(KLit{}, P, vgs, vds, vbs, gmin, t);
+  b4_two_terminal(KLit{}, B4DHere{}, P, vgs, vds, vbs, gmin, t);
   auto two = [&](double* val, double* gcol, int a, int b, double x, double dx) {
     val[a] += x; val[b] -= x;
     const double s = col == a ? dx : (col == b ? -dx : 0.0);
diff --git a/cedarsim.jl_amd/csrc/ch_engine_persist.hpp b/cedarsim.jl_amd/csrc/ch_engine_persist.hpp
--- a/cedarsim.jl_amd/csrc/ch_engine_persist.hpp
+++ b/cedarsim.jl_amd/csrc/ch_engine_persist.hpp
@@ -37,7 +37,7 @@
 }
 inline size_t ch_circuit::persist_wave_doubles(bool wg_consts) const {
   const size_t n_ent = wg_consts ? (size_t)P_MAXSRC : desc.A.known.size() + stru.n_dev_src();
-  return stru.lds_doubles_fixed + 16 * (size_t)desc.A.max_nc + 10 + 48 + P_MAXSRC + n_ent + (size_t)tab.max_mc * B4L_STRIDE + (stru.lds_extra_bytes + stru.lds_plan_bytes + 7) / 8 + 2;
+  return stru.lds_doubles_fixed + 16 * (size_t)desc.A.max_nc + 10 + 48 + P_MAXSRC + n_ent + (size_t)tab.max_mc * (B4L_STRIDE + B4D_STRIDE) + (stru.lds_extra_bytes + stru.lds_plan_bytes + 7) / 8 + 2;
 }
 inline bool ch_circuit::persist_blob(const std::vector<int>& kn, const std::vector<int>& ds, std::vector<int>& bi, std::vector<double>& bd, std::vector<int>& need) const {
   const int nsrc = (int)desc.src.size();
diff --git a/cedarsim.jl_amd/csrc/ch_kernels.hpp b/cedarsim.jl_amd/csrc/ch_kernels.hpp
--- a/cedarsim.jl_amd/csrc/ch_kernels.hpp
+++ b/cedarsim.jl_amd/csrc/ch_kernels.hpp
@@ -263,8 +263,8 @@
   q.m = a.dmult[pi]; q.par = a.dpar[pi]; q.cls = a.dcls_local[d]; q.src = a.dsrc[d];
   return q;
 }
-template <int PART, class K = KLit>
-__device__ __forceinline__ void eval_cached(const SlotMeta& q, double gmin, const double* xl, const double* kvl, const double* svl, const double* pl, double* stage, const K kc = K{}) {
+template <int PART, class K = KLit, bool DTAB = false>
+__device__ __forceinline__ void eval_cached(const SlotMeta& q, double gmin, const double* xl, const double* kvl, const double* svl, const double* pl, double* stage, const K kc = K{}, const double* dtab = nullptr) {
   if (q.kind == 0 || (PART == 0 && q.kind != K_MOS)) return;
   double* st = stage + (size_t)q.dl * StampLayout<false>::STRIDE;
   double v[4];
@@ -273,7 +273,8 @@
   if (q.kind == K_MOS) {
     const B4Col P{pl + (size_t)q.cls * B4L_STRIDE};
     double o[40];
-    b4_device(P, v[0], v[1], v[2], v[3], gmin, o, kc);
+    if constexpr (DTAB) b4_device(P, v[0], v[1], v[2], v[3], gmin, o, kc, B4DTab{dtab + (size_t)q.cls * B4D_STRIDE});
+    else b4_device(P, v[0], v[1], v[2], v[3], gmin, o, kc);
     if (PART != 1) {
 #pragma unroll
       for (int j = 0; j < 4; ++j) st[j] = q.m * o[j];
diff --git a/cedarsim.jl_amd/csrc/ch_persist.hpp b/cedarsim.jl_amd/csrc/ch_persist.hpp
--- a/cedarsim.jl_amd/csrc/ch_persist.hpp
+++ b/cedarsim.jl_amd/csrc/ch_persist.hpp
@@ -352,7 +352,8 @@
   long long* stl = (long long*)(coef + 40);
   double* kvl = coef + 48; double* svl = kvl + (wgc ? C.ci[3] : a.nk);
   double* pl = wgc ? kvl + P_MAXSRC : svl + a.nsrc;
-  int* mptr = (int*)(pl + (size_t)a.max_mc * B4L_STRIDE);
+  double* dl = pl + (size_t)a.max_mc * B4L_STRIDE;
+  int* mptr = (int*)(dl + (size_t)a.max_mc * B4D_STRIDE);
   int* slots = mptr + (nc * nc + 1) + (nc + 1);
   const int* gplan = mptr + cm.blob_ints;
   const int g_recs = (cm.spare0 - GP_HEAD_INTS) / 3;
@@ -369,7 +370,7 @@
   const int bqh = live_h ? blk_h : 0, c_h = bqh / a.S, s_h = bqh - c_h * a.S;
   const int uofs_h = PAIR ? a.bmeta[c_h].uofs : uofs, dofs_h = PAIR ? a.bmeta[c_h].dofs : dofs;
   double* Wh = summ + P_NREC + 4 + P_SCR + (size_t)((wave & ~1) + half) * p.wave_doubles;
-  double* st_h = Wh; double* xl_h = Wh + (xl - W); double* pl_h = Wh + (pl - W);
+  double* st_h = Wh; double* xl_h = Wh + (xl - W); double* pl_h = Wh + (pl - W); double* dl_h = Wh + (dl - W);
   const int* slots_h = (const int*)((const char*)slots + ((const char*)Wh - (const char*)W));
   int pseq = 0; bool pair_broken = false;
   auto pair_sync = [&]() {
@@ -399,6 +400,12 @@
 #pragma unroll
       for (int q = 1; q < 8; ++q) cl = (j == q) ? bm.mc[q] : cl;
       pl[j * B4L_STRIDE + i] = a.mosp[((long)cl * a.Smos + scol) * (long)B4I_COUNT + i];
+    }
+    lds_fence();
+    if (lane < bm.mc_n) {
+      const B4Col Pj{pl + (size_t)lane * B4L_STRIDE};
+#pragma unroll
+      for (int e = 0; e < B4D_COUNT; ++e) dl[(size_t)lane * B4D_STRIDE + e] = b4_derive(Pj, e);
     }
     for (int i = lane; i < nc * lda + nc * nc; i += 64) A[i] = 0.0;
     if (mine) {
@@ -638,8 +645,8 @@
               else if (wslot >= 0) eval_slot<true>(ectx, s_h, dofs_h, wslot, xl_h, uofs_h, kvl, svl, pl_h, st_h);
             }
             else {
-            if (role == 0) eval_cached<0>(smeta, gmin_h, xl_h, kvl, svl, pl_h, st_h, kpool);
-            if (role == 1 ? (p.pair_dbg & 1) == 0 : (p.pair_dbg & 1) == 1) eval_cached<1>(smeta, gmin_h, xl_h, kvl, svl, pl_h, st_h, kpool);
+            if (role == 0) eval_cached<0, KLds, true>(smeta, gmin_h, xl_h, kvl, svl, pl_h, st_h, kpool, dl_h);
+            if (role == 1 ? (p.pair_dbg & 1) == 0 : (p.pair_dbg & 1) == 1) eval_cached<1, KLds, true>(smeta, gmin_h, xl_h, kvl, svl, pl_h, st_h, kpool, dl_h);
             }
           }
           pair_sync();
@@ -653,7 +660,7 @@
           if (wmeta.mod >= 0) { if (va_lds) eval_wide_cached<true>(wmeta, ectx, wslot, xl, uofs, kvl, st); else eval_wide_cached<false>(wmeta, ectx, wslot, xl, uofs, kvl, st); }
           else if (wslot >= 0) eval_slot<true>(ectx, s, dofs, wslot, xl, uofs, kvl, svl, pl, st);
         }
-        else if (!bbd || live) eval_cached<-1>(smeta, gmin_h, xl, kvl, svl, pl, st, kpool);
+        else if (!bbd || live) eval_cached<-1, KLds, true>(smeta, gmin_h, xl, kvl, svl, pl, st, kpool, dl);
         lds_fence();
         P_STAMP(4);
         }
```
